# CFGpp-diffusion/CFGpp

Hardware: AMD Instinct MI355X
Metric: images/sec (higher is better)
Workload: dtype fp16; 1 GPU; SD1.5 512x512 ddim_cfg++ 50 NFE lambda=0.6 batch=8/GPU; per_gpu_batch=8, global_batch=8, nfe=50, unet_batch_rows=16, weights=seeded synthetic, exact diffusers shapes, build_id=cfgpp-build:af47ed5b841e1037:nogit

## Files before the change

cfgpp_amd/_lib.py:

```python
from __future__ import annotations

import ctypes as C
import os

HERE = os.path.dirname(os.path.abspath(__file__))
LIB_PATH = os.environ.get("CFGPP_LIB") or os.path.join(HERE, "libcfgpp_hip.so")


class CfgppError(RuntimeError):
    pass


class UNetConfigC(C.Structure):
    _fields_ = [
        ("in_channels", C.c_int), ("out_channels", C.c_int),
        ("num_levels", C.c_int),
        ("block_out_channels", C.c_int * 4),
        ("layers_per_block", C.c_int),
        ("level_has_attn", C.c_int * 4),
        ("transformer_depth", C.c_int * 4),
        ("num_heads", C.c_int * 4),
        ("cross_attention_dim", C.c_int),
        ("addition_embed", C.c_int),
        ("addition_time_embed_dim", C.c_int),
        ("addition_pooled_dim", C.c_int),
        ("norm_groups", C.c_int),
        ("sample_h", C.c_int), ("sample_w", C.c_int),
        ("max_rows", C.c_int),
    ]


_P, _I, _F, _L = C.c_void_p, C.c_int, C.c_float, C.c_long

PROTOTYPES = {
    "cfgpp_last_error": (C.c_char_p, []),
    "cfgpp_build_id": (C.c_char_p, []),
    "cfgpp_step_ddim": (_I, [_P, _P, _P, _P, _I, _F, _F, _F, _F, _F, _I, _I, _L, _P]),
    "cfgpp_step_ddim_h": (_I, [_P, _P, _P, _P, _F, _F, _F, _F, _F, _I, _I, _L, _P]),
    "cfgpp_step_ddim_masked": (_I, [_P, _P, _P, _P, _F, _F, _F, _F, _F, _I, _I, _P, _P, _P, _F, _F, _I, _L, _P]),
    "cfgpp_kdiff_input": (_I, [_P, _P, _F, _I, _L, _P]),
    "cfgpp_step_kdiff": (_I, [_P, _P, _P, _P, _P, C.POINTER(C.c_float), _I, _I, _I, _I, _L, _P]),
    "cfgpp_kdiff_denoise": (_I, [_P, _P, _P, _F, _F, _P, _P, _L, _P]),
    "cfgpp_lincomb": (_I, [_P, _P, _P, _P, _F, _F, _I, _L, _P]),
    "cfgpp_unet_create": (_P, [C.POINTER(UNetConfigC), _I]),
    "cfgpp_unet_destroy": (None, [_P]),
    "cfgpp_unet_load_tensor": (_I, [_P, C.c_char_p, _P, _I, C.POINTER(C.c_long), _I]),
    "cfgpp_unet_missing": (_I, [_P]),
    "cfgpp_unet_finalize": (_I, [_P]),
    "cfgpp_unet_set_context": (_I, [_P, _P, _I, _I, _P, _P, _I, _P]),
    "cfgpp_unet_image_condition": (_I, [_P, _P, _I, _P]),
    "cfgpp_unet_forward": (_I, [_P, _P, _I, _I, _F, _P, _I, _P]),
    "cfgpp_sample_graph_ddim": (_I, [_P, _P, _P, _I, _I, _P, _P, _P, _I, C.POINTER(C.c_float), _I, _F, _I, _I, _P]),
    "cfgpp_unet_profile": (_I, [_P, _P, _I, _I, _F, _P, _I, _P, C.POINTER(C.c_double), C.POINTER(C.c_double), C.POINTER(C.c_int), C.c_char_p, _L]),
    "cfgpp_unet_tuning": (_I, [_P, _I, C.POINTER(C.c_int), _I, _I]),
    "cfgpp_unet_attach_control": (_I, [_P, _P, _F]),
    "cfgpp_unet_flops": (C.c_double, [_P, _I]),
    "cfgpp_unet_device_bytes": (C.c_double, [_P]),
    "cfgpp_vae_create": (_P, [_I, _I, _I, _F, _I]),
    "cfgpp_vae_destroy": (None, [_P]),
    "cfgpp_vae_load_tensor": (_I, [_P, C.c_char_p, _P, _I, C.POINTER(C.c_long), _I]),
    "cfgpp_vae_finalize": (_I, [_P]),
    "cfgpp_vae_decode": (_I, [_P, _P, _P, _I, _P]),
    "cfgpp_vae_decode_image": (_I, [_P, _P, _P, _I, _P]),
    "cfgpp_vae_encode": (_I, [_P, _P, _P, _P, _P, _I, _P]),
    "cfgpp_vae_profile": (_I, [_P, _P, _P, _I, _P, C.c_char_p, C.c_long]),
    "cfgpp_vae_flops": (C.c_double, [_P, _I]),
    "cfgpp_text_create": (_P, [_I, _I, _I, _I, _I, _I, _I, _I, _I]),
    "cfgpp_text_destroy": (None, [_P]),
    "cfgpp_text_load_tensor": (_I, [_P, C.c_char_p, _P, _I, C.POINTER(C.c_long), _I]),
    "cfgpp_text_finalize": (_I, [_P]),
    "cfgpp_text_encode": (_I, [_P, C.POINTER(C.c_int), C.POINTER(C.c_int), _I, _I, _P, _P, _P]),
    "cfgpp_text_device_bytes": (C.c_double, [_P]),
    "cfgpp_vae_encode_flops": (C.c_double, [_P, _I]),
    "cfgpp_vae_device_bytes": (C.c_double, [_P]),
}

DEBUG_PROTOTYPES = {
    "cfgpp_op_softmax_rows": (_I, [_P, _L, _I, _P]),
    "cfgpp_op_conv_in_ex": (_I, [_P, _I, _P, _P, _P, _I, _I, _I, _I, _I, _I, _P, _P, _F, _P]),
    "cfgpp_op_groupnorm": (_I, [_P, _P, _P, _P, _P, _P, _I, _I, _I, _I, _I, _I, _F, _I, _I, _P]),
    "cfgpp_op_groupnorm_pre": (_I, [_P, _P, _P, _P, _P, _P, _P, _P, _I, _I, _I, _I, _I, _I, _F, _I, _I, _P]),
    "cfgpp_op_igemm_set_gstat": (None, [_P]),
    "cfgpp_op_igemm_gstat_written": (_I, []),
    "cfgpp_groupnorm_set_prestats": (None, [_I]),
    "cfgpp_groupnorm_prestats_enabled": (_I, []),
    "cfgpp_unet_set_share_prefix": (None, [_I]),
    "cfgpp_unet_share_prefix_enabled": (_I, []),
    "cfgpp_unet_shared_prefix_ops": (_I, [_P, _I, _I]),
    "cfgpp_op_layernorm": (_I, [_P, _P, _P, _P, _L, _I, _F, _P]),
    "cfgpp_op_attention_prepare_vt": (_I, [_P, _I, _I, _I, _P]),
    "cfgpp_op_attention": (_I, [_P, _P, _P, _P, _I, _I, _I, _I, _I, _I, _I, _P]),
    "cfgpp_op_conv_in": (_I, [_P, _I, _P, _P, _P, _I, _I, _I, _I, _I, _I, _P]),
    "cfgpp_op_conv_in_cond": (_I, [_P, _I, _P, _I, _I, _P, _P, _P, _I, _I, _I, _I, _I, _I, _P]),
    "cfgpp_op_conv_in_add": (_I, [_P, _I, _P, _I, _I, _P, _I, _P, _P, _P, _I, _I, _I, _I, _I, _I, _P]),
    "cfgpp_op_cn_conv3x3": (_I, [_P, _I, _P, _I, _P, _P, _I, _I, _I, _I, _I, _I, _I, _P]),
    "cfgpp_op_residual_add": (_I, [C.POINTER(C.c_void_p), C.POINTER(C.c_void_p), C.POINTER(C.c_int), _I, _I, _F, _P]),
    "cfgpp_op_residual_nchw": (_I, [_P, _P, _I, _I, _I, _I, _F, _P]),
    "cfgpp_controlnet_residual": (_I, [_P, _I, _F, _P, _I, C.POINTER(C.c_int), _P]),
    "cfgpp_op_vae_posterior": (_I, [_P, _P, _P, _P, _P, _P, _I, _I, _F, _P]),
    "cfgpp_op_conv_out": (_I, [_P, _P, _I, _P, _P, _I, _I, _I, _I, _I, _P]),
    "cfgpp_op_conv_out_ex": (_I, [_P, _P, _I, _P, _P, _I, _I, _I, _I, _I, _F, _F, _I, _P]),
    "cfgpp_conv_out_set_tiled": (None, [_I]),
    "cfgpp_op_sinusoid": (_I, [_P, _F, _P, _I, _I, _I, _I, _P]),
    "cfgpp_op_skinny_gemm": (_I, [_P, _I, _P, _P, _P, _I, _P, _I, _I, _I, _I, _I, _I, _P]),
    "cfgpp_op_f16_to_f32_rows": (_I, [_P, _P, _I, _I, _I, _I, _P]),
    "cfgpp_op_igemm": (_I, [_P, _P, _I, _I, _I, _I, _I, _I, _P, _I, _I, _P, _P, _I, _P, _I, _I, _P, _I, _I, _I, _P]),
    "cfgpp_op_igemm_heads": (_I, [_P, _I, _P, _I, _I, _P, _I, _P, _P, _P, _I, _I, _I, _I, _I, _I, _P]),
    "cfgpp_igemm_force_config": (None, [_I]),
    "cfgpp_igemm_set_staging": (None, [_I]),
    "cfgpp_igemm_set_staged_epilogue": (None, [_I]),
    "cfgpp_igemm_set_big_tiles": (None, [_I]),
    "cfgpp_igemm_set_tail_split": (None, [_I]),
    "cfgpp_igemm_set_autotune": (None, [_I]),
    "cfgpp_igemm_set_blocked_walk": (None, [_I]),
    "cfgpp_igemm_walk_plan_probe": (None, [_I, _I, _I, _I, _I, _I, _I, C.POINTER(C.c_int)]),
    "cfgpp_igemm_set_n_major": (None, [_I]),
    "cfgpp_igemm_force_split": (None, [_I]),
    "cfgpp_igemm_set_split_tile": (None, [_I]),
    "cfgpp_igemm_set_mf16": (None, [_I]),
    "cfgpp_igemm_set_mf16_rounds": (None, [_I]),
    "cfgpp_igemm_set_mf16_heads": (None, [_I]),
    "cfgpp_igemm_set_mf16_linear": (None, [_I]),
    "cfgpp_igemm_set_big_split": (None, [_I]),
    "cfgpp_igemm_set_tune_mask": (None, [C.c_uint]),
    "cfgpp_igemm_tuner_state": (C.c_uint, []),
    "cfgpp_igemm_timeline": (None, [_P, _L, _I]),
    "cfgpp_igemm_timeline_info": (None, [C.POINTER(C.c_int)]),
    "cfgpp_groupnorm_set_mode": (None, [_I]),
    "cfgpp_layernorm_set_rows_per_wave": (None, [_I]),
    "cfgpp_attention_set_dma": (None, [_I]),
    "cfgpp_attention_set_stagger": (None, [_I]),
    "cfgpp_attention_set_cross": (None, [_I]),
}

_lib = None


def load():
    global _lib
    if _lib is not None:
        return _lib
    if not os.path.exists(LIB_PATH):
        raise CfgppError(
            f"{LIB_PATH} not found: build it with `python -m cfgpp_amd.build` "
            "(__graft_entry__.build()).  The HIP path has no CPU fallback.")
    import torch
    try:
        lib = C.CDLL(LIB_PATH)
    except OSError as e:
        raise CfgppError(f"cannot load {LIB_PATH}: {e}") from e
    for name, (res, args) in list(PROTOTYPES.items()) + list(DEBUG_PROTOTYPES.items()):
        try:
            fn = getattr(lib, name)
        except AttributeError as e:
            raise CfgppError(f"{LIB_PATH} does not export {name}") from e
        fn.restype = res
        fn.argtypes = args
    if os.environ.get("CFGPP_AUTOTUNE", "1") == "0":
        lib.cfgpp_igemm_set_autotune(0)
    _lib = lib
    return lib


def build_id() -> str:
    return load().cfgpp_build_id().decode("utf-8", "replace")


def last_error() -> str:
    return load().cfgpp_last_error().decode("utf-8", "replace")


def check(rc: int, what: str):
    if rc != 0:
        raise CfgppError(f"{what} failed (rc={rc}): {last_error()}")
```

cfgpp_amd/build.py:

```python
from __future__ import annotations

import hashlib
import os
import subprocess
import sys
from concurrent.futures import ThreadPoolExecutor

HERE = os.path.dirname(os.path.abspath(__file__))
CSRC = os.path.join(HERE, "csrc")
OUT = os.path.join(HERE, "libcfgpp_hip.so")
OBJ = os.path.join(CSRC, "_obj")

SOURCES = [
    ("errors.cpp", []),
    ("step_kernels.hip", ["-ffp-contract=off"]),
    ("norm_kernels.hip", []),
    ("small_kernels.hip", []),
    ("igemm_kernel.hip", []),
    ("big4_kernel.hip", []),
    ("big4p_kernel.hip", []),
    ("attn_kernel.hip", ["-mllvm", "-amdgpu-mfma-vgpr-form=1"]),
    ("controlnet_kernels.hip", ["-ffp-contract=off"]),
    ("unet.hip", []),
    ("vae.hip", []),
    ("text.hip", []),
]
COMMON = ["--offload-arch=gfx950", "-O3", "-std=c++17", "-fPIC", "-Wno-unused-result"]
ASAN_FLAGS = ["-fsanitize=address", "-fno-gpu-sanitize", "-g", "-fno-omit-frame-pointer"]


def _hipcc() -> str:
    for c in (os.environ.get("HIPCC"), "/opt/rocm/bin/hipcc", "hipcc"):
        if c and (os.path.isabs(c) and os.path.exists(c) or not os.path.isabs(c)):
            return c
    return "hipcc"


_INC = None


def _deps(src: str) -> set:
    import re
    global _INC
    if _INC is None:
        _INC = re.compile(r'^\s*#\s*include\s+"([^"]+)"', re.M)
    seen, todo = set(), [src]
    while todo:
        f = todo.pop()
        try:
            text = open(f, errors="replace").read()
        except OSError:
            continue
        for inc in _INC.findall(text):
            h = os.path.normpath(os.path.join(os.path.dirname(f), inc))
            if h not in seen and os.path.exists(h):
                seen.add(h)
                todo.append(h)
    return seen


def _digest(src: str, flags) -> str:
    h = hashlib.sha256()
    h.update((" ".join(flags) + "\0" + _hipcc_version()).encode())
    for f in [src, *sorted(_deps(src))]:
        h.update(os.path.relpath(f, HERE).encode() + b"\0")
        with open(f, "rb") as fh:
            h.update(fh.read())
    return h.hexdigest()[:16]


_HIPCC_VERSION = None


def _hipcc_version() -> str:
    global _HIPCC_VERSION
    if _HIPCC_VERSION is None:
        try:
            out = subprocess.run([_hipcc(), "--version"], capture_output=True, text=True).stdout
            _HIPCC_VERSION = " ".join(ln.strip() for ln in out.splitlines() if "version" in ln.lower())[:200]
        except OSError:
            _HIPCC_VERSION = "unknown"
    return _HIPCC_VERSION


def source_digest() -> str:
    h = hashlib.sha256()
    for f, extra in SOURCES:
        h.update(_digest(os.path.join(CSRC, f), COMMON + extra).encode())
    return h.hexdigest()[:16]


def _git_head() -> str:
    try:
        root = os.path.dirname(HERE)
        head = subprocess.run(["git", "-C", root, "rev-parse", "--short=12", "HEAD"], capture_output=True, text=True).stdout.strip()
        dirty = subprocess.run(["git", "-C", root, "status", "--porcelain", "--", "cfgpp_amd/csrc", "include"], capture_output=True,
                               text=True).stdout.strip()
        return (head or "nogit") + ("+local" if dirty else "")
    except OSError:
        return "nogit"


def library_build_id(path: str = OUT) -> str:
    try:
        data = open(path, "rb").read()
    except OSError:
        return ""
    i = data.find(b"cfgpp-build:")
    return data[i:data.index(b"\0", i)].decode() if i >= 0 else ""


def build_asan(verbose: bool = True) -> str:
    out = os.path.join(HERE, "libcfgpp_hip_asan.so")
    obj_dir = os.path.join(CSRC, "_obj_asan")
    os.makedirs(obj_dir, exist_ok=True)
    hipcc = _hipcc()
    jobs, objs = [], []
    for f, extra in SOURCES:
        src = os.path.join(CSRC, f)
        flags = COMMON + ASAN_FLAGS + extra
        obj = os.path.join(obj_dir, f"{os.path.splitext(f)[0]}.{_digest(src, flags)}.o")
        objs.append(obj)
        if not os.path.exists(obj):
            jobs.append((f, [hipcc] + flags + ["-x", "hip", "-c", src, "-o", obj]))
    with ThreadPoolExecutor(max_workers=8) as ex:
        for f, r in zip([j[0] for j in jobs], ex.map(lambda j: subprocess.run(j[1], capture_output=True, text=True), jobs)):
            if verbose:
                print(f"[cfgpp build asan] {f}: {'ok' if r.returncode == 0 else 'FAILED'}", flush=True)
            if r.returncode != 0:
                raise RuntimeError(f"hipcc failed on {f}:\n{r.stdout}{r.stderr}")
    bid_src = os.path.join(obj_dir, "build_id.cpp")
    with open(bid_src, "w") as fh:
        fh.write('extern "C" const char* cfgpp_build_id(void) { return "cfgpp-build:%s:%s+asan"; }\n' % (source_digest(), _git_head()))
    cmd = [hipcc, "--offload-arch=gfx950", "-shared", "-fPIC", "-fsanitize=address", "-fno-gpu-sanitize", "-shared-libsan", "-o", out] + objs + [bid_src]
    r = subprocess.run(cmd, capture_output=True, text=True)
    if r.returncode != 0:
        raise RuntimeError("asan link failed:\n" + r.stdout + r.stderr)
    if verbose:
        print(f"[cfgpp build asan] linked {out}", flush=True)
    return out


def build(force: bool = False, verbose: bool = True) -> str:
    os.makedirs(OBJ, exist_ok=True)
    hipcc = _hipcc()
    jobs, objs = [], []
    for f, extra in SOURCES:
        src = os.path.join(CSRC, f)
        stem = os.path.splitext(f)[0]
        obj = os.path.join(OBJ, f"{stem}.{_digest(src, COMMON + extra)}.o")
        objs.append(obj)
        if force or not os.path.exists(obj):
            jobs.append((f, [hipcc] + COMMON + extra + ["-x", "hip", "-c", src, "-o", obj]))

    def run(job):
        f, cmd = job
        r = subprocess.run(cmd, capture_output=True, text=True)
        if r.returncode != 0 and os.path.exists(cmd[-1]):
            os.remove(cmd[-1])
        return f, r.returncode, r.stdout + r.stderr

    if jobs:
        with ThreadPoolExecutor(max_workers=min(8, len(jobs))) as ex:
            for f, rc, log in ex.map(run, jobs):
                if verbose:
                    print(f"[cfgpp build] {f}: {'ok' if rc == 0 else 'FAILED'}", flush=True)
                if rc != 0:
                    raise RuntimeError(f"hipcc failed on {f}:\n{log}")
    keep = set(objs)
    for old in os.listdir(OBJ):
        if old.endswith(".o") and os.path.join(OBJ, old) not in keep:
            os.remove(os.path.join(OBJ, old))
    want = source_digest()
    have = library_build_id()
    if force or jobs or not have.startswith(f"cfgpp-build:{want}:"):
        bid_src, bid_obj = os.path.join(OBJ, "build_id.cpp"), os.path.join(OBJ, "build_id.o")
        with open(bid_src, "w") as fh:
            fh.write('extern "C" const char* cfgpp_build_id(void) { return "cfgpp-build:%s:%s"; }\n' % (want, _git_head()))
        r = subprocess.run([hipcc, "-O2", "-fPIC", "-c", bid_src, "-o", bid_obj], capture_output=True, text=True)
        if r.returncode != 0:
            raise RuntimeError("build_id.cpp failed:\n" + r.stdout + r.stderr)
        cmd = [hipcc, "--offload-arch=gfx950", "-shared", "-fPIC", "-o", OUT + ".tmp"] + objs + [bid_obj]
        r = subprocess.run(cmd, capture_output=True, text=True)
        if r.returncode != 0:
            raise RuntimeError("link failed:\n" + r.stdout + r.stderr)
        os.replace(OUT + ".tmp", OUT)
        os.remove(bid_obj)
        if verbose:
            print(f"[cfgpp build] linked {OUT} ({library_build_id()})", flush=True)
    return OUT


if __name__ == "__main__":
    if "--asan" in sys.argv:
        print(build_asan())
    else:
        build(force="--force" in sys.argv)
        print(library_build_id())
```

cfgpp_amd/csrc/attn_kernel.hip:

```cpp
#include "common.h"

namespace {

constexpr float RESCALE_THR = 5.0f;

struct AttnArgs {
    const half_t* q; const half_t* k; const half_t* vt;
    half_t* o;
    int heads, d;
    int nq, nk_valid;
    int q_tok_pad, k_tok_pad;
    int o_ld;
    int nqb;
    float scale_log2e;
    int stagger;
};

__device__ __forceinline__ void attn_block_map(int nqb, int& qb, int& bh) {
    const int T = gridDim.x, bid = blockIdx.x;
    const int q = T >> 3, r = T & 7, xcd = bid & 7, idx = bid >> 3;
    const int w = (xcd < r ? xcd * (q + 1) : r * (q + 1) + (xcd - r) * q) + idx;
    bh = w / nqb; qb = w - bh * nqb;
}

template <int D16, int DT, bool ONES, int QT>
__global__ void __launch_bounds__(256)
attn_kernel(const AttnArgs a) {
    constexpr int DP = DT * 32;
    constexpr int KPITCH = DP * 2 + 16;
    constexpr int VPITCH = 64 * 2 + 16;
    constexpr int CH = (64 * DP / 8) / 256;
    constexpr int STAGE = 64 * KPITCH + DP * VPITCH;
    static_assert((64 * DP / 8) % 256 == 0, "tile/loader mismatch");
    extern __shared__ __attribute__((aligned(16))) char smem[];

    const int tid = threadIdx.x, lane = tid & 63, wid = tid >> 6;
    const int l31 = lane & 31, hi = lane >> 5;
    int qb, bh;
    attn_block_map(a.nqb, qb, bh);
    const int q0 = qb * (128 * QT) + wid * (32 * QT);
    const half_t* Qb = a.q + (long)bh * a.q_tok_pad * DP;
    const half_t* Kb = a.k + (long)bh * a.k_tok_pad * DP;
    const half_t* Vb = a.vt + (long)bh * DP * a.k_tok_pad;

    half8_t qf[QT][D16];
#pragma unroll
    for (int qt = 0; qt < QT; ++qt)
#pragma unroll
        for (int ks = 0; ks < D16; ++ks) {
            const half8_t raw = *reinterpret_cast<const half8_t*>(Qb + (long)(q0 + qt * 32 + l31) * DP + ks * 16 + hi * 8);
#pragma unroll
            for (int j = 0; j < 8; ++j) qf[qt][ks][j] = (half_t)((float)raw[j] * a.scale_log2e);
        }

    f32x16 oacc[QT][DT];
    f32x16 negm[QT];
    float l_run[QT];
#pragma unroll
    for (int qt = 0; qt < QT; ++qt) {
        l_run[qt] = 0.f;
#pragma unroll
        for (int r = 0; r < 16; ++r) negm[qt][r] = 0.f;
#pragma unroll
        for (int i = 0; i < DT; ++i)
#pragma unroll
            for (int r = 0; r < 16; ++r) oacc[qt][i][r] = 0.f;
    }

    const int ntiles = (a.nk_valid + 63) >> 6;
    const int tail = a.nk_valid & 63;

    half8_t rk[CH], rv[CH];
    auto load_tile = [&](int t) {
#pragma unroll
        for (int j = 0; j < CH; ++j) {
            const int c = tid + j * 256;
            const int kr = c / (DP / 8), kc = c - kr * (DP / 8);
            rk[j] = *reinterpret_cast<const half8_t*>(Kb + (long)(t * 64 + kr) * DP + kc * 8);
            const int vr = c >> 3, vc = c & 7;
            rv[j] = *reinterpret_cast<const half8_t*>(Vb + (long)vr * a.k_tok_pad + t * 64 + vc * 8);
        }
    };
    auto store_tile = [&](int stage) {
        char* Ks = smem + stage * STAGE;
        char* Vs = Ks + 64 * KPITCH;
#pragma unroll
        for (int j = 0; j < CH; ++j) {
            const int c = tid + j * 256;
            const int kr = c / (DP / 8), kc = c - kr * (DP / 8);
            *reinterpret_cast<half8_t*>(Ks + kr * KPITCH + kc * 16) = rk[j];
            const int vr = c >> 3, vc = c & 7;
            *reinterpret_cast<half8_t*>(Vs + vr * VPITCH + vc * 16) = rv[j];
        }
    };

    load_tile(0);
    store_tile(0);
    __syncthreads();
    if (ntiles > 1) load_tile(1);
    for (int t = 0; t < ntiles; ++t) {
        const char* Ks = smem + (t & 1) * STAGE;
        const char* Vs = Ks + 64 * KPITCH;

        f32x16 s[QT][2];
#pragma unroll
        for (int kt = 0; kt < 2; ++kt) {
#pragma unroll
            for (int ks = 0; ks < D16; ++ks) {
                const half8_t kf = *reinterpret_cast<const half8_t*>(Ks + (kt * 32 + l31) * KPITCH + (ks * 16 + hi * 8) * 2);
#pragma unroll
                for (int qt = 0; qt < QT; ++qt)
                    s[qt][kt] = __builtin_amdgcn_mfma_f32_32x32x16_f16(kf, qf[qt][ks], ks == 0 ? negm[qt] : s[qt][kt], 0, 0, 0);
            }
        }
        if (tail != 0 && t == ntiles - 1) {
            const int kbase = t * 64 + 4 * hi;
#pragma unroll
            for (int qt = 0; qt < QT; ++qt)
#pragma unroll
                for (int kt = 0; kt < 2; ++kt)
#pragma unroll
                    for (int r = 0; r < 16; ++r) {
                        const int key = kbase + kt * 32 + (r & 3) + 8 * (r >> 2);
                        s[qt][kt][r] = key < a.nk_valid ? s[qt][kt][r] : -INFINITY;
                    }
        }
#pragma unroll
        for (int qt = 0; qt < QT; ++qt) {
            float mx = s[qt][0][0];
#pragma unroll
            for (int kt = 0; kt < 2; ++kt)
#pragma unroll
                for (int r = 0; r < 16; ++r) mx = fmaxf(mx, s[qt][kt][r]);
            mx = fmaxf(mx, __shfl_xor(mx, 32));
            if (t == 0 || !__all(mx <= RESCALE_THR)) {
                const float delta = t == 0 ? mx : fmaxf(mx, 0.f);
                const float alpha = __builtin_amdgcn_exp2f(-delta);
                l_run[qt] *= alpha;
#pragma unroll
                for (int i = 0; i < DT; ++i)
#pragma unroll
                    for (int r = 0; r < 16; ++r) oacc[qt][i][r] *= alpha;
#pragma unroll
                for (int r = 0; r < 16; ++r) negm[qt][r] -= delta;
#pragma unroll
                for (int kt = 0; kt < 2; ++kt)
#pragma unroll
                    for (int r = 0; r < 16; ++r) s[qt][kt][r] -= delta;
            }
            float psum = 0.f;
#pragma unroll
            for (int kt = 0; kt < 2; ++kt)
#pragma unroll
                for (int r = 0; r < 16; ++r) {
                    const float pv = __builtin_amdgcn_exp2f(s[qt][kt][r]);
                    s[qt][kt][r] = pv;
                    if constexpr (!ONES) psum += pv;
                }
            if constexpr (!ONES) l_run[qt] += psum;
        }

#pragma unroll
        for (int kt = 0; kt < 2; ++kt)
#pragma unroll
            for (int tt = 0; tt < 2; ++tt) {
                half8_t pf[QT];
#pragma unroll
                for (int qt = 0; qt < QT; ++qt)
#pragma unroll
                    for (int j = 0; j < 8; ++j) pf[qt][j] = (half_t)s[qt][kt][8 * tt + j];
                const int kpos0 = kt * 32 + 16 * tt + 8 * hi;
#pragma unroll
                for (int i = 0; i < DT; ++i) {
                    const half8_t vf = *reinterpret_cast<const half8_t*>(Vs + (i * 32 + l31) * VPITCH + kpos0 * 2);
#pragma unroll
                    for (int qt = 0; qt < QT; ++qt)
                        oacc[qt][i] = __builtin_amdgcn_mfma_f32_32x32x16_f16(vf, pf[qt], oacc[qt][i], 0, 0, 0);
                }
            }
        if (t + 1 < ntiles) store_tile((t + 1) & 1);
        __syncthreads();
        if (t + 2 < ntiles) load_tile(t + 2);
    }

#pragma unroll
    for (int qt = 0; qt < QT; ++qt) {
        float l_tot;
        if constexpr (ONES) {
            const int dr = a.d & 31;
            float lv = 0.f;
#pragma unroll
            for (int g = 0; g < 4; ++g) if (dr == 8 * g) lv = oacc[qt][DT - 1][4 * g];
            l_tot = __shfl(lv, l31);
        } else {
            l_tot = l_run[qt] + __shfl_xor(l_run[qt], 32);
        }
        const float inv_l = 1.0f / l_tot;
        const int q = q0 + qt * 32 + l31;
        if (q < a.nq) {
            const int b = bh / a.heads, head = bh - b * a.heads;
            half_t* orow = a.o + ((long)b * a.nq + q) * a.o_ld + head * a.d;
#pragma unroll
            for (int i = 0; i < DT; ++i)
#pragma unroll
                for (int g = 0; g < 4; ++g) {
                    const int dd = i * 32 + 8 * g + 4 * hi;
                    if (dd < a.d) {
                        half4_t o;
#pragma unroll
                        for (int k = 0; k < 4; ++k) o[k] = (half_t)(oacc[qt][i][4 * g + k] * inv_l);
                        *reinterpret_cast<half4_t*>(orow + dd) = o;
                    }
                }
        }
    }
}

template <int D16, bool ONES, int NST, int WPE = 3>
__global__ void __launch_bounds__(256) __attribute__((amdgpu_waves_per_eu(WPE, WPE)))
attn64_kernel(const AttnArgs a) {
    constexpr int DP = 64, DT = 2;
    constexpr int TILE = 64 * 128;
    constexpr int STAGE = 2 * TILE;
    constexpr int PPW = 4;
    extern __shared__ __attribute__((aligned(16))) char smem[];

    const int tid = threadIdx.x, lane = tid & 63;
    const int wid = __builtin_amdgcn_readfirstlane(tid >> 6);
    const int l31 = lane & 31, hi = lane >> 5;
    int qb, bh;
    attn_block_map(a.nqb, qb, bh);
    const int q0 = qb * 128 + wid * 32;
    const half_t* Qb = a.q + (long)bh * a.q_tok_pad * DP;
    const half_t* Kb = a.k + (long)bh * a.k_tok_pad * DP;
    const half_t* Vb = a.vt + (long)bh * DP * a.k_tok_pad;

    const int r8 = lane >> 3, pc = lane & 7;
    int koff[2], voff[2];
#pragma unroll
    for (int h = 0; h < 2; ++h) {
        const int row = wid * 16 + h * 8 + r8;
        const int lc = pc ^ ((row >> 1) & 7);
        koff[h] = row * DP + lc * 8;
        voff[h] = row * a.k_tok_pad + lc * 8;
    }
    auto dma_tile = [&](int t, int stage) {
        char* Ks = smem + stage * STAGE;
        char* Vs = Ks + TILE;
        const half_t* Kt = Kb + (long)t * 64 * DP;
        const half_t* Vt = Vb + (long)t * 64;
#pragma unroll
        for (int h = 0; h < 2; ++h) {
            __builtin_amdgcn_global_load_lds((const __attribute__((address_space(1))) void*)(Kt + koff[h]),
                                             (__attribute__((address_space(3))) void*)(Ks + (wid * 16 + h * 8) * 128), 16, 0, 0);
            __builtin_amdgcn_global_load_lds((const __attribute__((address_space(1))) void*)(Vt + voff[h]),
                                             (__attribute__((address_space(3))) void*)(Vs + (wid * 16 + h * 8) * 128), 16, 0, 0);
        }
    };

    const int ntiles = (a.nk_valid + 63) >> 6;
    const int tail = a.nk_valid & 63;
    if (a.stagger > 0) {
        const int slot = ((blockIdx.x >> 3) >> 5) % 3;
        for (int i = 0; i < slot * a.stagger; ++i) __builtin_amdgcn_s_sleep(1);
    }
#pragma unroll
    for (int t = 0; t < NST - 1; ++t) if (t < ntiles) dma_tile(t, t);

    half8_t qf[D16];
#pragma unroll
    for (int ks = 0; ks < D16; ++ks) {
        const half8_t raw = *reinterpret_cast<const half8_t*>(Qb + (long)(q0 + l31) * DP + ks * 16 + hi * 8);
#pragma unroll
        for (int j = 0; j < 8; ++j) qf[ks][j] = (half_t)((float)raw[j] * a.scale_log2e);
    }

    f32x16 oacc[DT];
    f32x16 negm;
    float l_run = 0.f;
#pragma unroll
    for (int r = 0; r < 16; ++r) negm[r] = 0.f;
#pragma unroll
    for (int i = 0; i < DT; ++i)
#pragma unroll
        for (int r = 0; r < 16; ++r) oacc[i][r] = 0.f;

    const int fsw = (l31 >> 1) & 7;
    const int frow = l31 * 128;
    for (int t = 0; t < ntiles; ++t) {
        if (NST > 2 && t + 1 < ntiles) asm volatile("s_waitcnt vmcnt(%0)" :: "n"((NST - 2) * PPW) : "memory");
        else asm volatile("s_waitcnt vmcnt(0)" ::: "memory");
        __builtin_amdgcn_s_barrier();
        asm volatile("" ::: "memory");
        if (t + NST - 1 < ntiles) dma_tile(t + NST - 1, (t + NST - 1) % NST);
        const char* Ks = smem + (t % NST) * STAGE;
        const char* Vs = Ks + TILE;

        f32x16 s[2];
        {
#pragma unroll
            for (int kt = 0; kt < 2; ++kt) {
#pragma unroll
                for (int k0 = 0; k0 < D16; k0 += 2) {
                    half8_t kf1[2];
#pragma unroll
                    for (int u = 0; u < 2; ++u)
                        if (k0 + u < D16) kf1[u] = *reinterpret_cast<const half8_t*>(Ks + kt * 32 * 128 + frow + (((((k0 + u) << 1) | hi) ^ fsw) << 4));
#pragma unroll
                    for (int u = 0; u < 2; ++u)
                        if (k0 + u < D16) s[kt] = __builtin_amdgcn_mfma_f32_32x32x16_f16(kf1[u], qf[k0 + u], k0 + u == 0 ? negm : s[kt], 0, 0, 0);
                    __builtin_amdgcn_sched_barrier(0);
                }
            }
        }
        if (tail != 0 && t == ntiles - 1) {
            const int kbase = t * 64 + 4 * hi;
#pragma unroll
            for (int kt = 0; kt < 2; ++kt)
#pragma unroll
                for (int r = 0; r < 16; ++r) {
                    const int key = kbase + kt * 32 + (r & 3) + 8 * (r >> 2);
                    s[kt][r] = key < a.nk_valid ? s[kt][r] : -INFINITY;
                }
        }
        float mx = s[0][0];
#pragma unroll
        for (int kt = 0; kt < 2; ++kt)
#pragma unroll
            for (int r = 0; r < 16; ++r) mx = fmaxf(mx, s[kt][r]);
        mx = fmaxf(mx, __shfl_xor(mx, 32));
        if (t == 0 || !__all(mx <= RESCALE_THR)) {
            const float delta = t == 0 ? mx : fmaxf(mx, 0.f);
            const float alpha = __builtin_amdgcn_exp2f(-delta);
            l_run *= alpha;
#pragma unroll
            for (int i = 0; i < DT; ++i)
#pragma unroll
                for (int r = 0; r < 16; ++r) oacc[i][r] *= alpha;
#pragma unroll
            for (int r = 0; r < 16; ++r) negm[r] -= delta;
#pragma unroll
            for (int kt = 0; kt < 2; ++kt)
#pragma unroll
                for (int r = 0; r < 16; ++r) s[kt][r] -= delta;
        }
        float psum = 0.f;
#pragma unroll
        for (int kt = 0; kt < 2; ++kt)
#pragma unroll
            for (int r = 0; r < 16; ++r) {
                const float pv = __builtin_amdgcn_exp2f(s[kt][r]);
                s[kt][r] = pv;
                if constexpr (!ONES) psum += pv;
            }
        if constexpr (!ONES) l_run += psum;

#pragma unroll
        for (int kt = 0; kt < 2; ++kt)
#pragma unroll
            for (int tt = 0; tt < 2; ++tt) {
                half8_t pf;
#pragma unroll
                for (int j = 0; j < 8; ++j) pf[j] = (half_t)s[kt][8 * tt + j];
                const int lc = kt * 4 + 2 * tt + hi;
#pragma unroll
                for (int i = 0; i < DT; ++i) {
                    const half8_t vf = *reinterpret_cast<const half8_t*>(Vs + i * 32 * 128 + frow + ((lc ^ fsw) << 4));
                    oacc[i] = __builtin_amdgcn_mfma_f32_32x32x16_f16(vf, pf, oacc[i], 0, 0, 0);
                }
            }
    }

    int lane_f = threadIdx.x & 63;
    asm volatile("" : "+v"(lane_f));
    const int l31_f = lane_f & 31, hi_f = lane_f >> 5;
    float l_tot;
    if constexpr (ONES) {
        const int dr = a.d & 31;
        float lv = 0.f;
#pragma unroll
        for (int g = 0; g < 4; ++g) if (dr == 8 * g) lv = oacc[DT - 1][4 * g];
        l_tot = __shfl(lv, l31_f);
    } else {
        l_tot = l_run + __shfl_xor(l_run, 32);
    }
    const float inv_l = 1.0f / l_tot;
    const int q = qb * 128 + wid * 32 + l31_f;
    if (q < a.nq) {
        const int b = bh / a.heads, head = bh - b * a.heads;
        half_t* orow = a.o + ((long)b * a.nq + q) * a.o_ld + head * a.d;
#pragma unroll
        for (int i = 0; i < DT; ++i)
#pragma unroll
            for (int g = 0; g < 4; ++g) {
                const int dd = i * 32 + 8 * g + 4 * hi_f;
                if (dd < a.d) {
                    half4_t o;
#pragma unroll
                    for (int k = 0; k < 4; ++k) o[k] = (half_t)(oacc[i][4 * g + k] * inv_l);
                    *reinterpret_cast<half4_t*>(orow + dd) = o;
                }
            }
    }
}

template <int D16, bool ONES>
__global__ void __launch_bounds__(256)
xattn64_kernel(const AttnArgs a, int xqb , int nxb ) {
    constexpr int DP = 64, DT = 2, TILE = 64 * 128;
    extern __shared__ __attribute__((aligned(16))) char smem[];
    const int tid = threadIdx.x, lane = tid & 63;
    const int wid = __builtin_amdgcn_readfirstlane(tid >> 6);
    const int l31 = lane & 31, hi = lane >> 5;
    int xb, bh;
    {
        const int T = gridDim.x, bid = blockIdx.x;
        const int q = T >> 3, r = T & 7, xcd = bid & 7, idx = bid >> 3;
        const int w = (xcd < r ? xcd * (q + 1) : r * (q + 1) + (xcd - r) * q) + idx;
        bh = w / nxb; xb = w - bh * nxb;
    }
    const half_t* Qb = a.q + (long)bh * a.q_tok_pad * DP;
    const half_t* Kb = a.k + (long)bh * a.k_tok_pad * DP;
    const half_t* Vb = a.vt + (long)bh * DP * a.k_tok_pad;
    const int ntiles = (a.nk_valid + 63) >> 6;
    {
        const int r8 = lane >> 3, pc = lane & 7;
#pragma unroll
        for (int t = 0; t < 2; ++t) {
            if (t < ntiles) {
#pragma unroll
                for (int h = 0; h < 2; ++h) {
                    const int row = wid * 16 + h * 8 + r8;
                    const int lc = pc ^ ((row >> 1) & 7);
                    __builtin_amdgcn_global_load_lds((const __attribute__((address_space(1))) void*)(Kb + (long)(t * 64 + row) * DP + lc * 8),
                                                     (__attribute__((address_space(3))) void*)(smem + t * 2 * TILE + (wid * 16 + h * 8) * 128), 16, 0, 0);
                    __builtin_amdgcn_global_load_lds((const __attribute__((address_space(1))) void*)(Vb + (long)row * a.k_tok_pad + t * 64 + lc * 8),
                                                     (__attribute__((address_space(3))) void*)(smem + t * 2 * TILE + TILE + (wid * 16 + h * 8) * 128), 16, 0, 0);
                }
            }
        }
    }
    const int fsw = (l31 >> 1) & 7;
    const int frow = l31 * 128;
    const int nsub = (a.nk_valid + 31) >> 5;
    const int b = bh / a.heads, head = bh - b * a.heads;
    half8_t qf[D16];
    int q0 = (xb * xqb) * 128 + wid * 32;
#pragma unroll
    for (int ks = 0; ks < D16; ++ks) qf[ks] = *reinterpret_cast<const half8_t*>(Qb + (long)(q0 + l31) * DP + ks * 16 + hi * 8);
    asm volatile("s_waitcnt vmcnt(0)" ::: "memory");
    __syncthreads();
    for (int blk = 0; blk < xqb; ++blk) {
        half8_t qs[D16];
#pragma unroll
        for (int ks = 0; ks < D16; ++ks)
#pragma unroll
            for (int j = 0; j < 8; ++j) qs[ks][j] = (half_t)((float)qf[ks][j] * a.scale_log2e);
        const int qrow = q0 + l31;
        const int q0n = blk + 1 < xqb ? q0 + 128 : q0;
#pragma unroll
        for (int ks = 0; ks < D16; ++ks) qf[ks] = *reinterpret_cast<const half8_t*>(Qb + (long)(q0n + l31) * DP + ks * 16 + hi * 8);
        f32x16 s[4];
#pragma unroll
        for (int st = 0; st < 4; ++st) {
#pragma unroll
            for (int r = 0; r < 16; ++r) s[st][r] = 0.f;
            if (st < nsub) {
                const char* Ks = smem + (st >> 1) * 2 * TILE + (st & 1) * 32 * 128;
#pragma unroll
                for (int ks = 0; ks < D16; ++ks) {
                    const half8_t kf = *reinterpret_cast<const half8_t*>(Ks + frow + ((((ks << 1) | hi) ^ fsw) << 4));
                    s[st] = __builtin_amdgcn_mfma_f32_32x32x16_f16(kf, qs[ks], s[st], 0, 0, 0);
                }
            }
        }
        float mx = -INFINITY;
#pragma unroll
        for (int st = 0; st < 4; ++st) {
            if (st < nsub) {
                if (st == nsub - 1 && (a.nk_valid & 31) != 0) {
                    const int nv = (a.nk_valid & 31) - 4 * hi;
#pragma unroll
                    for (int r = 0; r < 16; ++r) s[st][r] = ((r & 3) + 8 * (r >> 2)) < nv ? s[st][r] : -INFINITY;
                }
#pragma unroll
                for (int r = 0; r < 16; ++r) mx = fmaxf(mx, s[st][r]);
            }
        }
        mx = fmaxf(mx, __shfl_xor(mx, 32));
        float psum = 0.f;
#pragma unroll
        for (int st = 0; st < 4; ++st) {
            if (st < nsub) {
#pragma unroll
                for (int r = 0; r < 16; ++r) {
                    const float pv = __builtin_amdgcn_exp2f(s[st][r] - mx);
                    s[st][r] = pv;
                    if constexpr (!ONES) psum += pv;
                }
            }
        }
        f32x16 oacc[DT];
#pragma unroll
        for (int i = 0; i < DT; ++i)
#pragma unroll
            for (int r = 0; r < 16; ++r) oacc[i][r] = 0.f;
#pragma unroll
        for (int st = 0; st < 4; ++st) {
            if (st < nsub) {
                const char* Vs = smem + (st >> 1) * 2 * TILE + TILE;
#pragma unroll
                for (int tt = 0; tt < 2; ++tt) {
                    half8_t pf;
#pragma unroll
                    for (int j = 0; j < 8; ++j) pf[j] = (half_t)s[st][8 * tt + j];
                    const int lc = (st & 1) * 4 + 2 * tt + hi;
#pragma unroll
                    for (int i = 0; i < DT; ++i) {
                        const half8_t vf = *reinterpret_cast<const half8_t*>(Vs + i * 32 * 128 + frow + ((lc ^ fsw) << 4));
                        oacc[i] = __builtin_amdgcn_mfma_f32_32x32x16_f16(vf, pf, oacc[i], 0, 0, 0);
                    }
                }
            }
        }
        float l_tot;
        if constexpr (ONES) {
            const int dr = a.d & 31;
            float lv = 0.f;
#pragma unroll
            for (int g = 0; g < 4; ++g) if (dr == 8 * g) lv = oacc[DT - 1][4 * g];
            l_tot = __shfl(lv, l31);
        } else {
            l_tot = psum + __shfl_xor(psum, 32);
        }
        const float inv_l = 1.0f / l_tot;
        if (qrow < a.nq) {
            half_t* orow = a.o + ((long)b * a.nq + qrow) * a.o_ld + head * a.d;
#pragma unroll
            for (int i = 0; i < DT; ++i)
#pragma unroll
                for (int g = 0; g < 4; ++g) {
                    const int dd = i * 32 + 8 * g + 4 * hi;
                    if (dd < a.d) {
                        half4_t o;
#pragma unroll
                        for (int k = 0; k < 4; ++k) o[k] = (half_t)(oacc[i][4 * g + k] * inv_l);
                        *reinterpret_cast<half4_t*>(orow + dd) = o;
                    }
                }
        }
        q0 = q0n;
    }
}

template <int D16, bool ONES, int NST, int WPE = 3>
int launch_attn64(const AttnArgs& a, dim3 grid, hipStream_t s) {
    constexpr int smem = NST * 2 * 64 * 128;
    static bool attr_set = false;
    auto kern = attn64_kernel<D16, ONES, NST, WPE>;
    if (!attr_set) {
        CFGPP_HIP_CHECK(hipFuncSetAttribute(reinterpret_cast<const void*>(kern), hipFuncAttributeMaxDynamicSharedMemorySize, smem));
        attr_set = true;
    }
    hipLaunchKernelGGL(kern, grid, dim3(256), smem, s, a);
    return 0;
}

__global__ void attn_ones_row_kernel(half_t* vt, int BH, int d, int dp, int tok_pad) {
    const long i = (long)blockIdx.x * blockDim.x + threadIdx.x;
    if (i >= (long)BH * tok_pad) return;
    const long bh = i / tok_pad, k = i - bh * tok_pad;
    vt[(bh * dp + d) * tok_pad + k] = (half_t)1.0f;
}

template <int D16, int DT, bool ONES, int QT>
int launch_attn(const AttnArgs& a, dim3 grid, hipStream_t s) {
    constexpr int DP = DT * 32;
    constexpr int smem = 2 * (64 * (DP * 2 + 16) + DP * (64 * 2 + 16));
    static bool attr_set = false;
    auto kern = attn_kernel<D16, DT, ONES, QT>;
    if (!attr_set) {
        CFGPP_HIP_CHECK(hipFuncSetAttribute(reinterpret_cast<const void*>(kern), hipFuncAttributeMaxDynamicSharedMemorySize, smem));
        attr_set = true;
    }
    hipLaunchKernelGGL(kern, grid, dim3(256), smem, s, a);
    return 0;
}

}

static int g_attn_dma = 1;
static int g_attn_cross = 1;
static int g_attn_stagger = 0;

extern "C" {

void cfgpp_attention_set_dma(int mode) { g_attn_dma = mode ? 1 : 0; }
void cfgpp_attention_set_stagger(int sleeps) { g_attn_stagger = sleeps > 0 ? sleeps : 0; }
void cfgpp_attention_set_cross(int on) { g_attn_cross = on ? 1 : 0; }

int cfgpp_op_attention_prepare_vt(void* vt, int BH, int d, int tok_pad, void* stream) {
    CFGPP_REQUIRE(vt && BH > 0 && d > 0 && tok_pad > 0, "attention_prepare_vt: bad args");
    if (d % 32 == 0) return 0;
    CFGPP_REQUIRE(d % 8 == 0, "attention: head dim %d (not a multiple of 32) must be a multiple of 8", d);
    const int dp = (d + 31) / 32 * 32;
    hipLaunchKernelGGL(attn_ones_row_kernel, dim3(cdiv((long)BH * tok_pad, 256)), dim3(256), 0, (hipStream_t)stream, (half_t*)vt, BH, d, dp, tok_pad);
    CFGPP_HIP_CHECK(hipGetLastError());
    return 0;
}

int cfgpp_op_attention(const void* q, const void* k, const void* vt, void* o, int B, int heads, int d,
                       int nq, int nk, int q_tok_pad, int k_tok_pad, void* stream) {
    CFGPP_REQUIRE(q && k && vt && o, "attention: null pointer");
    CFGPP_REQUIRE(d > 0 && d <= 160 && (d % 32 == 0 || d % 8 == 0), "attention: head dim %d unsupported (multiple of 8, <= 160)", d);
    CFGPP_REQUIRE(q_tok_pad % 128 == 0 && q_tok_pad >= nq, "attention: q_tok_pad=%d (nq=%d) must be a multiple of 128", q_tok_pad, nq);
    CFGPP_REQUIRE(k_tok_pad % 64 == 0 && k_tok_pad >= nk, "attention: k_tok_pad=%d (nk=%d) must be a multiple of 64", k_tok_pad, nk);
    AttnArgs a;
    a.q = (const half_t*)q; a.k = (const half_t*)k; a.vt = (const half_t*)vt; a.o = (half_t*)o;
    a.heads = heads; a.d = d; a.nq = nq; a.nk_valid = nk; a.q_tok_pad = q_tok_pad; a.k_tok_pad = k_tok_pad;
    a.o_ld = heads * d;
    a.scale_log2e = (1.0f / sqrtf((float)d)) * 1.4426950408889634f;
    a.nqb = cdiv(nq, 128);
    a.stagger = g_attn_stagger;
    dim3 grid(a.nqb * B * heads);
    hipStream_t s = (hipStream_t)stream;
    const int d16 = (d + 15) / 16, dt = (d + 31) / 32;
    const bool ones = (d % 32) != 0;
    if (dt == 2 && g_attn_dma && g_attn_cross && nk <= 128 && k_tok_pad >= 64 * ((nk + 63) >> 6)) {
        const int BH = B * heads;
        int xqb = 1;
        while (xqb < 8 && a.nqb % (xqb * 2) == 0 && (long)BH * (a.nqb / (xqb * 2)) >= 512) xqb *= 2;
        const int nxb = a.nqb / xqb;
        static bool attr_set = false;
        if (!attr_set) {
            CFGPP_HIP_CHECK(hipFuncSetAttribute(reinterpret_cast<const void*>(xattn64_kernel<3, true>), hipFuncAttributeMaxDynamicSharedMemorySize, 4 * 64 * 128));
            CFGPP_HIP_CHECK(hipFuncSetAttribute(reinterpret_cast<const void*>(xattn64_kernel<4, true>), hipFuncAttributeMaxDynamicSharedMemorySize, 4 * 64 * 128));
            CFGPP_HIP_CHECK(hipFuncSetAttribute(reinterpret_cast<const void*>(xattn64_kernel<4, false>), hipFuncAttributeMaxDynamicSharedMemorySize, 4 * 64 * 128));
            attr_set = true;
        }
        const dim3 xg(BH * nxb);
        if (d16 == 3) hipLaunchKernelGGL((xattn64_kernel<3, true>), xg, dim3(256), 4 * 64 * 128, s, a, xqb, nxb);
        else if (ones) hipLaunchKernelGGL((xattn64_kernel<4, true>), xg, dim3(256), 4 * 64 * 128, s, a, xqb, nxb);
        else hipLaunchKernelGGL((xattn64_kernel<4, false>), xg, dim3(256), 4 * 64 * 128, s, a, xqb, nxb);
        CFGPP_HIP_CHECK(hipGetLastError());
        return 0;
    }
    if (dt == 2 && g_attn_dma) {
        int rc;
        if (d16 == 3) rc = launch_attn64<3, true, 2, 4>(a, grid, s);
        else rc = ones ? launch_attn64<4, true, 2, 4>(a, grid, s) : launch_attn64<4, false, 2, 4>(a, grid, s);
        if (rc) return -1;
        CFGPP_HIP_CHECK(hipGetLastError());
        return 0;
    }
#define ATTN_CASE(D16_, DT_) \
    if (d16 == D16_ && dt == DT_) { if (ones ? launch_attn<D16_, DT_, true, 1>(a, grid, s) : launch_attn<D16_, DT_, false, 1>(a, grid, s)) return -1; } else
    ATTN_CASE(1, 1) ATTN_CASE(2, 1) ATTN_CASE(3, 2) ATTN_CASE(4, 2) ATTN_CASE(5, 3) ATTN_CASE(6, 3)
    ATTN_CASE(8, 4) ATTN_CASE(10, 5)
    { cfgpp_set_error("attention: no kernel instance for head dim %d", d); return -2; }
#undef ATTN_CASE
    CFGPP_HIP_CHECK(hipGetLastError());
    return 0;
}

}
```

cfgpp_amd/csrc/cfgpp_debug.h:

```cpp
#ifndef CFGPP_DEBUG_H
#define CFGPP_DEBUG_H
#ifdef __cplusplus
extern "C" {
#endif

int cfgpp_op_softmax_rows(void* s, long rows, int ncols, void* stream);
int cfgpp_op_conv_in_ex(const void* z, int z_is_half, void* out, const float* w, const float* bias,
                        int R, int zB, int Cin, int H, int W, int Cout, const float* pre_w, const float* pre_b,
                        float in_scale, void* stream);
int cfgpp_op_groupnorm(const void* src0, const void* src1, void* dst, const float* gamma, const float* beta,
                       float* stats, int N, int H, int W, int C0, int C1, int G, float eps, int silu,
                       int dst_padded, void* stream);
int cfgpp_op_groupnorm_pre(const void* src0, const void* src1, void* dst, const float* gamma, const float* beta,
                           const float* gst0, const float* gst1, float* stats, int N, int H, int W, int C0, int C1, int G,
                           float eps, int silu, int dst_padded, void* stream);
void cfgpp_op_igemm_set_gstat(void* buf);
int cfgpp_op_igemm_gstat_written(void);
void cfgpp_groupnorm_set_prestats(int on);
int cfgpp_groupnorm_prestats_enabled(void);
void cfgpp_unet_set_share_prefix(int on);
int cfgpp_unet_share_prefix_enabled(void);
int cfgpp_unet_shared_prefix_ops(cfgpp_unet* u, int rows, int z_rows);
void cfgpp_groupnorm_set_mode(int mode);
int cfgpp_op_layernorm(const void* x, void* y, const float* gamma, const float* beta, long rows, int C,
                       float eps, void* stream);
void cfgpp_layernorm_set_rows_per_wave(int rpw);
int cfgpp_op_attention_prepare_vt(void* vt, int BH, int d, int tok_pad, void* stream);
int cfgpp_op_attention(const void* q, const void* k, const void* vt, void* o, int B, int heads, int d,
                       int nq, int nk, int q_tok_pad, int k_tok_pad, void* stream);
void cfgpp_attention_set_dma(int mode);
void cfgpp_attention_set_stagger(int sleeps);
void cfgpp_attention_set_cross(int on);
int cfgpp_op_conv_in(const void* z, int z_is_half, void* out, const float* w, const float* bias,
                     int R, int zB, int Cin, int H, int W, int Cout, void* stream);
int cfgpp_op_conv_in_cond(const void* z, int z_is_half, const void* cond, int cond_rows, int Cc, void* out, const float* w,
                          const float* bias, int R, int zB, int Cz, int H, int W, int Cout, void* stream);
int cfgpp_op_conv_in_add(const void* z, int z_is_half, const void* cond, int cond_rows, int Cc, const void* addend, int add_rows,
                         void* out, const float* w, const float* bias, int R, int zB, int Cz, int H, int W, int Cout, void* stream);
int cfgpp_op_cn_conv3x3(const void* in, int in_kind, void* out, int out_pad, const float* w, const float* bias, int R, int Ci, int Co,
                        int Hi, int Wi, int stride, int silu, void* stream);
int cfgpp_op_residual_add(void* const* dst, const void* const* src, const int* hwc, int n, int rows, float scale, void* stream);
int cfgpp_op_residual_nchw(const void* src, float* out, int rows, int H, int W, int C, float scale, void* stream);
int cfgpp_controlnet_residual(cfgpp_unet* cn, int i, float scale, float* out, int rows, int* hwc_out, void* stream);

int cfgpp_op_vae_posterior(const float* conv_out, const float* qw, const float* qb, const float* noise, float* z,
                           float* moments, int B, int HW, float scale, void* stream);
int cfgpp_op_conv_out(const void* x, void* out, int out_is_half, const void* w, const float* bias,
                      int R, int H, int W, int C, int Cout, void* stream);
int cfgpp_op_conv_out_ex(const void* x, void* out, int out_is_half, const void* w, const float* bias,
                         int R, int H, int W, int C, int Cout, float post_scale, float post_shift, int clamp01, void* stream);
void cfgpp_conv_out_set_tiled(int on);
int cfgpp_op_sinusoid(const float* vals, float scalar, float* out, int count, int dim, int out_ld, int out_off,
                      void* stream);
int cfgpp_op_skinny_gemm(const float* x, int ldx, const void* w, const float* bias, const float* addend, int add_ld,
                         float* out, int ldo, int M, int N, int K, int silu_in, int silu_out, void* stream);
int cfgpp_op_f16_to_f32_rows(const void* in, float* out, int rows, int cols, int out_ld, int out_off, void* stream);

int cfgpp_op_igemm(const void* a0, const void* a1, int C0, int C1, int taps, int amode, int H, int W,
                   const void* w, int M, int N, const float* bias, const float* temb, int temb_ld,
                   const void* resid, int rmode, int rld, void* out, int omode, int old_, int epi,
                   void* stream);
int cfgpp_op_igemm_heads(const void* a, int K, const void* w, int M, int N, const float* bias, int rows_per_batch,
                         void* hq, void* hk, void* hvt, int part0, int part_width, int head_dim, int heads,
                         int q_tok_pad, int tok_pad, void* stream);
void cfgpp_igemm_force_config(int cfg);
void cfgpp_igemm_set_tail_split(int on);
void cfgpp_igemm_set_mf16(int mode);
void cfgpp_igemm_set_mf16_linear(int on);
void cfgpp_igemm_set_mf16_heads(int on);
void cfgpp_igemm_set_mf16_rounds(int n);
void cfgpp_igemm_set_split_tile(int cfg);
void cfgpp_igemm_force_split(int s);
void cfgpp_igemm_set_big_split(int min_kt);
void cfgpp_igemm_set_n_major(int mode);
void cfgpp_igemm_set_blocked_walk(int on);
void cfgpp_igemm_walk_plan_probe(int M, int N, int K, int BM, int BN, int smem, int n_major, int* out5);
void cfgpp_igemm_set_tune_mask(unsigned mask);
unsigned cfgpp_igemm_tuner_state(void);
void cfgpp_igemm_set_autotune(int on);
void cfgpp_igemm_set_big_tiles(int on);
void cfgpp_igemm_set_staged_epilogue(int on);
void cfgpp_igemm_set_staging(int glds);
void cfgpp_igemm_timeline(void* buf, long cap_blocks, int target);
void cfgpp_igemm_timeline_info(int* out12);

#ifdef __cplusplus
}
#endif
#endif
```

cfgpp_amd/csrc/common.h:

```cpp
#pragma once
#include <hip/hip_runtime.h>
#include <stdint.h>

typedef _Float16 half_t;
typedef _Float16 half2_t __attribute__((ext_vector_type(2)));
typedef _Float16 half4_t __attribute__((ext_vector_type(4)));
typedef _Float16 half8_t __attribute__((ext_vector_type(8)));
typedef float f32x4 __attribute__((ext_vector_type(4)));
typedef float f32x16 __attribute__((ext_vector_type(16)));

#define CFGPP_WAVE 64

void cfgpp_set_error(const char* fmt, ...);
int cfgpp_claim_device(int device_id);
#define CFGPP_HIP_CHECK(expr)                                                         \
    do {                                                                              \
        hipError_t _e = (expr);                                                       \
        if (_e != hipSuccess) {                                                       \
            cfgpp_set_error("%s:%d: %s -> %s", __FILE__, __LINE__, #expr,             \
                            hipGetErrorString(_e));                                   \
            return -1;                                                                \
        }                                                                             \
    } while (0)
#define CFGPP_REQUIRE(cond, ...)                                                      \
    do {                                                                              \
        if (!(cond)) {                                                                \
            cfgpp_set_error(__VA_ARGS__);                                             \
            return -2;                                                                \
        }                                                                             \
    } while (0)

int step_advance_launch(const float* tab, int* idx, float* cur, hipStream_t s);
int step_ddim_dev_launch(void* z, void* z0t_out, const void* eps_uc, const void* eps_c, int eps_is_half, int z_is_half, float lam,
                         const float* cdev, int tweedie_uc, int renoise_uc, long n, hipStream_t s);

struct CnAddEntry {
    half_t* dst;
    const half_t* src;
    int H, W, C, pad_;
};
int cn_residual_add_launch(const CnAddEntry* tab, int n, long max_n8, int rows, float scale, hipStream_t s);

int fanout_rows_launch(half_t* const* p, const long* row_elems, int nseg, int h, hipStream_t s);

static inline int cdiv(long a, long b) { return (int)((a + b - 1) / b); }

struct RowMap {
    int mode;
    int H, W;
    int ld;
};

__host__ __device__ __forceinline__ int cfgpp_vt_pos(int tok) {
    return (tok & ~12) | ((tok & 4) << 1) | ((tok & 8) >> 1);
}

__device__ __forceinline__ float silu_f(float x) { return x / (1.0f + __expf(-x)); }
__device__ __forceinline__ float gelu_erf_f(float x) {
    const float ax = fabsf(x) * 0.70710678118654752440f;
    const float t = __builtin_amdgcn_rcpf(1.0f + 0.3275911f * ax);
    const float poly = t * (0.254829592f + t * (-0.284496736f + t * (1.421413741f + t * (-1.453152027f + t * 1.061405429f))));
    const float erfc_ax = poly * __builtin_amdgcn_exp2f(-ax * ax * 1.4426950408889634f);
    const float cdf = x >= 0.f ? 1.0f - 0.5f * erfc_ax : 0.5f * erfc_ax;
    return x * cdf;
}

typedef float f32x2 __attribute__((ext_vector_type(2)));
#define CFGPP_GELU_C 4.75f
#define CFGPP_GELU_POLY {4.912262559e-01f, 5.645360425e-02f, -1.591939032e-01f, 2.464362979e-01f, -1.982378513e-01f, 1.363233291e-02f, \
                         1.386516690e-01f, -1.158297956e-01f, -9.092462249e-03f, 6.090912968e-02f, -1.936562732e-02f, -1.160200126e-02f, \
                         6.012340542e-03f}
__device__ __forceinline__ f32x2 gelu_erf_pk(f32x2 x) {
    constexpr float k[13] = CFGPP_GELU_POLY;
    f32x2 a;
    a.x = fminf(fabsf(x.x), CFGPP_GELU_C); a.y = fminf(fabsf(x.y), CFGPP_GELU_C);
    const f32x2 t = __builtin_elementwise_fma(a, (f32x2){2.0f / CFGPP_GELU_C, 2.0f / CFGPP_GELU_C}, (f32x2){-1.0f, -1.0f});
    f32x2 p = {k[12], k[12]};
#pragma unroll
    for (int i = 11; i >= 0; --i) p = __builtin_elementwise_fma(p, t, (f32x2){k[i], k[i]});
    f32x2 m;
    m.x = fabsf(x.x) * p.x; m.y = fabsf(x.y) * p.y;
    return __builtin_elementwise_fma(x, (f32x2){0.5f, 0.5f}, m);
}

template <int MAXV>
__device__ __forceinline__ void ln_row_stats(const half8_t (&raw)[MAXV], int chunks, int C, float eps, int lane,
                                             float (&v)[MAXV][8], float& mean, float& rstd) {
    float sum = 0.f;
#pragma unroll
    for (int j = 0; j < MAXV; ++j) {
        const bool live = lane + j * 64 < chunks;
#pragma unroll
        for (int k = 0; k < 8; ++k) { v[j][k] = live ? (float)raw[j][k] : 0.f; sum += v[j][k]; }
    }
#pragma unroll
    for (int o = 32; o > 0; o >>= 1) sum += __shfl_xor(sum, o);
    mean = sum / (float)C;
    float sq = 0.f;
#pragma unroll
    for (int j = 0; j < MAXV; ++j) {
        const bool live = lane + j * 64 < chunks;
#pragma unroll
        for (int k = 0; k < 8; ++k) { const float d = v[j][k] - mean; sq += live ? d * d : 0.f; }
    }
#pragma unroll
    for (int o = 32; o > 0; o >>= 1) sq += __shfl_xor(sq, o);
    rstd = rsqrtf(sq / (float)C + eps);
}
__device__ __forceinline__ half8_t ln_row_affine(const float (&v)[8], float mean, float rstd, const float4 (&g)[2], const float4 (&be)[2]) {
    const float gg[8] = {g[0].x, g[0].y, g[0].z, g[0].w, g[1].x, g[1].y, g[1].z, g[1].w};
    const float bb[8] = {be[0].x, be[0].y, be[0].z, be[0].w, be[1].x, be[1].y, be[1].z, be[1].w};
    half8_t o;
#pragma unroll
    for (int k = 0; k < 8; ++k) o[k] = (half_t)((v[k] - mean) * rstd * gg[k] + bb[k]);
    return o;
}
```

cfgpp_amd/csrc/engine_base.h:

```cpp
#pragma once
#include <algorithm>
#include <cmath>
#include <cstring>
#include <deque>
#include <functional>
#include <map>
#include <string>
#include <utility>
#include <vector>

#include "../../include/cfgpp.h"
#include "cfgpp_debug.h"
#include "igemm.h"

namespace {


struct HostParam {
    std::vector<long> shape;
    std::vector<half_t> h;
    std::vector<float> f;
    bool is_matrix = false;
    bool loaded = false;
    long numel() const { long n = 1; for (long s : shape) n *= s; return n; }
};

struct Tensor {
    half_t* p = nullptr;
    int H = 0, W = 0, C = 0;
    float* gst = nullptr;
    int* gst_ok = nullptr;
};

using Op = std::function<int(hipStream_t, int )>;


struct EngineBase {
    int max_rows = 1;
    int norm_groups = 32;
    std::map<std::string, HostParam> params;
    std::vector<void*> allocs;
    double dev_bytes = 0;
    double macs_per_row = 0;
    double attn_macs_per_row = 0;

    std::vector<Op> plan;
    std::vector<int> plan_kind;
    std::vector<double> plan_macs;
    std::vector<std::string> plan_desc;
    std::vector<char> plan_share;
    int rows_for(size_t i, int rows, bool shared) const {
        const int m = i < plan_share.size() ? plan_share[i] : 0;
        if (m == 0) return rows;
        return shared ? rows / 2 : (m == 1 ? rows : 0);
    }
    void tag(int kind, double macs, const std::string& desc = "") {
        plan_kind.resize(plan.size(), 3); plan_macs.resize(plan.size(), 0.0); plan_desc.resize(plan.size());
        if (!plan.empty()) { plan_kind.back() = kind; plan_macs.back() = macs; plan_desc.back() = desc; }
    }
    std::deque<int> cfg_hints;
    std::vector<int*> plan_hint;
    int tuned_rows = 0;
    bool tuned_shared = false;
    std::map<std::pair<int, bool>, std::vector<int>> tuned_by_rows;
    int* new_hint(bool in_main_plan) {
        cfg_hints.push_back(0);
        int* h = &cfg_hints.back();
        if (in_main_plan) { plan_hint.resize(plan.size() + 1, nullptr); plan_hint[plan.size()] = h; }
        return h;
    }
    int tune_plan(hipStream_t s, int rows, bool shared = false) {
        const auto key = std::make_pair(rows, shared);
        auto cached = tuned_by_rows.find(key);
        if (cached != tuned_by_rows.end() && cached->second.size() == cfg_hints.size()) {
            size_t k = 0;
            for (int& h : cfg_hints) h = cached->second[k++];
            tuned_rows = rows; tuned_shared = shared;
            return 0;
        }
        static const int cands[] = {0, 1, 4, 5, 6, 7, 8, 9, 10, 11, 12, 13, 14, 15, 16, 17, 20, 24, 25, 26, 27, 28};
        const size_t n = plan.size();
        plan_hint.resize(n, nullptr);
        hipStreamCaptureStatus cap = hipStreamCaptureStatusNone;
        if (hipStreamIsCapturing(s, &cap) != hipSuccess || cap != hipStreamCaptureStatusNone) return 0;
        std::vector<hipEvent_t> ev(n + 1, nullptr);
        for (auto& e : ev) if (hipEventCreate(&e) != hipSuccess) return -1;
        std::vector<float> base(n, 1e30f), best(n, 1e30f), t(n);
        std::vector<char> applied(n, 1);
        std::vector<int> bestc(n, 0);
        int rc = 0;
        auto timed_passes = [&]() {
            std::fill(t.begin(), t.end(), 1e30f);
            for (int rep = 0; rep < 2 && rc == 0; ++rep) {
                if (hipEventRecord(ev[0], s) != hipSuccess) rc = -1;
                for (size_t i = 0; i < n && rc == 0; ++i) {
                    rc = plan[i](s, rows_for(i, rows, shared));
                    if (plan_hint[i]) applied[i] = (char)igemm_last_hint_applied();
                    if (rc == 0 && hipEventRecord(ev[i + 1], s) != hipSuccess) rc = -1;
                }
                if (rc == 0 && hipEventSynchronize(ev[n]) != hipSuccess) rc = -1;
                for (size_t i = 0; i < n && rc == 0; ++i) {
                    if (!plan_hint[i]) continue;
                    float ms = 0.f;
                    if (hipEventElapsedTime(&ms, ev[i], ev[i + 1]) == hipSuccess && ms < t[i]) t[i] = ms;
                }
            }
        };
        const unsigned mask = igemm_tune_mask();
        for (int c : cands) {
            if (c != 0 && !((mask >> c) & 1u)) continue;
            for (int& h : cfg_hints) h = c;
            timed_passes();
            for (size_t i = 0; i < n; ++i) {
                if (c == 0) base[i] = t[i];
                if (t[i] < best[i] && (c == 0 || applied[i])) { best[i] = t[i]; bestc[i] = c; }
            }
        }
        for (size_t i = 0; i < n; ++i)
            if (plan_hint[i] && !(bestc[i] != 0 && best[i] < 0.97f * base[i])) { bestc[i] = 0; best[i] = base[i]; }
        for (int walk = 1; walk <= 2 && rc == 0 && (mask >> 31); ++walk) {
            for (size_t i = 0; i < n; ++i) if (plan_hint[i]) *plan_hint[i] = (bestc[i] & 63) | (walk << 6);
            timed_passes();
            for (size_t i = 0; i < n; ++i)
                if (plan_hint[i] && t[i] < 0.97f * best[i]) { best[i] = t[i]; bestc[i] = (bestc[i] & 63) | (walk << 6); }
        }
        for (int& h : cfg_hints) h = 0;
        for (size_t i = 0; i < n; ++i) if (plan_hint[i]) *plan_hint[i] = bestc[i];
        for (auto& e : ev) hipEventDestroy(e);
        if (rc == 0) tuned_by_rows[key] = std::vector<int>(cfg_hints.begin(), cfg_hints.end());
        tuned_rows = rows; tuned_shared = shared;
        return rc;
    }
    std::map<std::tuple<int, int, int>, std::vector<std::pair<half_t*, float*>>> pool;
    std::deque<int> gst_flags;
    float* d_gn_stats = nullptr;
    static constexpr long KSPLIT_WS_BYTES = 128L << 20;
    float* d_ksplit_ws = nullptr;
    float* ksplit_ws() {
        if (!d_ksplit_ws) d_ksplit_ws = (float*)dmalloc((size_t)KSPLIT_WS_BYTES, false);
        return d_ksplit_ws;
    }

    void* dmalloc(size_t bytes, bool zero = true) {
        void* p = nullptr;
        if (hipMalloc(&p, bytes) != hipSuccess) return nullptr;
        if (zero) hipMemset(p, 0, bytes);
        allocs.push_back(p);
        dev_bytes += (double)bytes;
        return p;
    }
    Tensor acq(int H, int W, int C) {
        auto key = std::make_tuple(H, W, C);
        auto& fl = pool[key];
        Tensor t; t.H = H; t.W = W; t.C = C;
        gst_flags.push_back(0);
        t.gst_ok = &gst_flags.back();
        if (!fl.empty()) { t.p = fl.back().first; t.gst = fl.back().second; fl.pop_back(); return t; }
        t.p = (half_t*)dmalloc((size_t)max_rows * (H + 2) * (W + 2) * C * sizeof(half_t));
        if (H * W >= 1024 && (H * W) % 32 == 0 && C % 8 == 0)
            t.gst = (float*)dmalloc((size_t)max_rows * (H * W / 32) * C * 2 * sizeof(float), false);
        return t;
    }
    void rel(const Tensor& t) { if (t.p) pool[std::make_tuple(t.H, t.W, t.C)].push_back(std::make_pair(t.p, t.gst)); }
    ~EngineBase() { for (void* p : allocs) hipFree(p); }
};

void expect(EngineBase* u, const std::string& key, std::vector<long> shape, bool matrix) {
    HostParam hp; hp.shape = std::move(shape); hp.is_matrix = matrix;
    u->params[key] = std::move(hp);
}
void expect_linear(EngineBase* u, const std::string& p, long out, long in, bool bias = true) {
    expect(u, p + ".weight", {out, in}, true);
    if (bias) expect(u, p + ".bias", {out}, false);
}
void expect_conv(EngineBase* u, const std::string& p, long out, long in, int k) {
    expect(u, p + ".weight", {out, in, k, k}, true);
    expect(u, p + ".bias", {out}, false);
}
void expect_norm(EngineBase* u, const std::string& p, long c) {
    expect(u, p + ".weight", {c}, false);
    expect(u, p + ".bias", {c}, false);
}
void expect_resnet(EngineBase* u, const std::string& p, long cin, long cout, long temb) {
    expect_norm(u, p + ".norm1", cin);
    expect_conv(u, p + ".conv1", cout, cin, 3);
    expect_linear(u, p + ".time_emb_proj", cout, temb);
    expect_norm(u, p + ".norm2", cout);
    expect_conv(u, p + ".conv2", cout, cout, 3);
    if (cin != cout) expect_conv(u, p + ".conv_shortcut", cout, cin, 1);
}
void expect_transformer(EngineBase* u, const std::string& p, long c, int depth, long cross) {
    expect_norm(u, p + ".norm", c);
    expect(u, p + ".proj_in.weight", {c, c}, true);  expect(u, p + ".proj_in.bias", {c}, false);
    expect(u, p + ".proj_out.weight", {c, c}, true); expect(u, p + ".proj_out.bias", {c}, false);
    for (int k = 0; k < depth; ++k) {
        const std::string b = p + ".transformer_blocks." + std::to_string(k);
        expect_norm(u, b + ".norm1", c); expect_norm(u, b + ".norm2", c); expect_norm(u, b + ".norm3", c);
        expect_linear(u, b + ".attn1.to_q", c, c, false); expect_linear(u, b + ".attn1.to_k", c, c, false);
        expect_linear(u, b + ".attn1.to_v", c, c, false); expect_linear(u, b + ".attn1.to_out.0", c, c, true);
        expect_linear(u, b + ".attn2.to_q", c, c, false); expect_linear(u, b + ".attn2.to_k", c, cross, false);
        expect_linear(u, b + ".attn2.to_v", c, cross, false); expect_linear(u, b + ".attn2.to_out.0", c, c, true);
        expect_linear(u, b + ".ff.net.0.proj", 8 * c, c, true);
        expect_linear(u, b + ".ff.net.2", c, 4 * c, true);
    }
}

struct Builder {
    EngineBase* u;
    bool ok = true;
    std::string err;

    HostParam* get(const std::string& key) {
        auto it = u->params.find(key);
        if (it == u->params.end() || !it->second.loaded) { ok = false; err = "missing parameter " + key; return nullptr; }
        return &it->second;
    }
    template <typename T>
    T* upload(const std::vector<T>& v) {
        T* d = (T*)u->dmalloc(v.size() * sizeof(T), false);
        if (!d) { ok = false; err = "hipMalloc failed"; return nullptr; }
        if (hipMemcpy(d, v.data(), v.size() * sizeof(T), hipMemcpyHostToDevice) != hipSuccess) { ok = false; err = "hipMemcpy failed"; }
        return d;
    }
    void drop(const std::string& key) { auto& p = u->params[key]; std::vector<half_t>().swap(p.h); std::vector<float>().swap(p.f); }

    float* f32(const std::string& key) {
        HostParam* p = get(key); if (!p) return nullptr;
        float* d = upload(p->f); drop(key); return d;
    }
    half_t* linear(const std::string& key) {
        HostParam* p = get(key); if (!p) return nullptr;
        half_t* d = upload(p->h); drop(key); return d;
    }
    half_t* conv3(const std::string& key) {
        HostParam* p = get(key); if (!p) return nullptr;
        const long O = p->shape[0], I = p->shape[1];
        std::vector<half_t> r((size_t)O * 9 * I);
        for (long o = 0; o < O; ++o)
            for (long i = 0; i < I; ++i)
                for (int t = 0; t < 9; ++t) r[(size_t)o * 9 * I + ((i >> 6) * 9 + t) * 64 + (i & 63)] = p->h[((size_t)o * I + i) * 9 + t];
        half_t* d = upload(r); drop(key); return d;
    }
    std::vector<half_t> concat_host(const std::vector<std::string>& keys) {
        std::vector<half_t> r;
        for (auto& k : keys) { HostParam* p = get(k); if (!p) return {}; r.insert(r.end(), p->h.begin(), p->h.end()); }
        for (auto& k : keys) drop(k);
        return r;
    }
    half_t* concat(const std::vector<std::string>& keys) {
        std::vector<half_t> r = concat_host(keys);
        return ok ? upload(r) : nullptr;
    }
    bool geglu_host(const std::string& pfx, long C, std::vector<half_t>& rw, std::vector<float>& rb) {
        HostParam* pw = get(pfx + ".weight"); HostParam* pb = get(pfx + ".bias");
        if (!pw || !pb) return false;
        const long F = 4 * C;
        rw.resize((size_t)2 * F * C); rb.resize((size_t)2 * F);
        for (long f = 0; f < F; ++f) {
            const long pv = (f / 32) * 64 + (f % 32), pg = pv + 32;
            std::memcpy(&rw[(size_t)pv * C], &pw->h[(size_t)f * C], C * sizeof(half_t));
            std::memcpy(&rw[(size_t)pg * C], &pw->h[(size_t)(F + f) * C], C * sizeof(half_t));
            rb[pv] = pb->f[f]; rb[pg] = pb->f[F + f];
        }
        drop(pfx + ".weight"); drop(pfx + ".bias");
        return true;
    }
    void geglu(const std::string& pfx, long C, half_t** w, float** b) {
        std::vector<half_t> rw; std::vector<float> rb;
        if (!geglu_host(pfx, C, rw, rb)) return;
        *w = upload(rw); *b = upload(rb);
    }
};

inline int round_up(int a, int b) { return (a + b - 1) / b * b; }

IGemmArgs base_args(EngineBase* u = nullptr) {
    IGemmArgs a; std::memset(&a, 0, sizeof(a)); a.out_scale = 1.0f; a.taps = 1;
    if (u) { a.ws_buf = u->ksplit_ws(); a.ws_bytes = a.ws_buf ? EngineBase::KSPLIT_WS_BYTES : 0; }
    return a;
}

struct Plan {
    EngineBase* u;
    Builder* B;
    std::vector<Op>* ops;

    void conv3x3(const Tensor& src, const Tensor& dst, const half_t* w, const float* bias, int amode,
                 const float* temb, int temb_ld, const Tensor* resid, int ashift = 0) {
        IGemmArgs a = base_args(u);
        a.a0 = src.p; a.C0 = src.C; a.taps = 9; a.amode = amode; a.ashift = ashift; a.H = dst.H; a.W = dst.W;
        a.w = w; a.N = dst.C; a.K = 9 * src.C; a.bias = bias; a.temb = temb; a.temb_ld = temb_ld;
        a.rows_per_batch = dst.H * dst.W;
        if (resid) { a.resid = resid->p; a.rmode = 1; a.rld = resid->C; }
        a.out = dst.p; a.omode = 1; a.old = dst.C; a.epi = EPI_STORE;
        a.gstat = dst.gst; a.stat_flag = dst.gst ? dst.gst_ok : nullptr;
        const int HW = dst.H * dst.W;
        u->macs_per_row += (double)HW * dst.C * 9.0 * src.C;
        int* hint = u->new_hint(ops == &u->plan);
        ops->push_back([a, HW, hint](hipStream_t s, int rows) mutable { IGemmArgs b = a; b.M = rows * HW; b.cfg_hint = *hint; return igemm_launch(b, s); });
        if (ops == &u->plan) u->tag(0, (double)HW * dst.C * 9.0 * src.C, "conv3x3 amode=" + std::to_string(amode) + " HW=" + std::to_string(HW) + " N=" + std::to_string(dst.C) + " K=" + std::to_string(9 * src.C) + (resid ? " +res" : "") + (temb ? " +temb" : ""));
    }
    void conv1x1(const Tensor& s0, const Tensor* s1, const Tensor& dst, const half_t* w, const float* bias) {
        IGemmArgs a = base_args(u);
        a.a0 = s0.p; a.C0 = s0.C; if (s1) { a.a1 = s1->p; a.C1 = s1->C; }
        a.amode = 1; a.H = dst.H; a.W = dst.W; a.w = w; a.N = dst.C; a.K = a.C0 + a.C1; a.bias = bias;
        a.rows_per_batch = dst.H * dst.W; a.out = dst.p; a.omode = 1; a.old = dst.C; a.epi = EPI_STORE;
        const int HW = dst.H * dst.W;
        u->macs_per_row += (double)HW * dst.C * a.K;
        int* hint = u->new_hint(ops == &u->plan);
        ops->push_back([a, HW, hint](hipStream_t s, int rows) mutable { IGemmArgs b = a; b.M = rows * HW; b.cfg_hint = *hint; return igemm_launch(b, s); });
        if (ops == &u->plan) u->tag(0, (double)HW * dst.C * a.K, "conv1x1 HW=" + std::to_string(HW) + " N=" + std::to_string(dst.C) + " K=" + std::to_string(a.K));
    }
    void linear(const half_t* A, int K, half_t* out, int N, const half_t* w, const float* bias, const half_t* resid,
                int tokens, int epi = EPI_STORE) {
        IGemmArgs a = base_args(u);
        a.a0 = A; a.C0 = K; a.amode = 0; a.w = w; a.N = N; a.K = K; a.bias = bias;
        a.resid = resid; a.rmode = 0; a.rld = N; a.out = out; a.omode = 0;
        a.old = (epi == EPI_GEGLU) ? N / 2 : N; a.epi = epi; a.rows_per_batch = tokens;
        u->macs_per_row += (double)tokens * N * K;
        int* hint = u->new_hint(ops == &u->plan);
        ops->push_back([a, tokens, hint](hipStream_t s, int rows) mutable { IGemmArgs b = a; b.M = rows * tokens; b.cfg_hint = *hint; return igemm_launch(b, s); });
        if (ops == &u->plan) u->tag(0, (double)tokens * N * K, std::string(epi == EPI_GEGLU ? "geglu" : "linear") + " HW=" + std::to_string(tokens) + " N=" + std::to_string(N) + " K=" + std::to_string(K) + (resid ? " +res" : ""));
    }
    void linear_to_padded(const half_t* A, int K, const Tensor& dst, const half_t* w, const float* bias, const Tensor& resid) {
        IGemmArgs a = base_args(u);
        a.a0 = A; a.C0 = K; a.amode = 0; a.H = dst.H; a.W = dst.W; a.w = w; a.N = dst.C; a.K = K; a.bias = bias;
        a.resid = resid.p; a.rmode = 1; a.rld = resid.C; a.out = dst.p; a.omode = 1; a.old = dst.C;
        a.epi = EPI_STORE; a.rows_per_batch = dst.H * dst.W;
        a.gstat = dst.gst; a.stat_flag = dst.gst ? dst.gst_ok : nullptr;
        const int HW = dst.H * dst.W;
        u->macs_per_row += (double)HW * dst.C * K;
        int* hint = u->new_hint(ops == &u->plan);
        ops->push_back([a, HW, hint](hipStream_t s, int rows) mutable { IGemmArgs b = a; b.M = rows * HW; b.cfg_hint = *hint; return igemm_launch(b, s); });
        if (ops == &u->plan) u->tag(0, (double)HW * dst.C * K, "proj_out HW=" + std::to_string(HW) + " N=" + std::to_string(dst.C) + " K=" + std::to_string(K));
    }
    void heads(const half_t* A, int K, const half_t* w, int N, int tokens, int part0, int C, int nheads,
               half_t* q, half_t* k, half_t* vt, int q_tok_pad, int tok_pad, bool count = true,
               const float* bias = nullptr) {
        IGemmArgs a = base_args(u);
        const int d = C / nheads;
        a.a0 = A; a.C0 = K; a.amode = 0; a.w = w; a.N = N; a.K = K; a.epi = EPI_HEADS;
        a.bias = bias;
        a.rows_per_batch = tokens; a.hq = q; a.hk = k; a.hvt = vt; a.part0 = part0; a.part_width = C;
        a.head_dim = d; a.head_dim_pad = round_up(d, 32); a.heads = nheads; a.tok_pad = tok_pad; a.q_tok_pad = q_tok_pad;
        if (count) u->macs_per_row += (double)tokens * N * K;
        int* hint = u->new_hint(ops == &u->plan);
        ops->push_back([a, tokens, hint](hipStream_t s, int rows) mutable { IGemmArgs b = a; b.M = rows * tokens; b.cfg_hint = *hint; return igemm_launch(b, s); });
        if (ops == &u->plan) u->tag(0, count ? (double)tokens * N * K : 0.0, "heads HW=" + std::to_string(tokens) + " N=" + std::to_string(N) + " K=" + std::to_string(K));
    }
    void groupnorm(const Tensor& s0, const Tensor* s1, half_t* dst, bool dst_padded, const float* g, const float* b,
                   float eps, bool silu) {
        EngineBase* uu = u;
        const half_t* p0 = s0.p; const half_t* p1 = s1 ? s1->p : nullptr;
        const int H = s0.H, W = s0.W, C0 = s0.C, C1 = s1 ? s1->C : 0, G = u->norm_groups;
        const float* gst0 = s0.gst; const float* gst1 = s1 ? s1->gst : nullptr;
        const int* ok0 = s0.gst_ok; const int* ok1 = s1 ? s1->gst_ok : nullptr;
        ops->push_back([=](hipStream_t s, int rows) {
            if (cfgpp_groupnorm_prestats_enabled() && gst0 && ok0 && *ok0 && (!p1 || (gst1 && ok1 && *ok1)))
                return cfgpp_op_groupnorm_pre(p0, p1, dst, g, b, gst0, gst1, uu->d_gn_stats, rows, H, W, C0, C1, G, eps, silu ? 1 : 0,
                                              dst_padded ? 1 : 0, s);
            return cfgpp_op_groupnorm(p0, p1, dst, g, b, uu->d_gn_stats, rows, H, W, C0, C1, G, eps, silu ? 1 : 0,
                                      dst_padded ? 1 : 0, s);
        });
        if (ops == &u->plan) u->tag(2, 0.0, "groupnorm HW=" + std::to_string(H * W) + " C=" + std::to_string(C0 + C1));
    }
    void layernorm(const half_t* x, half_t* y, const float* g, const float* b, int tokens, int C) {
        ops->push_back([=](hipStream_t s, int rows) { return cfgpp_op_layernorm(x, y, g, b, (long)rows * tokens, C, 1e-5f, s); });
        if (ops == &u->plan) u->tag(2, 0.0, "layernorm HW=" + std::to_string(tokens) + " C=" + std::to_string(C));
    }
    void attention(const half_t* q, const half_t* k, const half_t* vt, half_t* o, int nheads, int d, int nq, int nk,
                   int q_tok_pad, int k_tok_pad) {
        u->attn_macs_per_row += 2.0 * (double)nheads * nq * nk * d;
        ops->push_back([=](hipStream_t s, int rows) {
            return cfgpp_op_attention(q, k, vt, o, rows, nheads, d, nq, nk, q_tok_pad, k_tok_pad, s);
        });
        if (ops == &u->plan) u->tag(1, 2.0 * (double)nheads * nq * nk * d, "self_attn heads=" + std::to_string(nheads) + " N=" + std::to_string(nq) + " d=" + std::to_string(d));
    }
};

}
```

cfgpp_amd/csrc/unet.hip:

```cpp
#include "engine_base.h"

struct cfgpp_unet : EngineBase {
    cfgpp_unet_config cfg;
    int device = 0;
    bool finalized = false;

    std::vector<Op> ctx_plan;
    const void* in_z = nullptr; int in_z_half = 0; int in_z_rows = 0; float in_t = 0.f; void* out_eps = nullptr;
    const float* in_t_dev = nullptr;
    half_t* d_cond = nullptr; int cond_rows = 0;
    float* d_step_tab = nullptr; int step_tab_cap = 0; float* d_step_cur = nullptr; int* d_step_idx = nullptr;
    hipStream_t cap_stream = nullptr;
    struct GraphKey { const void* z; void* z0t; void* eps; const void* euc; const void* ec; int z_half, z_rows, rows, tw, rn; float lam; long n; int tuned_serial; int cond_rows; };
    struct Graph { GraphKey key; hipGraph_t graph; hipGraphExec_t exec; };
    std::vector<Graph> graphs;
    int tuned_serial = 0;
    int prefix_ops = 0;
    double prefix_macs_per_row = 0;
    int ran_shared = -1;
    bool shares(int rows, int z_rows) const;
    bool enter_call(int rows, int z_rows) {
        const bool sh = shares(rows, z_rows);
        if (ran_shared != (int)sh) { if (ran_shared >= 0) ++tuned_serial; ran_shared = (int)sh; }
        return sh;
    }
    static void destroy(Graph& g) { if (g.exec) hipGraphExecDestroy(g.exec); if (g.graph) hipGraphDestroy(g.graph); g.exec = nullptr; g.graph = nullptr; }
    void drop_graphs() { for (auto& g : graphs) destroy(g); graphs.clear(); }
    ~cfgpp_unet() { drop_graphs(); if (cap_stream) hipStreamDestroy(cap_stream); }
    const half_t* ctx_ehs = nullptr; int ctx_rows = 0; int ctx_tokens = 77;
    const half_t* ctx_text = nullptr; const float* ctx_tids = nullptr; int ctx_cond_rows = 0;
    bool ctx_set = false;

    float* d_sin_t = nullptr; float* d_emb_h = nullptr; float* d_emb_t = nullptr; float* d_emb = nullptr;
    float* d_temb_all = nullptr; int temb_total = 0;
    float* d_add_in = nullptr; float* d_add_h = nullptr; float* d_aug = nullptr;

    half_t *tok_x = nullptr, *tok_ln = nullptr, *tok_attn = nullptr, *tok_ff = nullptr;
    half_t *hq[4] = {nullptr, nullptr, nullptr, nullptr}, *hk[4] = {nullptr, nullptr, nullptr, nullptr},
           *hvt[4] = {nullptr, nullptr, nullptr, nullptr};

    bool control = false;
    std::vector<int> embed_ch;
    std::vector<Op> img_plan;
    const void* img_in = nullptr; int img_in_half = 0;
    half_t* d_img_emb = nullptr; int img_rows = 0;
    std::vector<Tensor> ctrl_res;
    std::vector<Tensor> ctrl_dst;
    cfgpp_unet* ctrl = nullptr; float ctrl_scale = 0.f;
    CnAddEntry* d_ctrl_tab = nullptr; long ctrl_max_n8 = 0;
};

static int g_share_prefix = 1;
bool cfgpp_unet::shares(int rows, int z_rows) const { return g_share_prefix && prefix_ops > 0 && rows == 2 * z_rows; }

namespace {

void build_param_table(cfgpp_unet* u) {
    const cfgpp_unet_config& c = u->cfg;
    const int L = c.num_levels;
    const long c0 = c.block_out_channels[0], temb = 4 * c0;
    expect_conv(u, "conv_in", c0, c.in_channels, 3);
    expect_linear(u, "time_embedding.linear_1", temb, c0);
    expect_linear(u, "time_embedding.linear_2", temb, temb);
    if (c.addition_embed) {
        const long in = (long)c.addition_time_embed_dim * 6 + c.addition_pooled_dim;
        expect_linear(u, "add_embedding.linear_1", temb, in);
        expect_linear(u, "add_embedding.linear_2", temb, temb);
    }
    long ch = c0;
    for (int i = 0; i < L; ++i) {
        const long co = c.block_out_channels[i];
        const std::string p = "down_blocks." + std::to_string(i);
        for (int j = 0; j < c.layers_per_block; ++j) {
            expect_resnet(u, p + ".resnets." + std::to_string(j), ch, co, temb);
            if (c.level_has_attn[i])
                expect_transformer(u, p + ".attentions." + std::to_string(j), co, c.transformer_depth[i], c.cross_attention_dim);
            ch = co;
        }
        if (i != L - 1) expect_conv(u, p + ".downsamplers.0.conv", co, co, 3);
    }
    const long cm = c.block_out_channels[L - 1];
    expect_resnet(u, "mid_block.resnets.0", cm, cm, temb);
    expect_transformer(u, "mid_block.attentions.0", cm, c.transformer_depth[L - 1], c.cross_attention_dim);
    expect_resnet(u, "mid_block.resnets.1", cm, cm, temb);
    if (u->control) {
        const std::vector<int>& e = u->embed_ch;
        const std::string q = "controlnet_cond_embedding.";
        expect_conv(u, q + "conv_in", e[0], 3, 3);
        for (size_t i = 0; i + 1 < e.size(); ++i) {
            expect_conv(u, q + "blocks." + std::to_string(2 * i), e[i], e[i], 3);
            expect_conv(u, q + "blocks." + std::to_string(2 * i + 1), e[i + 1], e[i], 3);
        }
        expect_conv(u, q + "conv_out", c0, e.back(), 3);
        int k = 0;
        expect_conv(u, "controlnet_down_blocks." + std::to_string(k++), c0, c0, 1);
        for (int i = 0; i < L; ++i) {
            const long co = c.block_out_channels[i];
            for (int j = 0; j < c.layers_per_block; ++j) expect_conv(u, "controlnet_down_blocks." + std::to_string(k++), co, co, 1);
            if (i != L - 1) expect_conv(u, "controlnet_down_blocks." + std::to_string(k++), co, co, 1);
        }
        expect_conv(u, "controlnet_mid_block", cm, cm, 1);
        return;
    }
    long prev = cm;
    for (int i = 0; i < L; ++i) {
        const int lvl = L - 1 - i;
        const long co = c.block_out_channels[lvl];
        const long cin_lvl = c.block_out_channels[std::max(lvl - 1, 0)];
        const std::string p = "up_blocks." + std::to_string(i);
        for (int j = 0; j < c.layers_per_block + 1; ++j) {
            const long skip = (j == c.layers_per_block) ? cin_lvl : co;
            const long rin = (j == 0 ? prev : co) + skip;
            expect_resnet(u, p + ".resnets." + std::to_string(j), rin, co, temb);
            if (c.level_has_attn[lvl])
                expect_transformer(u, p + ".attentions." + std::to_string(j), co, c.transformer_depth[lvl], c.cross_attention_dim);
        }
        if (i != L - 1) expect_conv(u, p + ".upsamplers.0.conv", co, co, 3);
        prev = co;
    }
    expect_norm(u, "conv_norm_out", c0);
    expect_conv(u, "conv_out", c.out_channels, c0, 3);
}

struct ResW {
    float *n1g, *n1b, *n2g, *n2b, *b1, *b2, *bsc;
    half_t *w1, *w2, *wsc;
    int temb_off;
    int cin, cout;
};

int controlnet_tail(cfgpp_unet* u, Builder& B, Plan& P, const std::vector<Tensor>& skips, const Tensor& mid) {
    const cfgpp_unet_config& c = u->cfg;
    const int R = c.max_rows, c0 = c.block_out_channels[0];
    auto persist = [&](int H, int W, int C) {
        Tensor t; t.H = H; t.W = W; t.C = C;
        t.p = (half_t*)u->dmalloc((size_t)R * (H + 2) * (W + 2) * C * sizeof(half_t));
        return t;
    };
    for (size_t k = 0; k <= skips.size(); ++k) {
        const Tensor& src = k < skips.size() ? skips[k] : mid;
        const std::string key = k < skips.size() ? "controlnet_down_blocks." + std::to_string(k) : std::string("controlnet_mid_block");
        half_t* w = B.linear(key + ".weight"); float* b = B.f32(key + ".bias");
        Tensor r = persist(src.H, src.W, src.C);
        CFGPP_REQUIRE(r.p, "finalize: hipMalloc failed");
        P.conv1x1(src, nullptr, r, w, b);
        u->ctrl_res.push_back(r);
    }
    const std::vector<int>& e = u->embed_ch;
    const int n = (int)e.size();
    const std::string q = "controlnet_cond_embedding.";
    struct Layer { std::string key; int ci, co, stride; };
    std::vector<Layer> layers;
    layers.push_back({q + "conv_in", 3, e[0], 1});
    for (int i = 0; i + 1 < n; ++i) {
        layers.push_back({q + "blocks." + std::to_string(2 * i), e[i], e[i], 1});
        layers.push_back({q + "blocks." + std::to_string(2 * i + 1), e[i], e[i + 1], 2});
    }
    long scratch = 1;
    {
        int h = c.sample_h << (n - 1), w = c.sample_w << (n - 1);
        for (size_t l = 0; l + 1 < layers.size(); ++l) {
            if (layers[l].stride == 2) { h = (h - 1) / 2 + 1; w = (w - 1) / 2 + 1; }
            scratch = std::max(scratch, (long)R * h * w * layers[l].co);
        }
    }
    half_t* buf[2] = {(half_t*)u->dmalloc((size_t)scratch * sizeof(half_t), false), (half_t*)u->dmalloc((size_t)scratch * sizeof(half_t), false)};
    Tensor pre = persist(c.sample_h, c.sample_w, e.back());
    CFGPP_REQUIRE(buf[0] && buf[1] && pre.p, "finalize: hipMalloc failed");
    cfgpp_unet* uu = u;
    int h = c.sample_h << (n - 1), w = c.sample_w << (n - 1);
    for (size_t l = 0; l < layers.size(); ++l) {
        const Layer& ly = layers[l];
        HostParam* pw = B.get(ly.key + ".weight");
        CFGPP_REQUIRE(pw, "finalize: %s", B.err.c_str());
        std::vector<float> r((size_t)9 * ly.ci * ly.co);
        for (int o = 0; o < ly.co; ++o) for (int i = 0; i < ly.ci; ++i) for (int t = 0; t < 9; ++t)
            r[((size_t)t * ly.ci + i) * ly.co + o] = (float)pw->h[((size_t)o * ly.ci + i) * 9 + t];
        B.drop(ly.key + ".weight");
        float* dw = B.upload(r); float* db = B.f32(ly.key + ".bias");
        const bool last = l + 1 == layers.size();
        const half_t* in = l == 0 ? nullptr : buf[(l - 1) & 1];
        half_t* out = last ? pre.p : buf[l & 1];
        const int hi = h, wi = w, ci = ly.ci, co = ly.co, st = ly.stride, first = l == 0;
        u->img_plan.push_back([=](hipStream_t s, int rows) {
            return cfgpp_op_cn_conv3x3(first ? uu->img_in : in, first ? (uu->img_in_half ? 1 : 2) : 0, out, last ? 1 : 0, dw, db, rows, ci,
                                       co, hi, wi, st, 1, s);
        });
        if (st == 2) { h = (h - 1) / 2 + 1; w = (w - 1) / 2 + 1; }
    }
    CFGPP_REQUIRE(h == c.sample_h && w == c.sample_w, "finalize: internal error, the embedding ends at %d x %d", h, w);
    {
        half_t* wo = B.conv3(q + "conv_out.weight"); float* bo = B.f32(q + "conv_out.bias");
        Tensor dst; dst.p = u->d_img_emb; dst.H = c.sample_h; dst.W = c.sample_w; dst.C = c0;
        Plan PI{u, &B, &u->img_plan};
        const double macs = u->macs_per_row;
        PI.conv3x3(pre, dst, wo, bo, 1, nullptr, 0, nullptr);
        u->macs_per_row = macs;
    }
    CFGPP_REQUIRE(B.ok, "finalize: %s", B.err.c_str());
    return 0;
}

}

extern "C" {

static cfgpp_unet* unet_new(const cfgpp_unet_config* cfg, int device_id, const int* embed, int n_embed) {
    if (!cfg) { cfgpp_set_error("unet_create: null config"); return nullptr; }
    if (cfg->num_levels < 1 || cfg->num_levels > 4 || cfg->layers_per_block < 1 || cfg->max_rows < 1) {
        cfgpp_set_error("unet_create: bad config"); return nullptr;
    }
    for (int i = 0; i < cfg->num_levels; ++i) {
        const int c = cfg->block_out_channels[i];
        if (c % 64 != 0 || c % cfg->norm_groups != 0) { cfgpp_set_error("unet_create: channels %d must be a multiple of 64 and of norm_groups", c); return nullptr; }
        if (cfg->level_has_attn[i]) {
            const int d = c / cfg->num_heads[i];
            if (c % cfg->num_heads[i] != 0 || d % 4 != 0 || d > 160) { cfgpp_set_error("unet_create: head dim %d unsupported", d); return nullptr; }
        }
    }
    if (cfg->cross_attention_dim % 64 != 0) { cfgpp_set_error("unet_create: cross_attention_dim must be a multiple of 64"); return nullptr; }
    if (!embed && cfg->in_channels > cfg->out_channels && cfg->in_channels > 16) {
        cfgpp_set_error("unet_create: in_channels=%d out_channels=%d (an inpaint UNet takes at most 16 input channels)", cfg->in_channels,
                        cfg->out_channels);
        return nullptr;
    }
    if ((cfg->sample_h % (1 << (cfg->num_levels - 1))) || (cfg->sample_w % (1 << (cfg->num_levels - 1)))) {
        cfgpp_set_error("unet_create: sample size must be divisible by 2^(levels-1)"); return nullptr;
    }
    int ndev = 0;
    if (hipGetDeviceCount(&ndev) != hipSuccess || ndev <= device_id) {
        cfgpp_set_error("unet_create: no HIP device %d (found %d) - the HIP path has no CPU fallback", device_id, ndev);
        return nullptr;
    }
    if (cfgpp_claim_device(device_id)) return nullptr;
    if (hipSetDevice(device_id) != hipSuccess) { cfgpp_set_error("unet_create: hipSetDevice failed"); return nullptr; }
    cfgpp_unet* u = new cfgpp_unet();
    u->cfg = *cfg; u->device = device_id; u->max_rows = cfg->max_rows; u->norm_groups = cfg->norm_groups;
    if (embed) { u->control = true; u->embed_ch.assign(embed, embed + n_embed); }
    build_param_table(u);
    return u;
}

cfgpp_unet* cfgpp_unet_create(const cfgpp_unet_config* cfg, int device_id) {
    if (cfg && cfg->out_channels == 0) {
        static const int embed[4] = {16, 32, 96, 256};
        if (cfg->in_channels < 1 || cfg->in_channels > 8) {
            cfgpp_set_error("unet_create: ControlNet (out_channels = 0) with in_channels=%d (1 .. 8 latent channels)", cfg->in_channels);
            return nullptr;
        }
        return unet_new(cfg, device_id, embed, 4);
    }
    return unet_new(cfg, device_id, nullptr, 0);
}


void cfgpp_unet_destroy(cfgpp_unet* u) {
    if (!u) return;
    delete u;
}

int cfgpp_unet_load_tensor(cfgpp_unet* u, const char* key, const void* host, int dtype, const long* shape, int ndim) {
    CFGPP_REQUIRE(u && key && host && shape, "load_tensor: null argument");
    CFGPP_REQUIRE(!u->finalized, "load_tensor: context already finalized");
    auto it = u->params.find(key);
    if (it == u->params.end()) { cfgpp_set_error("load_tensor: unknown key %s", key); return -3; }
    HostParam& p = it->second;
    long n = 1; for (int i = 0; i < ndim; ++i) n *= shape[i];
    CFGPP_REQUIRE(n == p.numel(), "load_tensor: %s has %ld elements, expected %ld", key, n, p.numel());
    if (ndim == 4) { p.shape.assign(shape, shape + 4); }
    if (p.is_matrix && !(std::string(key) == "conv_in.weight")) {
        p.h.resize(n);
        if (dtype == 0) { const float* s = (const float*)host; for (long i = 0; i < n; ++i) p.h[i] = (half_t)s[i]; }
        else std::memcpy(p.h.data(), host, n * sizeof(half_t));
    } else {
        p.f.resize(n);
        if (dtype == 0) std::memcpy(p.f.data(), host, n * sizeof(float));
        else { const half_t* s = (const half_t*)host; for (long i = 0; i < n; ++i) p.f[i] = (float)s[i]; }
    }
    p.loaded = true;
    return 0;
}

int cfgpp_unet_missing(cfgpp_unet* u) {
    if (!u) return -1;
    int n = 0; std::string names;
    for (auto& kv : u->params) if (!kv.second.loaded) { if (n < 8) names += kv.first + " "; ++n; }
    if (n) cfgpp_set_error("missing %d parameters: %s...", n, names.c_str());
    return n;
}

int cfgpp_unet_finalize(cfgpp_unet* u) {
    CFGPP_REQUIRE(u, "finalize: null");
    CFGPP_REQUIRE(!u->finalized, "finalize: already finalized");
    if (cfgpp_unet_missing(u) != 0) { const std::string m = cfgpp_last_error(); cfgpp_set_error("finalize: %s", m.c_str()); return -2; }
    CFGPP_HIP_CHECK(hipSetDevice(u->device));
    const cfgpp_unet_config& c = u->cfg;
    const int L = c.num_levels, R = c.max_rows;
    const int c0 = c.block_out_channels[0], temb_dim = 4 * c0;
    Builder B{u};
    Plan P{u, &B, &u->plan};
    Plan PC{u, &B, &u->ctx_plan};

    long max_tok_c = 0, max_ff = 0;
    {
        int H = c.sample_h, W = c.sample_w;
        for (int i = 0; i < L; ++i) {
            const long C = c.block_out_channels[i];
            if (c.level_has_attn[i] || i == L - 1) {
                const long tok = (long)H * W;
                const int d = (int)(C / c.num_heads[i]), dp = round_up(d, 32);
                max_tok_c = std::max(max_tok_c, tok * C);
                max_ff = std::max(max_ff, tok * 4 * C);
                u->hq[i] = (half_t*)u->dmalloc((size_t)R * c.num_heads[i] * round_up((int)tok, 128) * dp * 2);
                u->hk[i] = (half_t*)u->dmalloc((size_t)R * c.num_heads[i] * round_up((int)tok, 128) * dp * 2);
                u->hvt[i] = (half_t*)u->dmalloc((size_t)R * c.num_heads[i] * dp * round_up((int)tok, 64) * 2);
                CFGPP_REQUIRE(u->hq[i] && u->hk[i] && u->hvt[i], "finalize: hipMalloc failed");
                if (cfgpp_op_attention_prepare_vt(u->hvt[i], R * c.num_heads[i], d, round_up((int)tok, 64), nullptr)) return -1;
            }
            if (i != L - 1) { H /= 2; W /= 2; }
        }
    }
    u->tok_x = (half_t*)u->dmalloc((size_t)R * max_tok_c * 2);
    u->tok_ln = (half_t*)u->dmalloc((size_t)R * max_tok_c * 2);
    u->tok_attn = (half_t*)u->dmalloc((size_t)R * max_tok_c * 2);
    u->tok_ff = (half_t*)u->dmalloc((size_t)R * max_ff * 2);
    u->d_gn_stats = (float*)u->dmalloc((size_t)R * (1024 * 64 * 2 + 64 * 2) * sizeof(float));
    u->d_sin_t = (float*)u->dmalloc((size_t)c0 * sizeof(float));
    u->d_emb_h = (float*)u->dmalloc((size_t)temb_dim * sizeof(float));
    u->d_emb_t = (float*)u->dmalloc((size_t)temb_dim * sizeof(float));
    u->d_emb = (float*)u->dmalloc((size_t)R * temb_dim * sizeof(float));
    CFGPP_REQUIRE(u->tok_x && u->tok_ln && u->tok_attn && u->tok_ff, "finalize: hipMalloc failed");

    std::vector<std::string> res_names;
    {
        for (int i = 0; i < L; ++i)
            for (int j = 0; j < c.layers_per_block; ++j) res_names.push_back("down_blocks." + std::to_string(i) + ".resnets." + std::to_string(j));
        res_names.push_back("mid_block.resnets.0"); res_names.push_back("mid_block.resnets.1");
        for (int i = 0; i < L && !u->control; ++i)
            for (int j = 0; j < c.layers_per_block + 1; ++j) res_names.push_back("up_blocks." + std::to_string(i) + ".resnets." + std::to_string(j));
    }
    std::map<std::string, int> temb_off;
    half_t* w_temb_all = nullptr; float* b_temb_all = nullptr;
    {
        std::vector<half_t> wa; std::vector<float> ba; int off = 0;
        for (auto& rn : res_names) {
            HostParam* pw = B.get(rn + ".time_emb_proj.weight"); HostParam* pb = B.get(rn + ".time_emb_proj.bias");
            CFGPP_REQUIRE(pw && pb, "finalize: %s", B.err.c_str());
            temb_off[rn] = off; off += (int)pw->shape[0];
            wa.insert(wa.end(), pw->h.begin(), pw->h.end()); ba.insert(ba.end(), pb->f.begin(), pb->f.end());
            B.drop(rn + ".time_emb_proj.weight"); B.drop(rn + ".time_emb_proj.bias");
        }
        u->temb_total = off;
        w_temb_all = B.upload(wa); b_temb_all = B.upload(ba);
        u->d_temb_all = (float*)u->dmalloc((size_t)R * off * sizeof(float));
    }
    const bool per_row_temb = c.addition_embed != 0;
    const int temb_ld = per_row_temb ? u->temb_total : 0;

    {
        half_t* w1 = B.linear("time_embedding.linear_1.weight"); float* b1 = B.f32("time_embedding.linear_1.bias");
        half_t* w2 = B.linear("time_embedding.linear_2.weight"); float* b2 = B.f32("time_embedding.linear_2.bias");
        cfgpp_unet* uu = u;
        u->plan.push_back([=](hipStream_t s, int) { return cfgpp_op_sinusoid(uu->in_t_dev, uu->in_t, uu->d_sin_t, 1, c0, c0, 0, s); });
        u->plan.push_back([=](hipStream_t s, int) { return cfgpp_op_skinny_gemm(uu->d_sin_t, c0, w1, b1, nullptr, 0, uu->d_emb_h, temb_dim, 1, temb_dim, c0, 0, 1, s); });
        if (per_row_temb) {
            u->plan.push_back([=](hipStream_t s, int rows) {
                const int add_ld = uu->ctx_cond_rows == 1 ? 0 : temb_dim;
                return cfgpp_op_skinny_gemm(uu->d_emb_h, 0, w2, b2, uu->d_aug, add_ld, uu->d_emb, temb_dim, rows, temb_dim, temb_dim, 0, 0, s);
            });
            u->plan.push_back([=](hipStream_t s, int rows) {
                return cfgpp_op_skinny_gemm(uu->d_emb, temb_dim, w_temb_all, b_temb_all, nullptr, 0, uu->d_temb_all, uu->temb_total, rows, uu->temb_total, temb_dim, 1, 0, s);
            });
        } else {
            u->plan.push_back([=](hipStream_t s, int) { return cfgpp_op_skinny_gemm(uu->d_emb_h, temb_dim, w2, b2, nullptr, 0, uu->d_emb_t, temb_dim, 1, temb_dim, temb_dim, 0, 0, s); });
            u->plan.push_back([=](hipStream_t s, int) {
                return cfgpp_op_skinny_gemm(uu->d_emb_t, temb_dim, w_temb_all, b_temb_all, nullptr, 0, uu->d_temb_all, uu->temb_total, 1, uu->temb_total, temb_dim, 1, 0, s);
            });
        }
        if (c.addition_embed) {
            const int tdim = c.addition_time_embed_dim, pooled = c.addition_pooled_dim, in = 6 * tdim + pooled;
            half_t* aw1 = B.linear("add_embedding.linear_1.weight"); float* ab1 = B.f32("add_embedding.linear_1.bias");
            half_t* aw2 = B.linear("add_embedding.linear_2.weight"); float* ab2 = B.f32("add_embedding.linear_2.bias");
            u->d_add_in = (float*)u->dmalloc((size_t)R * in * sizeof(float));
            u->d_add_h = (float*)u->dmalloc((size_t)R * temb_dim * sizeof(float));
            u->d_aug = (float*)u->dmalloc((size_t)R * temb_dim * sizeof(float));
            u->ctx_plan.push_back([=](hipStream_t s, int) { return cfgpp_op_f16_to_f32_rows(uu->ctx_text, uu->d_add_in, uu->ctx_cond_rows, pooled, in, 0, s); });
            u->ctx_plan.push_back([=](hipStream_t s, int) {
                for (int r = 0; r < uu->ctx_cond_rows; ++r) {
                    int e = cfgpp_op_sinusoid(uu->ctx_tids + (long)r * 6, 0.f, uu->d_add_in + (long)r * in + pooled, 6, tdim, tdim, 0, s);
                    if (e) return e;
                }
                return 0;
            });
            u->ctx_plan.push_back([=](hipStream_t s, int) { return cfgpp_op_skinny_gemm(uu->d_add_in, in, aw1, ab1, nullptr, 0, uu->d_add_h, temb_dim, uu->ctx_cond_rows, temb_dim, in, 0, 1, s); });
            u->ctx_plan.push_back([=](hipStream_t s, int) { return cfgpp_op_skinny_gemm(uu->d_add_h, temb_dim, aw2, ab2, nullptr, 0, uu->d_aug, temb_dim, uu->ctx_cond_rows, temb_dim, temb_dim, 0, 0, s); });
        }
    }

    auto load_res = [&](const std::string& p, int cin, int cout) {
        ResW w{}; w.cin = cin; w.cout = cout;
        w.n1g = B.f32(p + ".norm1.weight"); w.n1b = B.f32(p + ".norm1.bias");
        w.w1 = B.conv3(p + ".conv1.weight"); w.b1 = B.f32(p + ".conv1.bias");
        w.n2g = B.f32(p + ".norm2.weight"); w.n2b = B.f32(p + ".norm2.bias");
        w.w2 = B.conv3(p + ".conv2.weight"); w.b2 = B.f32(p + ".conv2.bias");
        if (cin != cout) { w.wsc = B.linear(p + ".conv_shortcut.weight"); w.bsc = B.f32(p + ".conv_shortcut.bias"); }
        w.temb_off = temb_off[p];
        return w;
    };
    auto resblock = [&](const std::string& p, const Tensor& x0, const Tensor* x1, int cout) {
        const int cin = x0.C + (x1 ? x1->C : 0);
        ResW w = load_res(p, cin, cout);
        Tensor g1 = u->acq(x0.H, x0.W, cin);
        P.groupnorm(x0, x1, g1.p, true, w.n1g, w.n1b, 1e-5f, true);
        Tensor h1 = u->acq(x0.H, x0.W, cout);
        P.conv3x3(g1, h1, w.w1, w.b1, 1, u->d_temb_all + w.temb_off, temb_ld, nullptr);
        u->rel(g1);
        Tensor g2 = u->acq(x0.H, x0.W, cout);
        P.groupnorm(h1, nullptr, g2.p, true, w.n2g, w.n2b, 1e-5f, true);
        u->rel(h1);
        Tensor out = u->acq(x0.H, x0.W, cout);
        if (cin != cout) {
            Tensor sc = u->acq(x0.H, x0.W, cout);
            P.conv1x1(x0, x1, sc, w.wsc, w.bsc);
            P.conv3x3(g2, out, w.w2, w.b2, 1, nullptr, 0, &sc);
            u->rel(sc);
        } else {
            P.conv3x3(g2, out, w.w2, w.b2, 1, nullptr, 0, &x0);
        }
        u->rel(g2);
        return out;
    };
    int cross_block_counter = 0;
    long prefix_from = -1;
    auto transformer = [&](const std::string& p, const Tensor& x, int depth, int nheads, int lvl) {
        half_t* const HQ = u->hq[lvl]; half_t* const HK = u->hk[lvl]; half_t* const HVT = u->hvt[lvl];
        const int C = x.C, tok = x.H * x.W, d = C / nheads, dp = round_up(d, 32);
        const int q_pad = round_up(tok, 128), k_pad = round_up(tok, 64);
        const int ck_pad = round_up(u->ctx_tokens, 64);
        float* ng = B.f32(p + ".norm.weight"); float* nb = B.f32(p + ".norm.bias");
        half_t* wpi = B.linear(p + ".proj_in.weight"); float* bpi = B.f32(p + ".proj_in.bias");
        half_t* wpo = B.linear(p + ".proj_out.weight"); float* bpo = B.f32(p + ".proj_out.bias");
        P.groupnorm(x, nullptr, u->tok_ln, false, ng, nb, 1e-6f, false);
        P.linear(u->tok_ln, C, u->tok_x, C, wpi, bpi, nullptr, tok);
        for (int k = 0; k < depth; ++k) {
            const std::string b = p + ".transformer_blocks." + std::to_string(k);
            float* l1g = B.f32(b + ".norm1.weight"); float* l1b = B.f32(b + ".norm1.bias");
            float* l2g = B.f32(b + ".norm2.weight"); float* l2b = B.f32(b + ".norm2.bias");
            float* l3g = B.f32(b + ".norm3.weight"); float* l3b = B.f32(b + ".norm3.bias");
            half_t* wqkv = B.concat({b + ".attn1.to_q.weight", b + ".attn1.to_k.weight", b + ".attn1.to_v.weight"});
            half_t* wq2 = B.linear(b + ".attn2.to_q.weight");
            half_t* wff1 = nullptr; float* bff1 = nullptr;
            B.geglu(b + ".ff.net.0.proj", C, &wff1, &bff1);
            half_t* wo1 = B.linear(b + ".attn1.to_out.0.weight"); float* bo1 = B.f32(b + ".attn1.to_out.0.bias");
            half_t* wkv2 = B.concat({b + ".attn2.to_k.weight", b + ".attn2.to_v.weight"});
            half_t* wo2 = B.linear(b + ".attn2.to_out.0.weight"); float* bo2 = B.f32(b + ".attn2.to_out.0.bias");
            half_t* wff2 = B.linear(b + ".ff.net.2.weight"); float* bff2 = B.f32(b + ".ff.net.2.bias");
            half_t* ck = (half_t*)u->dmalloc((size_t)R * nheads * ck_pad * dp * 2);
            half_t* cvt = (half_t*)u->dmalloc((size_t)R * nheads * dp * ck_pad * 2);
            if (!ck || !cvt || cfgpp_op_attention_prepare_vt(cvt, R * nheads, d, ck_pad, nullptr)) { B.ok = false; B.err = "cross-attention K/V^T allocation failed"; }
            {
                cfgpp_unet* uu = u; const int Dc = c.cross_attention_dim; const int ckp = ck_pad;
                IGemmArgs a = base_args(u);
                a.C0 = Dc; a.amode = 0; a.w = wkv2; a.N = 2 * C; a.K = Dc; a.epi = EPI_HEADS;
                a.hq = nullptr; a.hk = ck; a.hvt = cvt; a.part0 = 1; a.part_width = C; a.head_dim = d; a.head_dim_pad = dp;
                a.heads = nheads; a.tok_pad = ckp; a.q_tok_pad = ckp;
                u->ctx_plan.push_back([a, uu](hipStream_t s, int) mutable {
                    IGemmArgs b2 = a; b2.a0 = uu->ctx_ehs; b2.rows_per_batch = uu->ctx_tokens; b2.M = uu->ctx_rows * uu->ctx_tokens;
                    return igemm_launch(b2, s);
                });
            }
            ++cross_block_counter;
            P.layernorm(u->tok_x, u->tok_ln, l1g, l1b, tok, C);
            P.heads(u->tok_ln, C, wqkv, 3 * C, tok, 0, C, nheads, HQ, HK, HVT, q_pad, k_pad);
            P.attention(HQ, HK, HVT, u->tok_attn, nheads, d, tok, tok, q_pad, k_pad);
            P.linear(u->tok_attn, C, u->tok_x, C, wo1, bo1, u->tok_x, tok);
            P.layernorm(u->tok_x, u->tok_ln, l2g, l2b, tok, C);
            P.heads(u->tok_ln, C, wq2, C, tok, 0, C, nheads, HQ, nullptr, nullptr, q_pad, k_pad);
            if (prefix_from >= 0) {
                u->plan_share.assign(u->plan.size(), 0);
                for (size_t i = (size_t)prefix_from; i < u->plan.size(); ++i) {
                    u->plan_share[i] = 1; ++u->prefix_ops;
                    if (i < u->plan_macs.size()) u->prefix_macs_per_row += u->plan_macs[i];
                }
                half_t* const fp0 = u->tok_x; half_t* const fp1 = HQ; half_t* const fp2 = x.p;
                const long fe0 = (long)tok * C, fe1 = (long)nheads * q_pad * dp, fe2 = (long)(x.H + 2) * (x.W + 2) * C;
                u->plan.push_back([=](hipStream_t s, int h) {
                    if (h <= 0) return 0;
                    half_t* const fp[3] = {fp0, fp1, fp2}; const long fe[3] = {fe0, fe1, fe2};
                    return fanout_rows_launch(fp, fe, 3, h, s);
                });
                u->plan_share.push_back(2);
                u->tag(3, 0.0, "cfg fan-out tok_x + HQ + resid HW=" + std::to_string(tok) + " C=" + std::to_string(C));
                prefix_from = -1;
            }
            {
                cfgpp_unet* uu = u;
                u->attn_macs_per_row += 2.0 * (double)nheads * tok * 77 * d;
                half_t* hq = HQ; half_t* o = u->tok_attn;
                u->plan.push_back([=](hipStream_t s, int rows) {
                    return cfgpp_op_attention(hq, ck, cvt, o, rows, nheads, d, tok, uu->ctx_tokens, q_pad, ck_pad, s);
                });
                u->tag(1, 2.0 * (double)nheads * tok * 77 * d, "cross_attn heads=" + std::to_string(nheads) + " N=" + std::to_string(tok) + " d=" + std::to_string(d));
            }
            P.linear(u->tok_attn, C, u->tok_x, C, wo2, bo2, u->tok_x, tok);
            P.layernorm(u->tok_x, u->tok_ln, l3g, l3b, tok, C);
            P.linear(u->tok_ln, C, u->tok_ff, 8 * C, wff1, bff1, nullptr, tok, EPI_GEGLU);
            P.linear(u->tok_ff, 4 * C, u->tok_x, C, wff2, bff2, u->tok_x, tok);
        }
        Tensor out = u->acq(x.H, x.W, C);
        P.linear_to_padded(u->tok_x, C, out, wpo, bpo, x);
        return out;
    };

    int H = c.sample_h, W = c.sample_w;
    Tensor x = u->acq(H, W, c0);
    {
        HostParam* pw = B.get("conv_in.weight"); HostParam* pb = B.get("conv_in.bias");
        CFGPP_REQUIRE(pw && pb, "finalize: %s", B.err.c_str());
        const int Ci = c.in_channels;
        std::vector<float> r((size_t)9 * Ci * c0);
        for (int o = 0; o < c0; ++o) for (int i = 0; i < Ci; ++i) for (int t = 0; t < 9; ++t)
            r[(size_t)(t * Ci + i) * c0 + o] = pw->f[((size_t)o * Ci + i) * 9 + t];
        float* dw = B.upload(r); float* db = B.upload(pb->f);
        cfgpp_unet* uu = u; half_t* xp = x.p; const int HH = H, WW = W;
        if (u->control) {
            u->d_img_emb = (half_t*)u->dmalloc((size_t)R * (H + 2) * (W + 2) * c0 * sizeof(half_t));
            CFGPP_REQUIRE(u->d_img_emb, "finalize: hipMalloc failed");
            u->plan.push_back([=](hipStream_t s, int rows) {
                return cfgpp_op_conv_in_add(uu->in_z, uu->in_z_half, nullptr, 1, 0, uu->d_img_emb, uu->img_rows, xp, dw, db, rows,
                                            uu->in_z_rows, Ci, HH, WW, c0, s);
            });
        } else if (Ci > c.out_channels) {
            const int Cz = c.out_channels, Cc = Ci - Cz;
            u->d_cond = (half_t*)u->dmalloc((size_t)R * Cc * H * W * sizeof(half_t));
            CFGPP_REQUIRE(u->d_cond, "finalize: hipMalloc failed");
            u->plan.push_back([=](hipStream_t s, int rows) {
                return cfgpp_op_conv_in_cond(uu->in_z, uu->in_z_half, uu->d_cond, uu->cond_rows, Cc, xp, dw, db, rows, uu->in_z_rows, Cz,
                                             HH, WW, c0, s);
            });
        } else {
            u->plan.push_back([=](hipStream_t s, int rows) {
                return cfgpp_op_conv_in(uu->in_z, uu->in_z_half, xp, dw, db, rows, uu->in_z_rows, Ci, HH, WW, c0, s);
            });
        }
    }
    std::vector<Tensor> skips; skips.push_back(x);
    for (int i = 0; i < L; ++i) {
        const int co = c.block_out_channels[i];
        const std::string p = "down_blocks." + std::to_string(i);
        for (int j = 0; j < c.layers_per_block; ++j) {
            if (i == 0 && j == 0 && !per_row_temb && c.level_has_attn[0]) prefix_from = (long)u->plan.size();
            Tensor y = resblock(p + ".resnets." + std::to_string(j), x, nullptr, co);
            if (c.level_has_attn[i]) {
                Tensor z = transformer(p + ".attentions." + std::to_string(j), y, c.transformer_depth[i], c.num_heads[i], i);
                u->rel(y); y = z;
            }
            x = y; skips.push_back(x);
        }
        if (i != L - 1) {
            half_t* wd = B.conv3(p + ".downsamplers.0.conv.weight"); float* bd = B.f32(p + ".downsamplers.0.conv.bias");
            H /= 2; W /= 2;
            Tensor y = u->acq(H, W, co);
            P.conv3x3(x, y, wd, bd, 2, nullptr, 0, nullptr);
            x = y; skips.push_back(x);
        }
    }
    {
        const int cm = c.block_out_channels[L - 1];
        Tensor y = resblock("mid_block.resnets.0", x, nullptr, cm);
        Tensor z = transformer("mid_block.attentions.0", y, c.transformer_depth[L - 1], c.num_heads[L - 1], L - 1);
        u->rel(y);
        Tensor w = resblock("mid_block.resnets.1", z, nullptr, cm);
        u->rel(z);
        x = w;
    }
    if (u->control) {
        int e = controlnet_tail(u, B, P, skips, x);
        if (e) return e;
        skips.clear();
        CFGPP_REQUIRE(B.ok, "finalize: %s", B.err.c_str());
        CFGPP_HIP_CHECK(hipDeviceSynchronize());
        u->plan_kind.resize(u->plan.size(), 3); u->plan_macs.resize(u->plan.size(), 0.0); u->plan_desc.resize(u->plan.size());
        u->plan_share.resize(u->plan.size(), 0);
        u->finalized = true;
        return 0;
    }
    {
        u->ctrl_dst = skips; u->ctrl_dst.push_back(x);
        u->d_ctrl_tab = (CnAddEntry*)u->dmalloc(u->ctrl_dst.size() * sizeof(CnAddEntry));
        CFGPP_REQUIRE(u->d_ctrl_tab, "finalize: hipMalloc failed");
        for (const Tensor& t : u->ctrl_dst) u->ctrl_max_n8 = std::max(u->ctrl_max_n8, (long)R * t.H * t.W * (t.C / 8));
        cfgpp_unet* uu = u;
        const int n = (int)u->ctrl_dst.size();
        u->plan.push_back([uu, n](hipStream_t s, int rows) {
            if (!uu->ctrl || uu->ctrl_scale == 0.f) return 0;
            for (const Tensor& t : uu->ctrl_dst) if (t.gst_ok) *t.gst_ok = 0;
            return cn_residual_add_launch(uu->d_ctrl_tab, n, uu->ctrl_max_n8, rows, uu->ctrl_scale, s);
        });
        u->tag(3, 0.0, "controlnet residual add");
    }
    for (int i = 0; i < L; ++i) {
        const int lvl = L - 1 - i;
        const int co = c.block_out_channels[lvl];
        const std::string p = "up_blocks." + std::to_string(i);
        for (int j = 0; j < c.layers_per_block + 1; ++j) {
            Tensor skip = skips.back(); skips.pop_back();
            Tensor y = resblock(p + ".resnets." + std::to_string(j), x, &skip, co);
            u->rel(x); u->rel(skip);
            if (c.level_has_attn[lvl]) {
                Tensor z = transformer(p + ".attentions." + std::to_string(j), y, c.transformer_depth[lvl], c.num_heads[lvl], lvl);
                u->rel(y); y = z;
            }
            x = y;
        }
        if (i != L - 1) {
            half_t* wu = B.conv3(p + ".upsamplers.0.conv.weight"); float* bu = B.f32(p + ".upsamplers.0.conv.bias");
            H *= 2; W *= 2;
            Tensor y = u->acq(H, W, co);
            P.conv3x3(x, y, wu, bu, 3, nullptr, 0, nullptr);
            u->rel(x); x = y;
        }
    }
    {
        float* g = B.f32("conv_norm_out.weight"); float* b = B.f32("conv_norm_out.bias");
        Tensor gn = u->acq(H, W, c0);
        P.groupnorm(x, nullptr, gn.p, true, g, b, 1e-5f, true);
        HostParam* pw = B.get("conv_out.weight"); float* bo = B.f32("conv_out.bias");
        CFGPP_REQUIRE(pw, "finalize: %s", B.err.c_str());
        const int Co = c.out_channels;
        CFGPP_REQUIRE(Co <= 4, "finalize: out_channels %d > 4 unsupported", Co);
        std::vector<half_t> r((size_t)Co * 9 * c0);
        for (int o = 0; o < Co; ++o) for (int i = 0; i < c0; ++i) for (int t = 0; t < 9; ++t)
            r[((size_t)o * 9 + t) * c0 + i] = pw->h[((size_t)o * c0 + i) * 9 + t];
        half_t* dw = B.upload(r);
        cfgpp_unet* uu = u; half_t* gp = gn.p; const int HH = H, WW = W;
        u->macs_per_row += (double)H * W * Co * 9.0 * c0 + (double)c.sample_h * c.sample_w * c0 * 9.0 * c.in_channels;
        u->plan.push_back([=](hipStream_t s, int rows) { return cfgpp_op_conv_out(gp, uu->out_eps, 1, dw, bo, rows, HH, WW, c0, Co, s); });
    }
    CFGPP_REQUIRE(B.ok, "finalize: %s", B.err.c_str());
    CFGPP_REQUIRE(skips.empty(), "finalize: internal error, %d skips left", (int)skips.size());
    CFGPP_HIP_CHECK(hipDeviceSynchronize());
    u->plan_kind.resize(u->plan.size(), 3); u->plan_macs.resize(u->plan.size(), 0.0); u->plan_desc.resize(u->plan.size());
    u->plan_share.resize(u->plan.size(), 0);
    u->finalized = true;
    return 0;
}

int cfgpp_unet_set_context(cfgpp_unet* u, const void* ehs, int rows, int tokens, const void* text_embeds,
                           const void* time_ids, int cond_rows, void* stream) {
    CFGPP_REQUIRE(u && u->finalized, "set_context: context not finalized");
    CFGPP_REQUIRE(ehs && rows > 0 && rows <= u->cfg.max_rows, "set_context: rows=%d (max %d)", rows, u->cfg.max_rows);
    CFGPP_REQUIRE(tokens == 77, "set_context: tokens=%d (the engine is built for 77 text tokens)", tokens);
    if (u->cfg.addition_embed) {
        CFGPP_REQUIRE(text_embeds && time_ids, "set_context: SDXL needs text_embeds and time_ids");
        CFGPP_REQUIRE(cond_rows == rows || cond_rows == 1, "set_context: cond_rows=%d must be rows (%d) or 1", cond_rows, rows);
    }
    u->ctx_ehs = (const half_t*)ehs; u->ctx_rows = rows; u->ctx_tokens = tokens;
    u->ctx_text = (const half_t*)text_embeds; u->ctx_tids = (const float*)time_ids; u->ctx_cond_rows = cond_rows;
    for (auto& op : u->ctx_plan) { int e = op((hipStream_t)stream, rows); if (e) return e; }
    u->ctx_set = true;
    return 0;
}

int cfgpp_unet_image_condition(cfgpp_unet* u, const void* cond, int cond_rows, void* stream) {
    CFGPP_REQUIRE(u && u->finalized, "image_condition: engine not finalized");
    if (u->control) {
        CFGPP_REQUIRE(cond && cond_rows > 0 && cond_rows <= u->cfg.max_rows, "image_condition: ControlNet image_rows=%d (1 .. %d)", cond_rows,
                      u->cfg.max_rows);
        u->img_in = cond; u->img_in_half = 1;
        for (auto& op : u->img_plan) { int e = op((hipStream_t)stream, cond_rows); if (e) return e; }
        u->img_in = nullptr;
        u->img_rows = cond_rows;
        return 0;
    }
    CFGPP_REQUIRE(u->cfg.in_channels > u->cfg.out_channels && u->d_cond,
                  "image_condition: this UNet takes %d input channels for %d latent channels - no image condition (not an inpaint UNet)",
                  u->cfg.in_channels, u->cfg.out_channels);
    CFGPP_REQUIRE(cond && cond_rows > 0 && cond_rows <= u->cfg.max_rows, "image_condition: cond_rows=%d (1 .. %d)", cond_rows, u->cfg.max_rows);
    const size_t bytes = (size_t)cond_rows * (u->cfg.in_channels - u->cfg.out_channels) * u->cfg.sample_h * u->cfg.sample_w * sizeof(half_t);
    CFGPP_HIP_CHECK(hipMemcpyAsync(u->d_cond, cond, bytes, hipMemcpyDeviceToDevice, (hipStream_t)stream));
    u->cond_rows = cond_rows;
    return 0;
}

int cfgpp_unet_attach_control(cfgpp_unet* u, cfgpp_unet* cn, float scale) {
    CFGPP_REQUIRE(u && u->finalized, "attach_control: UNet not finalized");
    CFGPP_REQUIRE(!u->control, "attach_control: the target is itself a ControlNet");
    if (!cn) { u->ctrl = nullptr; u->ctrl_scale = 0.f; return 0; }
    CFGPP_REQUIRE(cn->finalized && cn->control, "attach_control: not a finalized ControlNet (cfgpp_unet_create with out_channels = 0, then finalize)");
    const cfgpp_unet_config &a = u->cfg, &b = cn->cfg;
    CFGPP_REQUIRE(a.num_levels == b.num_levels && a.layers_per_block == b.layers_per_block, "attach_control: levels %d x %d vs the UNet's %d x %d",
                  b.num_levels, b.layers_per_block, a.num_levels, a.layers_per_block);
    for (int i = 0; i < a.num_levels; ++i)
        CFGPP_REQUIRE(a.block_out_channels[i] == b.block_out_channels[i], "attach_control: channels of level %d: %d vs the UNet's %d", i,
                      b.block_out_channels[i], a.block_out_channels[i]);
    CFGPP_REQUIRE(a.sample_h == b.sample_h && a.sample_w == b.sample_w, "attach_control: latent %d x %d vs the UNet's %d x %d", b.sample_h,
                  b.sample_w, a.sample_h, a.sample_w);
    CFGPP_REQUIRE(a.max_rows == b.max_rows, "attach_control: max_rows %d vs the UNet's %d", b.max_rows, a.max_rows);
    CFGPP_REQUIRE(b.in_channels == a.out_channels, "attach_control: the ControlNet takes %d latent channels, the UNet %d", b.in_channels,
                  a.out_channels);
    CFGPP_REQUIRE(cn->ctrl_res.size() == u->ctrl_dst.size(), "attach_control: %d residuals for %d skip connections + mid block",
                  (int)cn->ctrl_res.size(), (int)u->ctrl_dst.size());
    std::vector<CnAddEntry> tab(u->ctrl_dst.size());
    for (size_t i = 0; i < tab.size(); ++i) {
        const Tensor &d = u->ctrl_dst[i], &r = cn->ctrl_res[i];
        CFGPP_REQUIRE(d.H == r.H && d.W == r.W && d.C == r.C, "attach_control: residual %d is %d x %d x %d, the UNet tensor %d x %d x %d", (int)i,
                      r.H, r.W, r.C, d.H, d.W, d.C);
        tab[i] = CnAddEntry{d.p, r.p, d.H, d.W, d.C, 0};
    }
    CFGPP_HIP_CHECK(hipSetDevice(u->device));
    CFGPP_HIP_CHECK(hipDeviceSynchronize());
    CFGPP_HIP_CHECK(hipMemcpy(u->d_ctrl_tab, tab.data(), tab.size() * sizeof(CnAddEntry), hipMemcpyHostToDevice));
    u->ctrl = cn; u->ctrl_scale = scale;
    return 0;
}

int cfgpp_controlnet_residual(cfgpp_unet* cn, int i, float scale, float* out, int rows, int* hwc_out, void* stream) {
    CFGPP_REQUIRE(cn && cn->finalized && cn->control, "controlnet_residual: not a finalized ControlNet");
    const int n = (int)cn->ctrl_res.size();
    if (!out && !hwc_out) return n;
    CFGPP_REQUIRE(i >= 0 && i < n, "controlnet_residual: index %d (0 .. %d)", i, n - 1);
    const Tensor& r = cn->ctrl_res[i];
    if (hwc_out) { hwc_out[0] = r.H; hwc_out[1] = r.W; hwc_out[2] = r.C; }
    if (!out) return n;
    CFGPP_REQUIRE(rows > 0 && rows <= cn->cfg.max_rows, "controlnet_residual: rows=%d", rows);
    int e = cfgpp_op_residual_nchw(r.p, out, rows, r.H, r.W, r.C, scale, stream);
    return e ? e : n;
}

int cfgpp_unet_forward(cfgpp_unet* u, const void* z, int z_is_half, int z_rows, float t, void* eps_out, int rows,
                       void* stream) {
    CFGPP_REQUIRE(u && u->finalized, "forward: context not finalized");
    CFGPP_REQUIRE(u->ctx_set, "forward: set_context has not been called");
    CFGPP_REQUIRE(z && eps_out && z_rows > 0 && rows > 0 && rows <= u->cfg.max_rows, "forward: bad args (rows=%d max=%d)", rows, u->cfg.max_rows);
    CFGPP_REQUIRE(rows == u->ctx_rows, "forward: rows=%d but context was set for %d rows", rows, u->ctx_rows);
    CFGPP_REQUIRE(u->control || u->cfg.in_channels == u->cfg.out_channels || (u->cond_rows > 0 && (u->cond_rows == 1 || u->cond_rows == z_rows)),
                  "forward: inpaint UNet (%d input channels) needs cfgpp_unet_image_condition with 1 or z_rows=%d rows first (has %d)",
                  u->cfg.in_channels, z_rows, u->cond_rows);
    CFGPP_REQUIRE(!u->control || u->img_rows > 0, "forward: ControlNet without a control image (call cfgpp_unet_image_condition first)");
    if (u->ctrl && u->ctrl_scale != 0.f) {
        cfgpp_unet* cn = u->ctrl;
        CFGPP_REQUIRE(cn->img_rows > 0, "forward: a ControlNet is attached but has no control image (cfgpp_unet_image_condition)");
        CFGPP_REQUIRE(cn->ctx_set && cn->ctx_rows == rows, "forward: the attached ControlNet's context is set for %d rows, the forward runs %d",
                      cn->ctx_set ? cn->ctx_rows : 0, rows);
        int e = cfgpp_unet_forward(cn, z, z_is_half, z_rows, t, eps_out, rows, stream);
        if (e) return e;
    }
    u->in_z = z; u->in_z_half = z_is_half; u->in_z_rows = z_rows; u->in_t = t; u->in_t_dev = nullptr; u->out_eps = eps_out;
    const bool shared = u->enter_call(rows, z_rows);
    if ((u->tuned_rows != rows || u->tuned_shared != shared) && igemm_autotune_enabled()) {
        int e = u->tune_plan((hipStream_t)stream, rows, shared); if (e) return e;
        ++u->tuned_serial;
    }
    for (size_t i = 0; i < u->plan.size(); ++i) { int e = u->plan[i]((hipStream_t)stream, u->rows_for(i, rows, shared)); if (e) return e; }
    return 0;
}

int cfgpp_sample_graph_ddim(cfgpp_unet* u, void* z, void* z0t, int z_is_half, int z_rows, void* eps, const void* eps_uc,
                            const void* eps_c, int rows, const float* host_steps, int n_steps, float lam, int tweedie_uc,
                            int renoise_uc, void* stream) {
    CFGPP_REQUIRE(u && u->finalized && u->ctx_set, "sample_graph: context not ready");
    CFGPP_REQUIRE(z && z0t && eps && eps_uc && eps_c && host_steps && n_steps > 0 && z_rows > 0, "sample_graph: bad args");
    CFGPP_REQUIRE(rows == u->ctx_rows && rows <= u->cfg.max_rows, "sample_graph: rows=%d but context was set for %d rows", rows, u->ctx_rows);
    CFGPP_REQUIRE(!u->ctrl && !u->control, "sample_graph: a ControlNet is attached (a controlled step is not captured): detach it "
                                            "(cfgpp_unet_attach_control(u, NULL, 0)) or run the eager loop");
    hipStream_t s = (hipStream_t)stream;
    CFGPP_REQUIRE(u->cfg.in_channels == u->cfg.out_channels || (u->cond_rows > 0 && (u->cond_rows == 1 || u->cond_rows == z_rows)),
                  "sample_graph: inpaint UNet (%d input channels) needs cfgpp_unet_image_condition with 1 or z_rows=%d rows first (has %d)",
                  u->cfg.in_channels, z_rows, u->cond_rows);
    const long n = (long)z_rows * u->cfg.out_channels * u->cfg.sample_h * u->cfg.sample_w;
    if (!u->d_step_cur) {
        u->d_step_cur = (float*)u->dmalloc(8 * sizeof(float));
        u->d_step_idx = (int*)u->dmalloc(sizeof(int));
        CFGPP_REQUIRE(u->d_step_cur && u->d_step_idx, "sample_graph: out of device memory");
        CFGPP_HIP_CHECK(hipStreamCreateWithFlags(&u->cap_stream, hipStreamNonBlocking));
    }
    if (n_steps > u->step_tab_cap) {
        u->drop_graphs();
        const int cap = n_steps < 64 ? 64 : n_steps;
        u->d_step_tab = (float*)u->dmalloc((size_t)cap * 8 * sizeof(float));
        CFGPP_REQUIRE(u->d_step_tab, "sample_graph: out of device memory");
        u->step_tab_cap = cap;
    }
    u->enter_call(rows, z_rows);
    const cfgpp_unet::GraphKey want{z, z0t, eps, eps_uc, eps_c, z_is_half, z_rows, rows, tweedie_uc, renoise_uc, lam, n, 0, u->cond_rows};
    auto same = [&](const cfgpp_unet::GraphKey& k) {
        return k.z == want.z && k.z0t == want.z0t && k.eps == want.eps && k.euc == want.euc && k.ec == want.ec && k.z_half == want.z_half &&
               k.z_rows == want.z_rows && k.rows == want.rows && k.tw == want.tw && k.rn == want.rn && k.lam == want.lam && k.n == want.n &&
               k.tuned_serial == u->tuned_serial && k.cond_rows == want.cond_rows;
    };
    int hit = -1;
    for (size_t i = 0; i < u->graphs.size(); ++i) if (same(u->graphs[i].key)) hit = (int)i;
    if (hit < 0) {
        int e = cfgpp_unet_forward(u, z, z_is_half, z_rows, host_steps[0], eps, rows, stream);
        if (e) return e;
        CFGPP_HIP_CHECK(hipStreamSynchronize(s));
        for (size_t i = 0; i < u->graphs.size();)
            if (u->graphs[i].key.tuned_serial != u->tuned_serial) { cfgpp_unet::destroy(u->graphs[i]); u->graphs.erase(u->graphs.begin() + i); } else ++i;
        cfgpp_unet::Graph g{want, nullptr, nullptr};
        g.key.tuned_serial = u->tuned_serial;
        u->in_t_dev = u->d_step_cur;
        hipError_t he = hipStreamBeginCapture(u->cap_stream, hipStreamCaptureModeRelaxed);
        int rc = 0;
        if (he == hipSuccess) {
            rc = step_advance_launch(u->d_step_tab, u->d_step_idx, u->d_step_cur, u->cap_stream);
            const bool shared = u->shares(rows, z_rows);
            for (size_t i = 0; i < u->plan.size() && rc == 0; ++i) rc = u->plan[i](u->cap_stream, u->rows_for(i, rows, shared));
            if (rc == 0) rc = step_ddim_dev_launch(z, z0t, eps_uc, eps_c, 1, z_is_half, lam, u->d_step_cur + 1, tweedie_uc, renoise_uc, n, u->cap_stream);
            he = hipStreamEndCapture(u->cap_stream, &g.graph);
        }
        u->in_t_dev = nullptr;
        if (he != hipSuccess || rc != 0 || !g.graph) {
            cfgpp_unet::destroy(g);
            if (rc == 0) cfgpp_set_error("sample_graph: stream capture failed: %s", hipGetErrorString(he));
            return rc ? rc : -1;
        }
        he = hipGraphInstantiate(&g.exec, g.graph, nullptr, nullptr, 0);
        if (he != hipSuccess) { cfgpp_unet::destroy(g); cfgpp_set_error("sample_graph: hipGraphInstantiate: %s", hipGetErrorString(he)); return -1; }
        if (u->graphs.size() >= 4) { cfgpp_unet::destroy(u->graphs.front()); u->graphs.erase(u->graphs.begin()); }
        u->graphs.push_back(g);
        hit = (int)u->graphs.size() - 1;
    }
    if (hit != (int)u->graphs.size() - 1) std::swap(u->graphs[hit], u->graphs.back());
    hipGraphExec_t exec = u->graphs.back().exec;
    std::vector<float> tab((size_t)n_steps * 8, 0.f);
    for (int i = 0; i < n_steps; ++i) for (int k = 0; k < 5; ++k) tab[(size_t)i * 8 + k] = host_steps[(size_t)i * 5 + k];
    CFGPP_HIP_CHECK(hipMemcpyAsync(u->d_step_tab, tab.data(), tab.size() * sizeof(float), hipMemcpyHostToDevice, s));
    CFGPP_HIP_CHECK(hipStreamSynchronize(s));
    CFGPP_HIP_CHECK(hipMemsetAsync(u->d_step_idx, 0, sizeof(int), s));
    for (int i = 0; i < n_steps; ++i) CFGPP_HIP_CHECK(hipGraphLaunch(exec, s));
    return 0;
}

int cfgpp_unet_profile(cfgpp_unet* u, const void* z, int z_is_half, int z_rows, float t, void* eps_out, int rows,
                       void* stream, double* out_ms, double* out_flops, int* out_launches, char* detail, long detail_cap) {
    CFGPP_REQUIRE(u && u->finalized && u->ctx_set, "profile: context not ready");
    CFGPP_REQUIRE(z && eps_out && out_ms && out_flops && out_launches && rows == u->ctx_rows, "profile: bad args");
    u->in_z = z; u->in_z_half = z_is_half; u->in_z_rows = z_rows; u->in_t = t; u->out_eps = eps_out;
    hipStream_t s = (hipStream_t)stream;
    const size_t n = u->plan.size();
    const bool shared = u->enter_call(rows, z_rows);
    std::vector<int> op_rows(n);
    for (size_t i = 0; i < n; ++i) op_rows[i] = u->rows_for(i, rows, shared);
    std::vector<hipEvent_t> ev(n + 1);
    for (auto& e : ev) CFGPP_HIP_CHECK(hipEventCreate(&e));
    CFGPP_HIP_CHECK(hipEventRecord(ev[0], s));
    int rc = 0;
    for (size_t i = 0; i < n && rc == 0; ++i) { rc = u->plan[i](s, op_rows[i]); if (rc == 0 && hipEventRecord(ev[i + 1], s) != hipSuccess) rc = -1; }
    if (rc == 0 && hipStreamSynchronize(s) != hipSuccess) rc = -1;
    for (int k = 0; k < 4; ++k) { out_ms[k] = 0; out_flops[k] = 0; out_launches[k] = 0; }
    if (rc == 0) {
        for (size_t i = 0; i < n; ++i) {
            if (op_rows[i] == 0) continue;
            float ms = 0.f; hipEventElapsedTime(&ms, ev[i], ev[i + 1]);
            const int k = u->plan_kind[i];
            out_ms[k] += ms; out_flops[k] += 2.0 * u->plan_macs[i] * op_rows[i]; out_launches[k] += 1;
        }
        if (detail && detail_cap > 0) {
            std::string txt;
            for (size_t i = 0; i < n; ++i) {
                if (op_rows[i] == 0) continue;
                float ms = 0.f; hipEventElapsedTime(&ms, ev[i], ev[i + 1]);
                char line[256];
                const std::string desc = u->plan_desc[i] + (op_rows[i] != rows ? " rows=" + std::to_string(op_rows[i]) : std::string());
                snprintf(line, sizeof(line), "%zu\t%d\t%s\t%.1f\t%.3f\n", i, u->plan_kind[i], desc.c_str(), ms * 1e3,
                         2.0 * u->plan_macs[i] * op_rows[i] * 1e-9);
                txt += line;
            }
            const long ncopy = std::min<long>((long)txt.size(), detail_cap - 1);
            std::memcpy(detail, txt.data(), ncopy); detail[ncopy] = 0;
        }
    }
    for (auto& e : ev) hipEventDestroy(e);
    return rc;
}

int cfgpp_unet_tuning(cfgpp_unet* u, int rows, int* hints, int cap, int set) {
    CFGPP_REQUIRE(u && u->finalized && hints && rows > 0, "unet_tuning: bad args");
    const int n = (int)u->cfg_hints.size();
    CFGPP_REQUIRE(cap >= n, "unet_tuning: buffer of %d for %d launches", cap, n);
    if (set) {
        for (int sh = 0; sh < 2; ++sh) u->tuned_by_rows[std::make_pair(rows, sh != 0)] = std::vector<int>(hints, hints + n);
        if (u->tuned_rows == rows) u->tuned_rows = 0;
        ++u->tuned_serial;
        return n;
    }
    auto it = u->tuned_by_rows.find(std::make_pair(rows, u->ran_shared == 1));
    if (it == u->tuned_by_rows.end()) { cfgpp_set_error("unet_tuning: batch %d has not been tuned", rows); return -3; }
    std::copy(it->second.begin(), it->second.end(), hints);
    return n;
}

double cfgpp_unet_flops(cfgpp_unet* u, int rows) {
    if (!u || !u->finalized) return 0.0;
    const double once = u->ran_shared == 1 ? u->prefix_macs_per_row * (rows / 2) : 0.0;
    return 2.0 * ((u->macs_per_row + u->attn_macs_per_row) * rows - once);
}

void cfgpp_unet_set_share_prefix(int on) { g_share_prefix = on ? 1 : 0; }
int cfgpp_unet_share_prefix_enabled(void) { return g_share_prefix; }
int cfgpp_unet_shared_prefix_ops(cfgpp_unet* u, int rows, int z_rows) {
    if (!u || !u->finalized) return 0;
    return u->shares(rows, z_rows) ? u->prefix_ops : 0;
}
double cfgpp_unet_device_bytes(cfgpp_unet* u) { return u ? u->dev_bytes : 0.0; }

static float* g_op_gstat = nullptr;
static int g_op_gstat_flag = 0;
void cfgpp_op_igemm_set_gstat(void* buf) { g_op_gstat = (float*)buf; }
int cfgpp_op_igemm_gstat_written() { return g_op_gstat_flag; }

int cfgpp_op_igemm(const void* a0, const void* a1, int C0, int C1, int taps, int amode, int H, int W,
                   const void* w, int M, int N, const float* bias, const float* temb, int temb_ld,
                   const void* resid, int rmode, int rld, void* out, int omode, int old_, int epi, void* stream) {
    IGemmArgs a = base_args();
    a.a0 = (const half_t*)a0; a.a1 = (const half_t*)a1; a.C0 = C0; a.C1 = C1; a.taps = taps; a.amode = amode; a.H = H; a.W = W;
    a.w = (const half_t*)w; a.M = M; a.N = N; a.K = taps * (C0 + C1); a.bias = bias; a.temb = temb; a.temb_ld = temb_ld;
    a.rows_per_batch = H * W; a.resid = (const half_t*)resid; a.rmode = rmode; a.rld = rld;
    a.out = (half_t*)out; a.omode = omode; a.old = old_; a.epi = epi;
    a.gstat = g_op_gstat; a.stat_flag = &g_op_gstat_flag; g_op_gstat_flag = 0;
    return igemm_launch(a, (hipStream_t)stream);
}

int cfgpp_op_igemm_heads(const void* a_, int K, const void* w, int M, int N, const float* bias, int rows_per_batch,
                         void* hq, void* hk, void* hvt, int part0, int part_width, int head_dim, int heads,
                         int q_tok_pad, int tok_pad, void* stream) {
    IGemmArgs a = base_args();
    a.a0 = (const half_t*)a_; a.C0 = K; a.amode = 0; a.w = (const half_t*)w; a.M = M; a.N = N; a.K = K; a.bias = bias;
    a.epi = EPI_HEADS; a.rows_per_batch = rows_per_batch; a.hq = (half_t*)hq; a.hk = (half_t*)hk; a.hvt = (half_t*)hvt;
    a.part0 = part0; a.part_width = part_width; a.head_dim = head_dim; a.head_dim_pad = round_up(head_dim, 32);
    a.heads = heads; a.q_tok_pad = q_tok_pad; a.tok_pad = tok_pad;
    return igemm_launch(a, (hipStream_t)stream);
}

}
```

cfgpp_amd/engine.py:

```python
from __future__ import annotations

import ctypes as C
from typing import Dict, Iterable, Optional, Tuple

import torch

from . import _lib
from ._lib import CfgppError, UNetConfigC, check
from .unet_config import UNetConfig


def _require_cuda(t: torch.Tensor, name: str):
    if not t.is_cuda:
        raise CfgppError(f"{name} must live on the GPU (got {t.device}); the HIP path has no CPU fallback")
    if not t.is_contiguous():
        raise CfgppError(f"{name} must be contiguous")


def _stream_ptr(t: Optional[torch.Tensor] = None) -> int:
    if t is not None and t.is_cuda:
        return torch.cuda.current_stream(t.device).cuda_stream
    return torch.cuda.current_stream().cuda_stream


def _ptr(t: Optional[torch.Tensor]) -> Optional[int]:
    return None if t is None else t.data_ptr()


def step_ddim(z: torch.Tensor, z0t_out: torch.Tensor, eps_uc: torch.Tensor, eps_c: torch.Tensor,
              lam: float, coeffs: Tuple[float, float, float, float], tweedie_uc: bool, renoise_uc: bool):
    lib = _lib.load()
    for n, t in (("z", z), ("z0t_out", z0t_out), ("eps_uc", eps_uc), ("eps_c", eps_c)):
        _require_cuda(t, n)
    if z.dtype != z0t_out.dtype or z.dtype not in (torch.float16, torch.float32):
        raise CfgppError("step_ddim: z and z0t_out must both be fp32 or both fp16")
    if eps_uc.dtype != eps_c.dtype or eps_uc.dtype not in (torch.float16, torch.float32):
        raise CfgppError("step_ddim: eps must both be fp16 or both fp32")
    if not (z.numel() == z0t_out.numel() == eps_uc.numel() == eps_c.numel()):
        raise CfgppError("step_ddim: size mismatch")
    c1, c2, c3, c4 = (float(x) for x in coeffs)
    if z.dtype == torch.float16:
        if eps_uc.dtype != torch.float16:
            raise CfgppError("step_ddim: an fp16 latent needs fp16 eps")
        check(lib.cfgpp_step_ddim_h(z.data_ptr(), z0t_out.data_ptr(), eps_uc.data_ptr(), eps_c.data_ptr(), float(lam),
                                    c1, c2, c3, c4, int(bool(tweedie_uc)), int(bool(renoise_uc)), z.numel(), _stream_ptr(z)),
              "cfgpp_step_ddim_h")
        return
    check(lib.cfgpp_step_ddim(z.data_ptr(), z0t_out.data_ptr(), eps_uc.data_ptr(), eps_c.data_ptr(),
                              1 if eps_uc.dtype == torch.float16 else 0, float(lam), c1, c2, c3, c4,
                              int(bool(tweedie_uc)), int(bool(renoise_uc)), z.numel(), _stream_ptr(z)),
          "cfgpp_step_ddim")


def step_ddim_masked(z: torch.Tensor, z0t_out: torch.Tensor, eps_uc: torch.Tensor, eps_c: torch.Tensor, lam: float,
                     coeffs: Tuple[float, float, float, float], tweedie_uc: bool, renoise_uc: bool, mask: torch.Tensor,
                     src: torch.Tensor, noise: torch.Tensor, a: float, b: float):
    lib = _lib.load()
    for n, t in (("z", z), ("z0t_out", z0t_out), ("eps_uc", eps_uc), ("eps_c", eps_c), ("mask", mask), ("src", src),
                 ("noise", noise)):
        _require_cuda(t, n)
    if z.dtype != torch.float32 or z0t_out.dtype != torch.float32 or noise.dtype != torch.float32:
        raise CfgppError("step_ddim_masked: z, z0t_out and noise must be fp32")
    if eps_uc.dtype != torch.float16 or eps_c.dtype != torch.float16 or src.dtype != torch.float16:
        raise CfgppError("step_ddim_masked: eps and src must be fp16")
    if mask.dtype not in (torch.bool, torch.uint8):
        raise CfgppError("step_ddim_masked: mask must be bool or uint8 (binarized)")
    if z.dim() != 4 or tuple(z.shape[1:2]) != (4,):
        raise CfgppError(f"step_ddim_masked: z shape {tuple(z.shape)} is not [B, 4, h, w]")
    B, hw = int(z.shape[0]), int(z.shape[2]) * int(z.shape[3])
    for n, t in (("z0t_out", z0t_out), ("eps_uc", eps_uc), ("eps_c", eps_c), ("src", src), ("noise", noise)):
        if tuple(t.shape) != tuple(z.shape):
            raise CfgppError(f"step_ddim_masked: {n} shape {tuple(t.shape)} != z shape {tuple(z.shape)}")
    if mask.numel() != B * hw:
        raise CfgppError(f"step_ddim_masked: mask has {mask.numel()} elements for B={B} x hw={hw}")
    c1, c2, c3, c4 = (float(x) for x in coeffs)
    check(lib.cfgpp_step_ddim_masked(z.data_ptr(), z0t_out.data_ptr(), eps_uc.data_ptr(), eps_c.data_ptr(), float(lam), c1, c2, c3, c4,
                                     int(bool(tweedie_uc)), int(bool(renoise_uc)), mask.data_ptr(), src.data_ptr(), noise.data_ptr(),
                                     float(a), float(b), B, hw, _stream_ptr(z)), "cfgpp_step_ddim_masked")


def kdiff_input(x: torch.Tensor, xc_out: torch.Tensor, s: float, mode: int):
    lib = _lib.load()
    _require_cuda(x, "x")
    _require_cuda(xc_out, "xc_out")
    if x.dtype != torch.float16 or xc_out.dtype != torch.float16:
        raise CfgppError("kdiff_input: fp16 latents expected")
    check(lib.cfgpp_kdiff_input(x.data_ptr(), xc_out.data_ptr(), float(s), int(mode), x.numel(), _stream_ptr(x)),
          "cfgpp_kdiff_input")


def step_kdiff(x: torch.Tensor, den_out: torch.Tensor, old: Optional[torch.Tensor], eps_uc: torch.Tensor,
               eps_c: torch.Tensor, coef9, variant: int, xl_form: bool, euler_branch: bool, write_old: bool):
    lib = _lib.load()
    for n, t in (("x", x), ("den_out", den_out), ("eps_uc", eps_uc), ("eps_c", eps_c)):
        _require_cuda(t, n)
        if t.dtype != torch.float16:
            raise CfgppError(f"step_kdiff: {n} must be fp16")
    if old is not None:
        _require_cuda(old, "old")
    arr = (C.c_float * 9)(*[float(v) for v in coef9])
    check(lib.cfgpp_step_kdiff(x.data_ptr(), den_out.data_ptr(), _ptr(old), eps_uc.data_ptr(), eps_c.data_ptr(),
                               arr, int(variant), int(bool(xl_form)), int(bool(euler_branch)), int(bool(write_old)),
                               x.numel(), _stream_ptr(x)), "cfgpp_step_kdiff")


def kdiff_denoise(x, eps_uc, eps_c, lam: float, sigma: float, den_out, uden_out):
    lib = _lib.load()
    for n, t in (("x", x), ("eps_uc", eps_uc), ("eps_c", eps_c), ("den_out", den_out), ("uden_out", uden_out)):
        _require_cuda(t, n)
        if t.dtype != torch.float16:
            raise CfgppError(f"kdiff_denoise: {n} must be fp16")
    check(lib.cfgpp_kdiff_denoise(x.data_ptr(), eps_uc.data_ptr(), eps_c.data_ptr(), float(lam), float(sigma),
                                  den_out.data_ptr(), uden_out.data_ptr(), x.numel(), _stream_ptr(x)), "cfgpp_kdiff_denoise")


def lincomb(out, x, y, z, a: float, b: float, mode: int):
    lib = _lib.load()
    for n, t in (("out", out), ("x", x), ("y", y)) + ((("z", z),) if z is not None else ()):
        _require_cuda(t, n)
        if t.dtype != torch.float16:
            raise CfgppError(f"lincomb: {n} must be fp16")
    check(lib.cfgpp_lincomb(out.data_ptr(), x.data_ptr(), y.data_ptr(), _ptr(z), float(a), float(b), int(mode), x.numel(),
                            _stream_ptr(x)), "cfgpp_lincomb")


def unet_config_c(cfg: UNetConfig, H: int, W: int, max_rows: int, out_channels: Optional[int] = None) -> UNetConfigC:
    cc = UNetConfigC()
    cc.in_channels = cfg.in_channels
    cc.out_channels = cfg.out_channels if out_channels is None else int(out_channels)
    cc.num_levels = cfg.num_levels
    for i in range(cfg.num_levels):
        cc.block_out_channels[i] = cfg.block_out_channels[i]
        cc.level_has_attn[i] = cfg.level_has_attn[i]
        cc.transformer_depth[i] = cfg.transformer_depth[i]
        cc.num_heads[i] = cfg.num_heads[i]
    cc.layers_per_block = cfg.layers_per_block
    cc.cross_attention_dim = cfg.cross_attention_dim
    cc.addition_embed = cfg.addition_embed
    cc.addition_time_embed_dim = cfg.addition_time_embed_dim
    cc.addition_pooled_dim = cfg.addition_pooled_dim
    cc.norm_groups = cfg.norm_groups
    cc.sample_h, cc.sample_w = int(H), int(W)
    cc.max_rows = int(max_rows)
    return cc


class HipUNet:

    def __init__(self, cfg: UNetConfig, max_rows: int, sample_hw: Optional[Tuple[int, int]] = None,
                 device: int = 0):
        self.lib = _lib.load()
        if not torch.cuda.is_available():
            raise CfgppError("HipUNet needs a ROCm GPU (torch.cuda.is_available() is False); "
                             "there is no CPU fallback for the HIP path")
        self.cfg = cfg
        self.device = int(device)
        self.max_rows = int(max_rows)
        H, W = sample_hw if sample_hw is not None else (cfg.sample_size, cfg.sample_size)
        self.H, self.W = int(H), int(W)
        cc = unet_config_c(cfg, self.H, self.W, self.max_rows)
        self._h = self.lib.cfgpp_unet_create(C.byref(cc), self.device)
        if not self._h:
            raise CfgppError("cfgpp_unet_create failed: " + _lib.last_error())
        self._keep = {}
        self.finalized = False
        self.latent_channels = cfg.out_channels
        self.cond_channels = cfg.in_channels - cfg.out_channels

    def __del__(self):
        h = getattr(self, "_h", None)
        if h:
            try:
                torch.cuda.synchronize()
            except Exception:
                pass
            self.lib.cfgpp_unet_destroy(h)
            self._h = None

    def load_tensor(self, key: str, t: torch.Tensor):
        t = t.detach().cpu().contiguous()
        if t.dtype == torch.float16:
            dt = 1
        else:
            t = t.to(torch.float32)
            dt = 0
        shape = (C.c_long * t.dim())(*t.shape)
        check(self.lib.cfgpp_unet_load_tensor(self._h, key.encode(), t.data_ptr(), dt, shape, t.dim()),
              f"cfgpp_unet_load_tensor({key})")

    def load_state_dict(self, items: Iterable[Tuple[str, torch.Tensor]]):
        if isinstance(items, dict):
            items = items.items()
        for k, v in items:
            self.load_tensor(k, v)
        return self

    def finalize(self):
        check(self.lib.cfgpp_unet_finalize(self._h), "cfgpp_unet_finalize")
        self.finalized = True
        return self

    def set_context(self, ehs: torch.Tensor, text_embeds: Optional[torch.Tensor] = None,
                    time_ids: Optional[torch.Tensor] = None):
        dev = torch.device("cuda", self.device)
        ehs = ehs.to(device=dev, dtype=torch.float16).contiguous()
        rows, tokens = int(ehs.shape[0]), int(ehs.shape[1])
        te = ti = None
        cond_rows = 0
        if self.cfg.addition_embed:
            if text_embeds is None or time_ids is None:
                raise CfgppError("set_context: SDXL needs text_embeds and time_ids")
            te = text_embeds.to(device=dev, dtype=torch.float16).contiguous()
            ti = time_ids.to(device=dev, dtype=torch.float32).contiguous()
            cond_rows = int(te.shape[0])
            if int(ti.shape[0]) != cond_rows:
                raise CfgppError("set_context: text_embeds / time_ids row mismatch")
        self._keep["ctx"] = (ehs, te, ti)
        self.rows = rows
        check(self.lib.cfgpp_unet_set_context(self._h, ehs.data_ptr(), rows, tokens, _ptr(te), _ptr(ti), cond_rows,
                                              _stream_ptr(ehs)), "cfgpp_unet_set_context")

    def image_condition(self, cond: torch.Tensor):
        if self.cond_channels <= 0:
            raise CfgppError(f"image_condition: {self.cfg.name} takes no image condition (in_channels == out_channels)")
        dev = torch.device("cuda", self.device)
        cond = cond.to(device=dev, dtype=torch.float16).contiguous()
        if cond.dim() != 4 or tuple(cond.shape[1:]) != (self.cond_channels, self.H, self.W):
            raise CfgppError(f"image_condition: cond shape {tuple(cond.shape)} != [*, {self.cond_channels}, {self.H}, {self.W}]")
        check(self.lib.cfgpp_unet_image_condition(self._h, cond.data_ptr(), int(cond.shape[0]), _stream_ptr(cond)),
              "cfgpp_unet_image_condition")
        self._keep["cond"] = cond

    def forward(self, z: torch.Tensor, t: float, eps_out: Optional[torch.Tensor] = None) -> torch.Tensor:
        _require_cuda(z, "z")
        if z.dtype not in (torch.float16, torch.float32):
            raise CfgppError("forward: z must be fp16 or fp32")
        zr = int(z.shape[0])
        if tuple(z.shape[1:]) != (self.latent_channels, self.H, self.W):
            raise CfgppError(f"forward: z shape {tuple(z.shape)} != [*, {self.latent_channels}, {self.H}, {self.W}]")
        rows = self.rows
        if rows % zr != 0:
            raise CfgppError(f"forward: rows={rows} is not a multiple of z rows={zr}")
        if eps_out is None:
            eps_out = torch.empty((rows, self.cfg.out_channels, self.H, self.W), dtype=torch.float16, device=z.device)
        check(self.lib.cfgpp_unet_forward(self._h, z.data_ptr(), 1 if z.dtype == torch.float16 else 0, zr, float(t),
                                          eps_out.data_ptr(), rows, _stream_ptr(z)), "cfgpp_unet_forward")
        return eps_out

    def attach_control(self, cn, scale: float):
        check(self.lib.cfgpp_unet_attach_control(self._h, None if cn is None else cn._h, float(scale)), "cfgpp_unet_attach_control")
        self._keep["control"] = cn

    def sample_graph_ddim(self, z: torch.Tensor, z0t: torch.Tensor, eps: torch.Tensor, eps_uc: torch.Tensor, eps_c: torch.Tensor,
                          steps, lam: float, tweedie_uc: bool, renoise_uc: bool):
        for n, t in (("z", z), ("z0t", z0t), ("eps", eps)):
            _require_cuda(t, n)
        if z.dtype != z0t.dtype or z.dtype not in (torch.float16, torch.float32) or eps.dtype != torch.float16:
            raise CfgppError("sample_graph_ddim: z / z0t must both be fp32 or both fp16, eps fp16")
        if tuple(z.shape[1:]) != (self.latent_channels, self.H, self.W) or z.shape != z0t.shape:
            raise CfgppError(f"sample_graph_ddim: z shape {tuple(z.shape)}")
        if int(eps.shape[0]) != self.rows or self.rows % int(z.shape[0]) != 0:
            raise CfgppError(f"sample_graph_ddim: eps rows {int(eps.shape[0])} / z rows {int(z.shape[0])} vs context rows {self.rows}")
        flat = [float(v) for st in steps for v in st]
        if len(flat) != 5 * len(steps) or not steps:
            raise CfgppError("sample_graph_ddim: steps must be a non-empty list of (t, c1, c2, c3, c4)")
        arr = (C.c_float * len(flat))(*flat)
        check(self.lib.cfgpp_sample_graph_ddim(self._h, z.data_ptr(), z0t.data_ptr(), 1 if z.dtype == torch.float16 else 0, int(z.shape[0]),
                                               eps.data_ptr(), eps_uc.data_ptr(), eps_c.data_ptr(), self.rows, arr, len(steps), float(lam),
                                               int(bool(tweedie_uc)), int(bool(renoise_uc)), _stream_ptr(z)), "cfgpp_sample_graph_ddim")

    def profile(self, z: torch.Tensor, t: float, detail: bool = False) -> dict:
        _require_cuda(z, "z")
        rows = self.rows
        eps = torch.empty((rows, self.cfg.out_channels, self.H, self.W), dtype=torch.float16, device=z.device)
        ms, fl, ln = (C.c_double * 4)(), (C.c_double * 4)(), (C.c_int * 4)()
        buf = C.create_string_buffer(1 << 20) if detail else None
        check(self.lib.cfgpp_unet_profile(self._h, z.data_ptr(), 1 if z.dtype == torch.float16 else 0, int(z.shape[0]),
                                          float(t), eps.data_ptr(), rows, _stream_ptr(z), ms, fl, ln, buf, (1 << 20) if detail else 0),
              "cfgpp_unet_profile")
        names = ("igemm", "attention", "norm", "small")
        out = {n: dict(ms=ms[i], flops=fl[i], launches=ln[i]) for i, n in enumerate(names)}
        if detail:
            out["detail"] = buf.value.decode()
        return out

    def export_tuning(self, rows: Optional[int] = None):
        rows = self.rows if rows is None else int(rows)
        buf = (C.c_int * 4096)()
        n = self.lib.cfgpp_unet_tuning(self._h, rows, buf, 4096, 0)
        if n < 0:
            raise CfgppError("cfgpp_unet_tuning: " + _lib.last_error())
        return [int(buf[i]) for i in range(n)]

    def import_tuning(self, hints, rows: int):
        buf = (C.c_int * len(hints))(*[int(h) for h in hints])
        n = self.lib.cfgpp_unet_tuning(self._h, int(rows), buf, len(hints), 1)
        if n < 0:
            raise CfgppError("cfgpp_unet_tuning: " + _lib.last_error())

    def flops(self, rows: int) -> float:
        return float(self.lib.cfgpp_unet_flops(self._h, int(rows)))

    def shared_prefix_ops(self, rows: int, z_rows: int) -> int:
        return int(self.lib.cfgpp_unet_shared_prefix_ops(self._h, int(rows), int(z_rows)))

    def device_bytes(self) -> float:
        return float(self.lib.cfgpp_unet_device_bytes(self._h))


def set_share_prefix(on: bool):
    _lib.load().cfgpp_unet_set_share_prefix(1 if on else 0)


def share_prefix_enabled() -> bool:
    return bool(_lib.load().cfgpp_unet_share_prefix_enabled())
```

cfgpp_amd/hip_engine.py:

```python
from __future__ import annotations

import os
from typing import Optional, Tuple

import torch

from . import engine as E
from . import _lib
from ._lib import CfgppError
from .tune_cache import PinCache, build_id
from .unet_config import CONFIGS, UNetConfig
from .weights import load_safetensors_iter, synth_state_dict_iter


class HipEngine:

    def __init__(self, cfg: UNetConfig, max_batch: int = 1, latent_hw: Optional[Tuple[int, int]] = None,
                 device=None, weights="synthetic", weight_seed: int = 0):
        if isinstance(cfg, str):
            cfg = CONFIGS[cfg]
        if not torch.cuda.is_available():
            raise CfgppError("HipEngine needs a ROCm GPU; the HIP path has no CPU fallback")
        dev = torch.device(device if device is not None else "cuda")
        if dev.type != "cuda":
            raise CfgppError(f"HipEngine cannot run on device '{dev}': the HIP path has no CPU fallback")
        self.device = torch.device("cuda", dev.index if dev.index is not None else torch.cuda.current_device())
        self.cfg = cfg
        self.max_batch = int(max_batch)
        torch.cuda.set_device(self.device)
        self.unet = E.HipUNet(cfg, max_rows=2 * self.max_batch, sample_hw=latent_hw, device=self.device.index)
        if weights == "synthetic":
            items = synth_state_dict_iter(cfg, weight_seed)
        elif isinstance(weights, str):
            items = load_safetensors_iter(weights)
        else:
            items = weights.items() if isinstance(weights, dict) else weights
        self.unet.load_state_dict(items).finalize()
        self.H, self.W = self.unet.H, self.unet.W
        self._pins = PinCache(getattr(cfg, "name", type(cfg).__name__), (self.H, self.W), torch.cuda.get_device_properties(self.device).name,
                              build_id(_lib.LIB_PATH), lambda rows: self.unet.export_tuning(rows), lambda h, rows: self.unet.import_tuning(h, rows),
                              knobs=lambda: (int(self.unet.lib.cfgpp_igemm_tuner_state()),),
                              mode=lambda rows: "shared" if self.unet.shared_prefix_ops(rows, rows // 2) else "")
        self._ctx_key = None
        self._ctx = None
        self._control = None
        self._eps = None
        self._g_buf = None
        self.check_finite = os.environ.get("CFGPP_CHECK_FINITE", "0") not in ("", "0")

    def _finite_or_raise(self, t):
        if not bool(torch.isfinite(self._eps).all()):
            bad = int((~torch.isfinite(self._eps)).sum())
            raise CfgppError(f"UNet output at t={t} holds {bad} non-finite values (fp16 overflow inside the UNet?) - CFGPP_CHECK_FINITE")

    def set_context(self, uc: torch.Tensor, c: torch.Tensor, text_embeds=None, time_ids=None):
        B = max(int(uc.shape[0]), int(c.shape[0]))
        if B > self.max_batch:
            raise CfgppError(f"batch {B} exceeds engine max_batch {self.max_batch}")
        if uc.shape[0] != B:
            uc = uc.expand(B, -1, -1)
        if c.shape[0] != B:
            c = c.expand(B, -1, -1)
        ehs = torch.cat([uc, c], dim=0)
        self.unet.set_context(ehs, text_embeds, time_ids)
        self._ctx = (ehs, text_embeds, time_ids)
        if self._control is not None:
            self._control[0].set_context(ehs, text_embeds, time_ids)
        self._pins.load(2 * B)
        self.B = B
        if self._eps is None or int(self._eps.shape[0]) != 2 * B:
            self._eps = torch.empty((2 * B, self.cfg.out_channels, self.H, self.W), dtype=torch.float16, device=self.device)

    def image_condition(self, cond: torch.Tensor):
        self.unet.image_condition(cond)

    def set_control(self, cn, image: torch.Tensor, scale: float = 1.0):
        cn.set_image(image)
        if self._ctx is not None:
            cn.set_context(*self._ctx)
        self.unet.attach_control(cn, float(scale))
        self._control = (cn, float(scale))

    def clear_control(self):
        if self._control is not None:
            self.unet.attach_control(None, 0.0)
        self._control = None

    def build_controlnet(self, spec, seed: int = 0):
        from .controlnet import build_controlnet
        return build_controlnet(spec, self.cfg, 2 * self.max_batch, (self.H, self.W), self.device.index, seed)

    @property
    def control(self):
        return self._control

    def predict(self, z: torch.Tensor, t: float):
        eps = self.unet.forward(z, float(t), self._eps)
        self._pins.save(self.unet.rows)
        if self.check_finite:
            self._finite_or_raise(t)
        return eps[: self.B], eps[self.B:]

    @property
    def graph_enabled(self) -> bool:
        return os.environ.get("CFGPP_GRAPH", "0") not in ("", "0") and self._control is None

    def ddim_loop_graph(self, zt: torch.Tensor, steps, lam: float, tweedie_uc: bool, renoise_uc: bool, single: str = ""):
        key = (int(zt.shape[0]), zt.dtype)
        if self._g_buf is None or self._g_buf[0] != key:
            self._g_buf = (key, torch.empty_like(zt), torch.empty_like(zt))
        _, gz, gz0 = self._g_buf
        gz.copy_(zt)
        eps = self._eps
        euc, ec = eps[: self.B], eps[self.B:]
        if single == "uc":
            ec = euc
        elif single == "c":
            euc = ec
        self.unet.sample_graph_ddim(gz, gz0, eps, euc, ec, steps, lam, tweedie_uc, renoise_uc)
        self._pins.save(self.unet.rows)
        if self.check_finite:
            self._finite_or_raise(steps[-1][0])
        return gz0.clone(), gz.clone()

    def export_tuning(self):
        return self.unet.export_tuning(self.unet.rows)

    def import_tuning(self, hints, batch: int):
        self.unet.import_tuning(hints, 2 * int(batch))
        self._pins.mark_imported(2 * int(batch))

    def device_bytes(self) -> float:
        return self.unet.device_bytes()

    step_ddim = staticmethod(E.step_ddim)
    step_ddim_masked = staticmethod(E.step_ddim_masked)
    kdiff_input = staticmethod(E.kdiff_input)
    step_kdiff = staticmethod(E.step_kdiff)
    kdiff_denoise = staticmethod(E.kdiff_denoise)
    lincomb = staticmethod(E.lincomb)

    def randn_like(self, x):
        return torch.randn_like(x)

    def flops_per_forward(self, rows: int) -> float:
        return self.unet.flops(rows)
```

Baseline: 9.091 images/sec.

## Fuse cross-attention Q projection into the attention kernel

Adds a new HIP kernel that computes the cross-attention query projection (x·Wq) on the fly and feeds it straight into the softmax(QK)V computation against the 77-token context. The separate Q heads GEMM and the write and read of the HQ buffer are dropped per transformer block. The plan gains fuse markers so the unfused or fused ops are skipped per mode, and the autotuning cache is keyed by a shared/fused mode. When the shared prefix is active it wraps the batch so one copy of x serves both CFG halves. The risk is that the fused kernel may not beat the tuned GEMM plus attention at some head dims, and it enlarges the plan and tuning state.

```diff
diff --git a/cfgpp_amd/_lib.py b/cfgpp_amd/_lib.py
--- a/cfgpp_amd/_lib.py
+++ b/cfgpp_amd/_lib.py
@@ -87,6 +87,12 @@
     "cfgpp_unet_set_share_prefix": (None, [_I]),
     "cfgpp_unet_share_prefix_enabled": (_I, []),
     "cfgpp_unet_shared_prefix_ops": (_I, [_P, _I, _I]),
+    "cfgpp_unet_set_fuse_xattn": (None, [_I]),
+    "cfgpp_unet_fuse_xattn_enabled": (_I, []),
+    "cfgpp_unet_fused_xattn_sites": (_I, [_P]),
+    "cfgpp_xattn_fused_supported": (_I, [_I, _I, _I, _I]),
+    "cfgpp_xattn_fused_preferred": (_I, [_I, _I, _I, _I]),
+    "cfgpp_op_xattn_fused": (_I, [_P, _P, _P, _P, _P, _I, _I, _I, _I, _I, _I, _I, _I, _P]),
     "cfgpp_op_layernorm": (_I, [_P, _P, _P, _P, _L, _I, _F, _P]),
     "cfgpp_op_attention_prepare_vt": (_I, [_P, _I, _I, _I, _P]),
     "cfgpp_op_attention": (_I, [_P, _P, _P, _P, _I, _I, _I, _I, _I, _I, _I, _P]),
diff --git a/cfgpp_amd/build.py b/cfgpp_amd/build.py
--- a/cfgpp_amd/build.py
+++ b/cfgpp_amd/build.py
@@ -20,6 +20,7 @@
     ("big4_kernel.hip", []),
     ("big4p_kernel.hip", []),
     ("attn_kernel.hip", ["-mllvm", "-amdgpu-mfma-vgpr-form=1"]),
+    ("xattn_fused_kernel.hip", ["-mllvm", "-amdgpu-mfma-vgpr-form=1"]),
     ("controlnet_kernels.hip", ["-ffp-contract=off"]),
     ("unet.hip", []),
     ("vae.hip", []),
diff --git a/cfgpp_amd/csrc/attn_kernel.hip b/cfgpp_amd/csrc/attn_kernel.hip
--- a/cfgpp_amd/csrc/attn_kernel.hip
+++ b/cfgpp_amd/csrc/attn_kernel.hip
@@ -2,7 +2,7 @@
 
 namespace {
 
-constexpr float RESCALE_THR = 5.0f;
+constexpr float RESCALE_THR = CFGPP_ATTN_RESCALE_THR;
 
 struct AttnArgs {
     const half_t* q; const half_t* k; const half_t* vt;
diff --git a/cfgpp_amd/csrc/cfgpp_debug.h b/cfgpp_amd/csrc/cfgpp_debug.h
--- a/cfgpp_amd/csrc/cfgpp_debug.h
+++ b/cfgpp_amd/csrc/cfgpp_debug.h
@@ -21,6 +21,9 @@
 void cfgpp_unet_set_share_prefix(int on);
 int cfgpp_unet_share_prefix_enabled(void);
 int cfgpp_unet_shared_prefix_ops(cfgpp_unet* u, int rows, int z_rows);
+void cfgpp_unet_set_fuse_xattn(int on);
+int cfgpp_unet_fuse_xattn_enabled(void);
+int cfgpp_unet_fused_xattn_sites(cfgpp_unet* u);
 void cfgpp_groupnorm_set_mode(int mode);
 int cfgpp_op_layernorm(const void* x, void* y, const float* gamma, const float* beta, long rows, int C,
                        float eps, void* stream);
@@ -31,6 +34,10 @@
 void cfgpp_attention_set_dma(int mode);
 void cfgpp_attention_set_stagger(int sleeps);
 void cfgpp_attention_set_cross(int on);
+int cfgpp_xattn_fused_supported(int heads, int d, int C, int nk);
+int cfgpp_xattn_fused_preferred(int heads, int d, int C, int nk);
+int cfgpp_op_xattn_fused(const void* x, const void* wq, const void* k, const void* vt, void* o, int B, int heads, int d, int C,
+                         int nq, int nk, int k_tok_pad, int wrap, void* stream);
 int cfgpp_op_conv_in(const void* z, int z_is_half, void* out, const float* w, const float* bias,
                      int R, int zB, int Cin, int H, int W, int Cout, void* stream);
 int cfgpp_op_conv_in_cond(const void* z, int z_is_half, const void* cond, int cond_rows, int Cc, void* out, const float* w,
diff --git a/cfgpp_amd/csrc/common.h b/cfgpp_amd/csrc/common.h
--- a/cfgpp_amd/csrc/common.h
+++ b/cfgpp_amd/csrc/common.h
@@ -54,6 +54,10 @@
 __host__ __device__ __forceinline__ int cfgpp_vt_pos(int tok) {
     return (tok & ~12) | ((tok & 4) << 1) | ((tok & 8) >> 1);
 }
+
+__host__ __device__ __forceinline__ int cfgpp_q_row(int m) { return cfgpp_vt_pos(m); }
+
+constexpr float CFGPP_ATTN_RESCALE_THR = 5.0f;
 
 __device__ __forceinline__ float silu_f(float x) { return x / (1.0f + __expf(-x)); }
 __device__ __forceinline__ float gelu_erf_f(float x) {
diff --git a/cfgpp_amd/csrc/engine_base.h b/cfgpp_amd/csrc/engine_base.h
--- a/cfgpp_amd/csrc/engine_base.h
+++ b/cfgpp_amd/csrc/engine_base.h
@@ -49,7 +49,12 @@
     std::vector<double> plan_macs;
     std::vector<std::string> plan_desc;
     std::vector<char> plan_share;
+    std::vector<char> plan_fuse;
+    bool fused = false;
+    void mark_fuse(char m) { plan_fuse.resize(plan.size(), 0); if (!plan.empty()) plan_fuse.back() = m; }
     int rows_for(size_t i, int rows, bool shared) const {
+        const int f = i < plan_fuse.size() ? plan_fuse[i] : 0;
+        if (f != 0 && (f == 2) != fused) return 0;
         const int m = i < plan_share.size() ? plan_share[i] : 0;
         if (m == 0) return rows;
         return shared ? rows / 2 : (m == 1 ? rows : 0);
@@ -62,7 +67,9 @@
     std::vector<int*> plan_hint;
     int tuned_rows = 0;
     bool tuned_shared = false;
-    std::map<std::pair<int, bool>, std::vector<int>> tuned_by_rows;
+    bool tuned_fused = false;
+    std::map<std::pair<int, int>, std::vector<int>> tuned_by_rows;
+    static int plan_mode(bool shared, bool fused_) { return (shared ? 1 : 0) | (fused_ ? 2 : 0); }
     int* new_hint(bool in_main_plan) {
         cfg_hints.push_back(0);
         int* h = &cfg_hints.back();
@@ -70,12 +77,12 @@
         return h;
     }
     int tune_plan(hipStream_t s, int rows, bool shared = false) {
-        const auto key = std::make_pair(rows, shared);
+        const auto key = std::make_pair(rows, plan_mode(shared, fused));
         auto cached = tuned_by_rows.find(key);
         if (cached != tuned_by_rows.end() && cached->second.size() == cfg_hints.size()) {
             size_t k = 0;
             for (int& h : cfg_hints) h = cached->second[k++];
-            tuned_rows = rows; tuned_shared = shared;
+            tuned_rows = rows; tuned_shared = shared; tuned_fused = fused;
             return 0;
         }
         static const int cands[] = {0, 1, 4, 5, 6, 7, 8, 9, 10, 11, 12, 13, 14, 15, 16, 17, 20, 24, 25, 26, 27, 28};
@@ -128,7 +135,7 @@
         for (size_t i = 0; i < n; ++i) if (plan_hint[i]) *plan_hint[i] = bestc[i];
         for (auto& e : ev) hipEventDestroy(e);
         if (rc == 0) tuned_by_rows[key] = std::vector<int>(cfg_hints.begin(), cfg_hints.end());
-        tuned_rows = rows; tuned_shared = shared;
+        tuned_rows = rows; tuned_shared = shared; tuned_fused = fused;
         return rc;
     }
     std::map<std::tuple<int, int, int>, std::vector<std::pair<half_t*, float*>>> pool;
@@ -345,7 +352,10 @@
         a.head_dim = d; a.head_dim_pad = round_up(d, 32); a.heads = nheads; a.tok_pad = tok_pad; a.q_tok_pad = q_tok_pad;
         if (count) u->macs_per_row += (double)tokens * N * K;
         int* hint = u->new_hint(ops == &u->plan);
-        ops->push_back([a, tokens, hint](hipStream_t s, int rows) mutable { IGemmArgs b = a; b.M = rows * tokens; b.cfg_hint = *hint; return igemm_launch(b, s); });
+        ops->push_back([a, tokens, hint](hipStream_t s, int rows) mutable {
+            if (rows <= 0) return 0;
+            IGemmArgs b = a; b.M = rows * tokens; b.cfg_hint = *hint; return igemm_launch(b, s);
+        });
         if (ops == &u->plan) u->tag(0, count ? (double)tokens * N * K : 0.0, "heads HW=" + std::to_string(tokens) + " N=" + std::to_string(N) + " K=" + std::to_string(K));
     }
     void groupnorm(const Tensor& s0, const Tensor* s1, half_t* dst, bool dst_padded, const float* g, const float* b,
diff --git a/cfgpp_amd/csrc/unet.hip b/cfgpp_amd/csrc/unet.hip
--- a/cfgpp_amd/csrc/unet.hip
+++ b/cfgpp_amd/csrc/unet.hip
@@ -18,10 +18,14 @@
     int prefix_ops = 0;
     double prefix_macs_per_row = 0;
     int ran_shared = -1;
+    int ran_fused = -1;
+    int fuse_sites = 0;
     bool shares(int rows, int z_rows) const;
     bool enter_call(int rows, int z_rows) {
         const bool sh = shares(rows, z_rows);
-        if (ran_shared != (int)sh) { if (ran_shared >= 0) ++tuned_serial; ran_shared = (int)sh; }
+        const int fu = cfgpp_unet_fuse_xattn_enabled();
+        if (ran_shared != (int)sh || ran_fused != fu) { if (ran_shared >= 0) ++tuned_serial; ran_shared = (int)sh; ran_fused = fu; }
+        fused = fu != 0;
         return sh;
     }
     static void destroy(Graph& g) { if (g.exec) hipGraphExecDestroy(g.exec); if (g.graph) hipGraphDestroy(g.graph); g.exec = nullptr; g.graph = nullptr; }
@@ -51,6 +55,7 @@
 };
 
 static int g_share_prefix = 1;
+static int g_fuse_xattn = 1;
 bool cfgpp_unet::shares(int rows, int z_rows) const { return g_share_prefix && prefix_ops > 0 && rows == 2 * z_rows; }
 
 namespace {
@@ -475,7 +480,10 @@
             P.attention(HQ, HK, HVT, u->tok_attn, nheads, d, tok, tok, q_pad, k_pad);
             P.linear(u->tok_attn, C, u->tok_x, C, wo1, bo1, u->tok_x, tok);
             P.layernorm(u->tok_x, u->tok_ln, l2g, l2b, tok, C);
+            const bool can_fuse = cfgpp_xattn_fused_supported(nheads, d, C, u->ctx_tokens) != 0;
+            const bool ends_prefix = prefix_from >= 0;
             P.heads(u->tok_ln, C, wq2, C, tok, 0, C, nheads, HQ, nullptr, nullptr, q_pad, k_pad);
+            if (can_fuse) { u->mark_fuse(1); ++u->fuse_sites; }
             if (prefix_from >= 0) {
                 u->plan_share.assign(u->plan.size(), 0);
                 for (size_t i = (size_t)prefix_from; i < u->plan.size(); ++i) {
@@ -484,8 +492,10 @@
                 }
                 half_t* const fp0 = u->tok_x; half_t* const fp1 = HQ; half_t* const fp2 = x.p;
                 const long fe0 = (long)tok * C, fe1 = (long)nheads * q_pad * dp, fe2 = (long)(x.H + 2) * (x.W + 2) * C;
+                cfgpp_unet* uf = u;
                 u->plan.push_back([=](hipStream_t s, int h) {
                     if (h <= 0) return 0;
+                    if (can_fuse && uf->fused) { half_t* const fp[2] = {fp0, fp2}; const long fe[2] = {fe0, fe2}; return fanout_rows_launch(fp, fe, 2, h, s); }
                     half_t* const fp[3] = {fp0, fp1, fp2}; const long fe[3] = {fe0, fe1, fe2};
                     return fanout_rows_launch(fp, fe, 3, h, s);
                 });
@@ -498,9 +508,22 @@
                 u->attn_macs_per_row += 2.0 * (double)nheads * tok * 77 * d;
                 half_t* hq = HQ; half_t* o = u->tok_attn;
                 u->plan.push_back([=](hipStream_t s, int rows) {
+                    if (rows <= 0) return 0;
                     return cfgpp_op_attention(hq, ck, cvt, o, rows, nheads, d, tok, uu->ctx_tokens, q_pad, ck_pad, s);
                 });
                 u->tag(1, 2.0 * (double)nheads * tok * 77 * d, "cross_attn heads=" + std::to_string(nheads) + " N=" + std::to_string(tok) + " d=" + std::to_string(d));
+                if (can_fuse) {
+                    u->mark_fuse(1);
+                    const half_t* xin = u->tok_ln;
+                    u->plan.push_back([=](hipStream_t s, int rows) {
+                        if (rows <= 0) return 0;
+                        const int wrap = ends_prefix && uu->ran_shared == 1 ? rows / 2 : rows;
+                        return cfgpp_op_xattn_fused(xin, wq2, ck, cvt, o, rows, nheads, d, C, tok, uu->ctx_tokens, ck_pad, wrap, s);
+                    });
+                    u->tag(1, (double)tok * C * C + 2.0 * (double)nheads * tok * 77 * d,
+                           "xattn_q heads=" + std::to_string(nheads) + " N=" + std::to_string(tok) + " d=" + std::to_string(d) + " C=" + std::to_string(C));
+                    u->mark_fuse(2);
+                }
             }
             P.linear(u->tok_attn, C, u->tok_x, C, wo2, bo2, u->tok_x, tok);
             P.layernorm(u->tok_x, u->tok_ln, l3g, l3b, tok, C);
@@ -581,7 +604,7 @@
         CFGPP_REQUIRE(B.ok, "finalize: %s", B.err.c_str());
         CFGPP_HIP_CHECK(hipDeviceSynchronize());
         u->plan_kind.resize(u->plan.size(), 3); u->plan_macs.resize(u->plan.size(), 0.0); u->plan_desc.resize(u->plan.size());
-        u->plan_share.resize(u->plan.size(), 0);
+        u->plan_share.resize(u->plan.size(), 0); u->plan_fuse.resize(u->plan.size(), 0);
         u->finalized = true;
         return 0;
     }
@@ -641,7 +664,7 @@
     CFGPP_REQUIRE(skips.empty(), "finalize: internal error, %d skips left", (int)skips.size());
     CFGPP_HIP_CHECK(hipDeviceSynchronize());
     u->plan_kind.resize(u->plan.size(), 3); u->plan_macs.resize(u->plan.size(), 0.0); u->plan_desc.resize(u->plan.size());
-    u->plan_share.resize(u->plan.size(), 0);
+    u->plan_share.resize(u->plan.size(), 0); u->plan_fuse.resize(u->plan.size(), 0);
     u->finalized = true;
     return 0;
 }
@@ -748,7 +771,7 @@
     }
     u->in_z = z; u->in_z_half = z_is_half; u->in_z_rows = z_rows; u->in_t = t; u->in_t_dev = nullptr; u->out_eps = eps_out;
     const bool shared = u->enter_call(rows, z_rows);
-    if ((u->tuned_rows != rows || u->tuned_shared != shared) && igemm_autotune_enabled()) {
+    if ((u->tuned_rows != rows || u->tuned_shared != shared || u->tuned_fused != u->fused) && igemm_autotune_enabled()) {
         int e = u->tune_plan((hipStream_t)stream, rows, shared); if (e) return e;
         ++u->tuned_serial;
     }
@@ -880,12 +903,12 @@
     const int n = (int)u->cfg_hints.size();
     CFGPP_REQUIRE(cap >= n, "unet_tuning: buffer of %d for %d launches", cap, n);
     if (set) {
-        for (int sh = 0; sh < 2; ++sh) u->tuned_by_rows[std::make_pair(rows, sh != 0)] = std::vector<int>(hints, hints + n);
+        for (int mode = 0; mode < 4; ++mode) u->tuned_by_rows[std::make_pair(rows, mode)] = std::vector<int>(hints, hints + n);
         if (u->tuned_rows == rows) u->tuned_rows = 0;
         ++u->tuned_serial;
         return n;
     }
-    auto it = u->tuned_by_rows.find(std::make_pair(rows, u->ran_shared == 1));
+    auto it = u->tuned_by_rows.find(std::make_pair(rows, EngineBase::plan_mode(u->ran_shared == 1, u->ran_fused == 1)));
     if (it == u->tuned_by_rows.end()) { cfgpp_set_error("unet_tuning: batch %d has not been tuned", rows); return -3; }
     std::copy(it->second.begin(), it->second.end(), hints);
     return n;
@@ -901,8 +924,15 @@
 int cfgpp_unet_share_prefix_enabled(void) { return g_share_prefix; }
 int cfgpp_unet_shared_prefix_ops(cfgpp_unet* u, int rows, int z_rows) {
     if (!u || !u->finalized) return 0;
-    return u->shares(rows, z_rows) ? u->prefix_ops : 0;
-}
+    if (!u->shares(rows, z_rows)) return 0;
+    int n = 0;
+    for (size_t i = 0; i < u->plan_share.size(); ++i)
+        if (u->plan_share[i] == 1 && !(g_fuse_xattn && i < u->plan_fuse.size() && u->plan_fuse[i] == 1)) ++n;
+    return n;
+}
+void cfgpp_unet_set_fuse_xattn(int on) { g_fuse_xattn = on ? 1 : 0; }
+int cfgpp_unet_fuse_xattn_enabled(void) { return g_fuse_xattn; }
+int cfgpp_unet_fused_xattn_sites(cfgpp_unet* u) { return u && u->finalized && g_fuse_xattn ? u->fuse_sites : 0; }
 double cfgpp_unet_device_bytes(cfgpp_unet* u) { return u ? u->dev_bytes : 0.0; }
 
 static float* g_op_gstat = nullptr;
diff --git a/cfgpp_amd/csrc/xattn_fused_kernel.hip b/cfgpp_amd/csrc/xattn_fused_kernel.hip
--- /dev/null
+++ b/cfgpp_amd/csrc/xattn_fused_kernel.hip
@@ -0,0 +1,396 @@
+#include "common.h"
+
+namespace {
+
+struct XFusedArgs {
+    const half_t* x; const half_t* wq; const half_t* k; const half_t* vt;
+    half_t* o;
+    int heads, d, C;
+    int nq, nk_valid;
+    int k_tok_pad;
+    int o_ld;
+    int xqb, nxb;
+    int wrap;
+    float scale_log2e;
+};
+
+template <int DT, int D16, bool ONES, bool FLASH>
+__global__ void __launch_bounds__(256)
+xattn_fused_kernel(const XFusedArgs a) {
+    constexpr int DP = DT * 32;
+    constexpr int KPITCH = DP * 2 + 16;
+    constexpr int WTILE = DP * 128;
+    constexpr int PPW = DT;
+    constexpr int NST = 2;
+    extern __shared__ __attribute__((aligned(16))) char smem[];
+
+    const int tid = threadIdx.x, lane = tid & 63;
+    const int wid = __builtin_amdgcn_readfirstlane(tid >> 6);
+    const int l31 = lane & 31, hi = lane >> 5;
+    const int nsub = (a.nk_valid + 31) >> 5;
+    const int VPITCH = nsub * 64 + 16;
+    char* const Ksm = smem + NST * WTILE;
+    char* const Vsm = Ksm + nsub * 32 * KPITCH;
+
+    int b, xb, head;
+    {
+        const int T = gridDim.x, bid = blockIdx.x;
+        const int q = T >> 3, r = T & 7, xcd = bid & 7, idx = bid >> 3;
+        const int w = (xcd < r ? xcd * (q + 1) : r * (q + 1) + (xcd - r) * q) + idx;
+        const int t = w / a.heads;
+        head = w - t * a.heads; b = t / a.nxb; xb = t - b * a.nxb;
+    }
+    const int bh = b * a.heads + head;
+    const half_t* Xb = a.x + (long)(b % a.wrap) * a.nq * a.C;
+    const half_t* Wh = a.wq + (long)head * a.d * a.C;
+    const half_t* Kb = a.k + (long)bh * a.k_tok_pad * DP;
+    const half_t* Vb = a.vt + (long)bh * DP * a.k_tok_pad;
+
+    int woff[PPW];
+    {
+        const int r8 = lane >> 3, pc = lane & 7;
+#pragma unroll
+        for (int h = 0; h < PPW; ++h) {
+            const int row = (wid * PPW + h) * 8 + r8;
+            const int lc = pc ^ ((row >> 1) & 7);
+            woff[h] = (row < a.d ? row : a.d - 1) * a.C + lc * 8;
+        }
+    }
+    auto dma_w = [&](int kt, int stage) {
+        const half_t* Wt = Wh + kt * 64;
+#pragma unroll
+        for (int h = 0; h < PPW; ++h)
+            __builtin_amdgcn_global_load_lds((const __attribute__((address_space(1))) void*)(Wt + woff[h]),
+                                             (__attribute__((address_space(3))) void*)(smem + stage * WTILE + (wid * PPW + h) * 8 * 128), 16, 0, 0);
+    };
+    const int qbase = xb * a.xqb * 128 + wid * 32 + l31;
+    half8_t xn[4];
+    auto load_x = [&](half8_t (&dst)[4], int blk, int kt) {
+        const int q = qbase + blk * 128;
+        const half_t* p = Xb + (long)(q < a.nq ? q : a.nq - 1) * a.C + kt * 64 + hi * 8;
+#pragma unroll
+        for (int ks = 0; ks < 4; ++ks) dst[ks] = *reinterpret_cast<const half8_t*>(p + ks * 16);
+    };
+
+    const int KT = a.C >> 6;
+    const int total = a.xqb * KT;
+    dma_w(0, 0);
+    load_x(xn, 0, 0);
+    for (int c = tid; c < nsub * 32 * (DP / 8); c += 256) {
+        const int kr = c / (DP / 8), kc = c - kr * (DP / 8);
+        *reinterpret_cast<half8_t*>(Ksm + kr * KPITCH + kc * 16) = *reinterpret_cast<const half8_t*>(Kb + (long)kr * DP + kc * 8);
+    }
+    for (int c = tid; c < DP * nsub * 4; c += 256) {
+        const int vr = c / (nsub * 4), vc = c - vr * (nsub * 4);
+        *reinterpret_cast<half8_t*>(Vsm + vr * VPITCH + vc * 16) = *reinterpret_cast<const half8_t*>(Vb + (long)vr * a.k_tok_pad + vc * 8);
+    }
+    __syncthreads();
+
+    const int pm = cfgpp_q_row(l31);
+    const int fsw = (pm >> 1) & 7;
+    const int frow = pm * 128;
+    f32x16 acc[DT];
+#pragma unroll
+    for (int i = 0; i < DT; ++i)
+#pragma unroll
+        for (int r = 0; r < 16; ++r) acc[i][r] = 0.f;
+
+    int kt = 0, blk = 0;
+    for (int g = 0; g < total; ++g) {
+        half8_t xc[4];
+#pragma unroll
+        for (int ks = 0; ks < 4; ++ks) xc[ks] = xn[ks];
+        asm volatile("s_waitcnt vmcnt(0)" ::: "memory");
+        __builtin_amdgcn_s_barrier();
+        asm volatile("" ::: "memory");
+        int ktn = kt + 1, blkn = blk;
+        if (ktn == KT) { ktn = 0; ++blkn; }
+        if (g + 1 < total) { dma_w(ktn, (g + 1) & 1); load_x(xn, blkn, ktn); }
+        const char* Ws = smem + (g & 1) * WTILE;
+#pragma unroll
+        for (int ks = 0; ks < 4; ++ks)
+#pragma unroll
+            for (int i = 0; i < DT; ++i) {
+                const half8_t wf = *reinterpret_cast<const half8_t*>(Ws + i * 32 * 128 + frow + ((((ks << 1) | hi) ^ fsw) << 4));
+                acc[i] = __builtin_amdgcn_mfma_f32_32x32x16_f16(wf, xc[ks], acc[i], 0, 0, 0);
+            }
+        if (kt == KT - 1) {
+            half8_t qs[D16];
+#pragma unroll
+            for (int ks = 0; ks < D16; ++ks)
+#pragma unroll
+                for (int j = 0; j < 8; ++j)
+                    qs[ks][j] = (half_t)((float)(half_t)acc[ks >> 1][8 * (ks & 1) + j] * a.scale_log2e);
+            float psum = 0.f;
+            if constexpr (!FLASH) {
+                f32x16 s[4];
+#pragma unroll
+                for (int st = 0; st < 4; ++st) {
+#pragma unroll
+                    for (int r = 0; r < 16; ++r) s[st][r] = 0.f;
+                    if (st < nsub) {
+                        const char* Ks = Ksm + (st * 32 + l31) * KPITCH + hi * 16;
+#pragma unroll
+                        for (int ks = 0; ks < D16; ++ks) {
+                            const half8_t kf = *reinterpret_cast<const half8_t*>(Ks + ks * 32);
+                            s[st] = __builtin_amdgcn_mfma_f32_32x32x16_f16(kf, qs[ks], s[st], 0, 0, 0);
+                        }
+                    }
+                }
+                float mx = -INFINITY;
+#pragma unroll
+                for (int st = 0; st < 4; ++st) {
+                    if (st < nsub) {
+                        if (st == nsub - 1 && (a.nk_valid & 31) != 0) {
+                            const int nv = (a.nk_valid & 31) - 4 * hi;
+#pragma unroll
+                            for (int r = 0; r < 16; ++r) s[st][r] = ((r & 3) + 8 * (r >> 2)) < nv ? s[st][r] : -INFINITY;
+                        }
+#pragma unroll
+                        for (int r = 0; r < 16; ++r) mx = fmaxf(mx, s[st][r]);
+                    }
+                }
+                mx = fmaxf(mx, __shfl_xor(mx, 32));
+#pragma unroll
+                for (int st = 0; st < 4; ++st) {
+                    if (st < nsub) {
+#pragma unroll
+                        for (int r = 0; r < 16; ++r) {
+                            const float pv = __builtin_amdgcn_exp2f(s[st][r] - mx);
+                            s[st][r] = pv;
+                            if constexpr (!ONES) psum += pv;
+                        }
+                    }
+                }
+#pragma unroll
+                for (int i = 0; i < DT; ++i)
+#pragma unroll
+                    for (int r = 0; r < 16; ++r) acc[i][r] = 0.f;
+#pragma unroll
+                for (int st = 0; st < 4; ++st) {
+                    if (st < nsub) {
+#pragma unroll
+                        for (int tt = 0; tt < 2; ++tt) {
+                            half8_t pf;
+#pragma unroll
+                            for (int j = 0; j < 8; ++j) pf[j] = (half_t)s[st][8 * tt + j];
+                            const char* Vs = Vsm + l31 * VPITCH + (st * 32 + 16 * tt + 8 * hi) * 2;
+#pragma unroll
+                            for (int i = 0; i < DT; ++i) {
+                                const half8_t vf = *reinterpret_cast<const half8_t*>(Vs + i * 32 * VPITCH);
+                                acc[i] = __builtin_amdgcn_mfma_f32_32x32x16_f16(vf, pf, acc[i], 0, 0, 0);
+                            }
+                        }
+                    }
+                }
+            } else {
+                const bool two = nsub > 2;
+                const int nv = (a.nk_valid & 31) - 4 * hi;
+                f32x16 s[4];
+#pragma unroll
+                for (int st = 0; st < 2; ++st) {
+#pragma unroll
+                    for (int r = 0; r < 16; ++r) s[st][r] = 0.f;
+                    if (st < nsub) {
+                        const char* Ks = Ksm + (st * 32 + l31) * KPITCH + hi * 16;
+#pragma unroll
+                        for (int ks = 0; ks < D16; ++ks) {
+                            const half8_t kf = *reinterpret_cast<const half8_t*>(Ks + ks * 32);
+                            s[st] = __builtin_amdgcn_mfma_f32_32x32x16_f16(kf, qs[ks], s[st], 0, 0, 0);
+                        }
+                        if (st == nsub - 1 && (a.nk_valid & 31) != 0) {
+#pragma unroll
+                            for (int r = 0; r < 16; ++r) s[st][r] = ((r & 3) + 8 * (r >> 2)) < nv ? s[st][r] : -INFINITY;
+                        }
+                    } else {
+#pragma unroll
+                        for (int r = 0; r < 16; ++r) s[st][r] = -INFINITY;
+                    }
+                }
+                float m0 = s[0][0];
+#pragma unroll
+                for (int st = 0; st < 2; ++st)
+#pragma unroll
+                    for (int r = 0; r < 16; ++r) m0 = fmaxf(m0, s[st][r]);
+                m0 = fmaxf(m0, __shfl_xor(m0, 32));
+                float delta = 0.f;
+                bool resc = false;
+                if (two) {
+                    const float negm = 0.f - m0;
+                    float mx = -INFINITY;
+#pragma unroll
+                    for (int st = 2; st < 4; ++st) {
+#pragma unroll
+                        for (int r = 0; r < 16; ++r) s[st][r] = negm;
+                        if (st < nsub) {
+                            const char* Ks = Ksm + (st * 32 + l31) * KPITCH + hi * 16;
+#pragma unroll
+                            for (int ks = 0; ks < D16; ++ks) {
+                                const half8_t kf = *reinterpret_cast<const half8_t*>(Ks + ks * 32);
+                                s[st] = __builtin_amdgcn_mfma_f32_32x32x16_f16(kf, qs[ks], s[st], 0, 0, 0);
+                            }
+                            if (st == nsub - 1 && (a.nk_valid & 31) != 0) {
+#pragma unroll
+                                for (int r = 0; r < 16; ++r) s[st][r] = ((r & 3) + 8 * (r >> 2)) < nv ? s[st][r] : -INFINITY;
+                            }
+#pragma unroll
+                            for (int r = 0; r < 16; ++r) mx = fmaxf(mx, s[st][r]);
+                        } else {
+#pragma unroll
+                            for (int r = 0; r < 16; ++r) s[st][r] = -INFINITY;
+                        }
+                    }
+                    mx = fmaxf(mx, __shfl_xor(mx, 32));
+                    resc =!__all(mx <= CFGPP_ATTN_RESCALE_THR);
+                    delta = fmaxf(mx, 0.f);
+                }
+#pragma unroll
+                for (int i = 0; i < DT; ++i)
+#pragma unroll
+                    for (int r = 0; r < 16; ++r) acc[i][r] = 0.f;
+                auto pv_tile = [&](int t) {
+                    float tsum = 0.f;
+#pragma unroll
+                    for (int st = 2 * t; st < 2 * t + 2; ++st)
+#pragma unroll
+                        for (int r = 0; r < 16; ++r) {
+                            const float pv = __builtin_amdgcn_exp2f(s[st][r]);
+                            s[st][r] = pv;
+                            tsum += pv;
+                        }
+#pragma unroll
+                    for (int st = 2 * t; st < 2 * t + 2; ++st) {
+                        if (st < nsub) {
+#pragma unroll
+                            for (int tt = 0; tt < 2; ++tt) {
+                                half8_t pf;
+#pragma unroll
+                                for (int j = 0; j < 8; ++j) pf[j] = (half_t)s[st][8 * tt + j];
+                                const char* Vs = Vsm + l31 * VPITCH + (st * 32 + 16 * tt + 8 * hi) * 2;
+#pragma unroll
+                                for (int i = 0; i < DT; ++i) {
+                                    const half8_t vf = *reinterpret_cast<const half8_t*>(Vs + i * 32 * VPITCH);
+                                    acc[i] = __builtin_amdgcn_mfma_f32_32x32x16_f16(vf, pf, acc[i], 0, 0, 0);
+                                }
+                            }
+                        }
+                    }
+                    return tsum;
+                };
+#pragma unroll
+                for (int st = 0; st < 2; ++st)
+#pragma unroll
+                    for (int r = 0; r < 16; ++r) s[st][r] -= m0;
+                psum = pv_tile(0);
+                if (two) {
+                    if (resc) {
+                        const float alpha = __builtin_amdgcn_exp2f(-delta);
+                        psum *= alpha;
+#pragma unroll
+                        for (int i = 0; i < DT; ++i)
+#pragma unroll
+                            for (int r = 0; r < 16; ++r) acc[i][r] *= alpha;
+#pragma unroll
+                        for (int st = 2; st < 4; ++st)
+#pragma unroll
+                            for (int r = 0; r < 16; ++r) s[st][r] -= delta;
+                    }
+                    psum += pv_tile(1);
+                }
+            }
+            float l_tot;
+            if constexpr (ONES) {
+                const int dr = a.d & 31;
+                float lv = 0.f;
+#pragma unroll
+                for (int gg = 0; gg < 4; ++gg) if (dr == 8 * gg) lv = acc[DT - 1][4 * gg];
+                l_tot = __shfl(lv, l31);
+            } else {
+                l_tot = psum + __shfl_xor(psum, 32);
+            }
+            const float inv_l = 1.0f / l_tot;
+            const int qrow = qbase + blk * 128;
+            if (qrow < a.nq) {
+                half_t* orow = a.o + ((long)b * a.nq + qrow) * a.o_ld + head * a.d;
+#pragma unroll
+                for (int i = 0; i < DT; ++i)
+#pragma unroll
+                    for (int gg = 0; gg < 4; ++gg) {
+                        const int dd = i * 32 + 8 * gg + 4 * hi;
+                        if (dd < a.d) {
+                            half4_t o;
+#pragma unroll
+                            for (int k = 0; k < 4; ++k) o[k] = (half_t)(acc[i][4 * gg + k] * inv_l);
+                            *reinterpret_cast<half4_t*>(orow + dd) = o;
+                        }
+                    }
+            }
+#pragma unroll
+            for (int i = 0; i < DT; ++i)
+#pragma unroll
+                for (int r = 0; r < 16; ++r) acc[i][r] = 0.f;
+        }
+        kt = ktn; blk = blkn;
+    }
+}
+
+constexpr int xfused_smem(int dt, int nsub) {
+    return 2 * dt * 32 * 128 + nsub * 32 * (dt * 64 + 16) + dt * 32 * (nsub * 64 + 16);
+}
+
+template <int DT, int D16, bool ONES, bool FLASH>
+int launch_xfused(const XFusedArgs& a, dim3 grid, int nsub, hipStream_t s) {
+    static bool attr_set = false;
+    auto kern = xattn_fused_kernel<DT, D16, ONES, FLASH>;
+    if (!attr_set) {
+        CFGPP_HIP_CHECK(hipFuncSetAttribute(reinterpret_cast<const void*>(kern), hipFuncAttributeMaxDynamicSharedMemorySize, xfused_smem(DT, 4)));
+        attr_set = true;
+    }
+    hipLaunchKernelGGL(kern, grid, dim3(256), xfused_smem(DT, nsub), s, a);
+    return 0;
+}
+
+}
+
+extern "C" {
+
+int cfgpp_xattn_fused_supported(int heads, int d, int C, int nk) {
+    const bool inst = d == 32 || d == 40 || d == 64 || d == 80 || d == 160;
+    return inst && heads > 0 && heads * d == C && C % 64 == 0 && nk > 0 && nk <= 128;
+}
+
+int cfgpp_xattn_fused_preferred(int heads, int d, int C, int nk) {
+    return cfgpp_xattn_fused_supported(heads, d, C, nk) && d != 64;
+}
+
+int cfgpp_op_xattn_fused(const void* x, const void* wq, const void* k, const void* vt, void* o, int B, int heads, int d, int C,
+                         int nq, int nk, int k_tok_pad, int wrap, void* stream) {
+    CFGPP_REQUIRE(x && wq && k && vt && o && B > 0 && nq > 0, "xattn_fused: bad args");
+    CFGPP_REQUIRE(cfgpp_xattn_fused_supported(heads, d, C, nk), "xattn_fused: no kernel instance for heads=%d d=%d C=%d keys=%d", heads, d, C, nk);
+    CFGPP_REQUIRE(k_tok_pad % 32 == 0 && k_tok_pad >= 32 * ((nk + 31) >> 5), "xattn_fused: k_tok_pad=%d (keys=%d)", k_tok_pad, nk);
+    CFGPP_REQUIRE(wrap > 0 && wrap <= B, "xattn_fused: wrap=%d (rows=%d)", wrap, B);
+    XFusedArgs a;
+    a.x = (const half_t*)x; a.wq = (const half_t*)wq; a.k = (const half_t*)k; a.vt = (const half_t*)vt; a.o = (half_t*)o;
+    a.heads = heads; a.d = d; a.C = C; a.nq = nq; a.nk_valid = nk; a.k_tok_pad = k_tok_pad; a.o_ld = C; a.wrap = wrap;
+    a.scale_log2e = (1.0f / sqrtf((float)d)) * 1.4426950408889634f;
+    const int nqb = cdiv(nq, 128), BH = B * heads;
+    int xqb = 1;
+    while (xqb < 8 && nqb % (xqb * 2) == 0 && (long)BH * (nqb / (xqb * 2)) >= 512) xqb *= 2;
+    a.xqb = xqb; a.nxb = nqb / xqb;
+    const dim3 grid(BH * a.nxb);
+    const int nsub = (nk + 31) >> 5;
+    hipStream_t s = (hipStream_t)stream;
+    int rc;
+    switch (d) {
+        case 32: rc = launch_xfused<1, 2, false, true>(a, grid, nsub, s); break;
+        case 40: rc = launch_xfused<2, 3, true, false>(a, grid, nsub, s); break;
+        case 64: rc = launch_xfused<2, 4, false, false>(a, grid, nsub, s); break;
+        case 80: rc = launch_xfused<3, 5, true, true>(a, grid, nsub, s); break;
+        default: rc = launch_xfused<5, 10, false, true>(a, grid, nsub, s); break;
+    }
+    if (rc) return -1;
+    CFGPP_HIP_CHECK(hipGetLastError());
+    return 0;
+}
+
+}
diff --git a/cfgpp_amd/engine.py b/cfgpp_amd/engine.py
--- a/cfgpp_amd/engine.py
+++ b/cfgpp_amd/engine.py
@@ -304,6 +304,9 @@
     def shared_prefix_ops(self, rows: int, z_rows: int) -> int:
         return int(self.lib.cfgpp_unet_shared_prefix_ops(self._h, int(rows), int(z_rows)))
 
+    def fused_xattn_sites(self) -> int:
+        return int(self.lib.cfgpp_unet_fused_xattn_sites(self._h))
+
     def device_bytes(self) -> float:
         return float(self.lib.cfgpp_unet_device_bytes(self._h))
 
@@ -314,3 +317,11 @@
 
 def share_prefix_enabled() -> bool:
     return bool(_lib.load().cfgpp_unet_share_prefix_enabled())
+
+
+def set_fuse_xattn(on: bool):
+    _lib.load().cfgpp_unet_set_fuse_xattn(1 if on else 0)
+
+
+def fuse_xattn_enabled() -> bool:
+    return bool(_lib.load().cfgpp_unet_fuse_xattn_enabled())
diff --git a/cfgpp_amd/hip_engine.py b/cfgpp_amd/hip_engine.py
--- a/cfgpp_amd/hip_engine.py
+++ b/cfgpp_amd/hip_engine.py
@@ -40,7 +40,8 @@
         self._pins = PinCache(getattr(cfg, "name", type(cfg).__name__), (self.H, self.W), torch.cuda.get_device_properties(self.device).name,
                               build_id(_lib.LIB_PATH), lambda rows: self.unet.export_tuning(rows), lambda h, rows: self.unet.import_tuning(h, rows),
                               knobs=lambda: (int(self.unet.lib.cfgpp_igemm_tuner_state()),),
-                              mode=lambda rows: "shared" if self.unet.shared_prefix_ops(rows, rows // 2) else "")
+                              mode=lambda rows: "_".join(m for m in ("shared" if self.unet.shared_prefix_ops(rows, rows // 2) else "",
+                                                                      "" if self.unet.fused_xattn_sites() else "xq2") if m))
         self._ctx_key = None
         self._ctx = None
         self._control = None
```

Result: no change. 9.101 images/sec (median of 6 runs) (+0.1%).
